# LabJunBMI/E3-invaraint-diffusion-model

Measured on AMD Instinct MI355X. Metric: denoising-steps/sec (batched pocket graphs), higher is better.
Workload: dtype f32 storage and accumulation, f16x3 products (fp32 grade); 1 GPU; structure_model sampling step, 256 x 256-residue pockets per GPU, 12+12 layers x 768, T=1000 schedule, encoder recomputed every step (as the reference); pockets_per_gpu=256, seq_len=256, parallelism=pocket-sharded x1, no collective

## Files before the change

### e3-invaraint-diffusion-model_amd/autograd.py

```python
import os

import torch

from . import hip, ops
from .ops import _chk, _p, _stream


def gemm_general(a, a_kmajor, b, b_kmajor, M, N, K, bias=None, act=ops.ACT_NONE, mode=None):
    _chk(a, "gemm_general.a"); _chk(b, "gemm_general.b"); _chk(bias, "gemm_general.bias")
    assert a.dim() == 2 and b.dim() == 2 and a.stride(1) == 1 and b.stride(1) == 1
    out = torch.empty((M, N), device=a.device, dtype=torch.float32)
    terms = ops.GEMM_MODES[ops.GEMM_MODE if mode is None else mode] or 6
    hip.check(hip.lib().e3d_gemm_f32_split_general(_p(a), a.stride(0), int(a_kmajor), _p(b), b.stride(0),
                                                   int(b_kmajor), _p(bias), _p(out), out.stride(0), M, N, K, act,
                                                   terms, _stream()), "e3d_gemm_f32_split_general")
    return out


class deferred_weight_grads:
    active = None

    MAX_BYTES = int(float(os.environ.get("E3D_DEFER_WGRAD_MAX_GB", "16")) * 2 ** 30)

    OVERLAP = os.environ.get("E3D_WGRAD_OVERLAP", "0") == "1"
# ... 437 lines not shown
        dy = torch.empty_like(y)
        dmod = torch.zeros_like(mod)
        hip.check(hip.lib().e3d_adaln_gate_bwd(_p(dout), _p(y), _p(mod), ctx.branch, ctx.rpc, _p(dy), _p(dmod), M, H,
                                               _stream()), "e3d_adaln_gate_bwd")
        return dout, dy, dmod, None, None


class _EmbedLayerNorm(torch.autograd.Function):

    @staticmethod
    def forward(ctx, x, weight, bias, gamma, beta, eps, post_add, rows_per_add):
        out, z = ops.embed_layernorm(x, weight, bias, gamma, beta, eps, post_add, rows_per_add, want_z=True)
        ctx.save_for_backward(x, z, gamma)
        ctx.eps, ctx.rpa, ctx.has_add = eps, rows_per_add, post_add is not None
        return out

    @staticmethod
    def backward(ctx, dout):
        x, z, gamma = ctx.saved_tensors
        dout = dout.contiguous()
        dz, dg, db_ln = layernorm_bwd(dout, z, gamma, ctx.eps)
        dW, db = small_k_wgrad(dz, x)
        dadd = group_sum(dout, ctx.rpa) if (ctx.has_add and ctx.needs_input_grad[6]) else None
        return None, dW, db, dg, db_ln, None, dadd, None


class _HeadLinear(torch.autograd.Function):
    @staticmethod
    def forward(ctx, x, weight, bias):
        ctx.save_for_backward(x, weight)
        return ops.head_linear(x, weight, bias)

    @staticmethod
    def backward(ctx, dout):
        x, weight = ctx.saved_tensors
        dout = dout.contiguous()
        M, H = x.shape
        dx = torch.empty_like(x)
        hip.check(hip.lib().e3d_head_linear_bwd_dx(_p(dout), _p(weight), _p(dx), M, H, weight.shape[0], _stream()),
                  "e3d_head_linear_bwd_dx")
        dW, _ = small_k_wgrad(x, dout, transpose_out=True, want_bias=False)
        return dx, dW, colsum(dout)


FUSE_HIDDEN_DROPOUT = os.environ.get("E3D_FUSE_HIDDEN_DROPOUT", "1") == "1"


def _needs_grad(*tensors):
    return torch.is_grad_enabled() and any(t is not None and t.requires_grad for t in tensors)


class functional:
    @staticmethod
    def linear(x, weight, bias=None, act=ops.ACT_NONE, absmax=None):
        if _needs_grad(x, weight, bias):
            out = _Linear.apply(x, weight, bias, act, absmax)
        else:
            out = ops.gemm(x, weight, bias, act, absmax=absmax)
        if absmax is not None:
            out._e3d_absmax = absmax
        return out

    @staticmethod
    def attention(q_src, kv_src, B, nh, Lq, Lk, key_mask=None, dist_emb=None, max_pos=0, drop_p=0.0, row_keys=None):
        q_abs = getattr(q_src, "_e3d_absmax", None)
        k_abs = q_abs if kv_src is None else getattr(kv_src, "_e3d_absmax", None)
        bounds = (q_abs, k_abs) if q_abs is not None and k_abs is not None else None
        if _needs_grad(q_src, kv_src, dist_emb):
            return _Attention.apply(q_src, kv_src, dist_emb, key_mask, B, nh, Lq, Lk, max_pos, drop_p, bounds, row_keys)
        q, k, v = _Attention._views(q_src, kv_src, nh * 64)
        drop = ops.site_drop(drop_p, row_keys) if drop_p > 0 else None
        return ops.attention(q, k, v, B, nh, Lq, Lk, key_mask=key_mask, dist_emb=dist_emb, max_pos=max_pos, drop=drop,
                             bounds=bounds)

    @staticmethod
    def dropout(x, p, training=True, row_keys=None):
        if not training or not p:
            return x
        if _needs_grad(x):
            return _Dropout.apply(x, p, row_keys)
        p, seed = ops.site_drop(p, row_keys)[:2]
        return ops.dropout(x.contiguous(), p, seed, row_keys=row_keys)

    @staticmethod
    def residual_layernorm(x, residual, gamma, beta, eps, p_drop=0.0, row_keys=None):
        if _needs_grad(x, residual, gamma, beta):
            return _ResidualLayerNorm.apply(x, residual, gamma, beta, eps, p_drop, row_keys)
        drop = ops.site_drop(p_drop, row_keys) if p_drop and p_drop > 0 else None
        return ops.residual_layernorm(x, residual, gamma, beta, eps, drop=drop)

    @staticmethod
    def linear_residual_layernorm(x, weight, bias, residual, gamma, beta, eps, p_drop=0.0, row_keys=None):
        if not p_drop and not _needs_grad(x, weight, bias, residual, gamma, beta):
            return ops.linear_residual_layernorm(x, weight, bias, residual, gamma, beta, eps)
        fn = functional
        if FUSE_HIDDEN_DROPOUT:
            return fn.residual_layernorm(fn.linear(x, weight, bias), residual, gamma, beta, eps, p_drop, row_keys)
        return fn.residual_layernorm(fn.dropout(fn.linear(x, weight, bias), p_drop, row_keys=row_keys), residual, gamma, beta, eps)

    @staticmethod
    def adaln_gate(x, y, mod, branch, rows_per_cond):
        if _needs_grad(x, y, mod):
            return _AdaLNGate.apply(x, y, mod, branch, rows_per_cond)
        return ops.adaln_gate(x, y, mod, branch, rows_per_cond)

    @staticmethod
    def embed_layernorm(x, weight, bias, gamma, beta, eps, post_add=None, rows_per_add=1):
        if _needs_grad(weight, bias, gamma, beta, post_add):
            return _EmbedLayerNorm.apply(x, weight, bias, gamma, beta, eps, post_add, rows_per_add)
        return ops.embed_layernorm(x, weight, bias, gamma, beta, eps, post_add, rows_per_add)

    @staticmethod
    def head_linear(x, weight, bias):
        if _needs_grad(x, weight, bias):
            return _HeadLinear.apply(x, weight, bias)
        return ops.head_linear(x, weight, bias)
```

### e3-invaraint-diffusion-model_amd/bert.py

```python
from dataclasses import dataclass

import os

import torch
from torch import nn

from . import ops
from .autograd import functional as F


@dataclass
class BertConfig:
    hidden_size: int = 768
    num_attention_heads: int = 12
    intermediate_size: int = 1024
    num_hidden_layers: int = 12
    max_position_embeddings: int = 64
    position_embedding_type: str = "relative_key"
    hidden_dropout_prob: float = 0.1
    attention_probs_dropout_prob: float = 0.1
    layer_norm_eps: float = 1e-12
    hidden_act: str = "gelu"
    use_cache: bool = False
    is_decoder: bool = False
# ... 111 lines not shown
    if not ok:
        with torch.no_grad():
            ent = torch.cat([t.detach() for t in tensors], dim=0).contiguous()
            r0 = 0
            for t in tensors:
                t.data = ent[r0:r0 + t.shape[0]]
                r0 += t.shape[0]
        tied[name] = ent
    return ent


def _packed(owner, name, weights, biases):
    if torch.is_grad_enabled() and any(t.requires_grad for t in weights):
        if TIE_PACKED and all(t.dtype == torch.float32 for t in list(weights) + list(biases)):
            w, b = _TiedPack.apply(_tie(owner, "w_" + name, weights), _tie(owner, "b_" + name, biases), len(weights),
                                   *weights, *biases)
        else:
            w, b = torch.cat(list(weights), dim=0), torch.cat(list(biases), dim=0)
        w._e3d_parts, b._e3d_parts = list(weights), list(biases)
        return w, b
    out = []
    cache = owner.__dict__.setdefault("_e3d_pack", {})
    for key_name, tensors in (("w_" + name, weights), ("b_" + name, biases)):
        key = ops.weight_key(*tensors)
        hit = cache.get(key_name)
        if hit is None or hit[0] != key:
            with torch.no_grad():
                hit = (key, torch.cat([t.detach() for t in tensors], dim=0).contiguous())
            cache[key_name] = hit
        out.append(hit[1])
    return out[0], out[1]


def qkv_weights(sa):
    return _packed(sa, "qkv", [sa.query.weight, sa.key.weight, sa.value.weight], [sa.query.bias, sa.key.bias, sa.value.bias])


def kv_weights(sa):
    return _packed(sa, "kv", [sa.key.weight, sa.value.weight], [sa.key.bias, sa.value.bias])


def dropout_rates(module):
    if not module.training:
        return 0.0, 0.0
    cfg = module.config
    return float(getattr(cfg, "hidden_dropout_prob", 0.0)), float(getattr(cfg, "attention_probs_dropout_prob", 0.0))


def _attention_output(att, ctx, x, p_hidden=0.0, row_keys=None):
    return F.linear_residual_layernorm(ctx, att.output.dense.weight, att.output.dense.bias, x, att.output.LayerNorm.weight,
                                       att.output.LayerNorm.bias, att.eps, p_hidden, row_keys)


def drop_keys(drop):
    return drop[2] if len(drop) > 2 else None


def run_self_attention(att, x, mask, B, L, drop=(0.0, 0.0), layout=None):
    sa = att.self
    w, b = qkv_weights(sa)
    qkv = F.linear(x, w, b, absmax=ops.absmax_slot(sa, "qkv", x.device))
    relkey = sa.position_embedding_type == "relative_key"
    if layout is not None:
        H = att.num_heads * 64
        ctx = ops.attention_varlen(qkv[:, :H], qkv[:, H:2 * H], qkv[:, 2 * H:], layout, layout, att.num_heads,
                                   dist_emb=sa.distance_embedding.weight if relkey else None,
                                   max_pos=sa.max_position_embeddings)
        return _attention_output(att, ctx, x)
    ctx = F.attention(qkv, None, B, att.num_heads, L, L, key_mask=mask,
                      dist_emb=sa.distance_embedding.weight if relkey else None,
                      max_pos=sa.max_position_embeddings, drop_p=drop[1], row_keys=drop_keys(drop))
    return _attention_output(att, ctx, x, drop[0], drop_keys(drop))


def project_cross_kv(att, enc):
    w, b = kv_weights(att.self)
    return F.linear(enc, w, b, absmax=torch.zeros(1, device=enc.device, dtype=torch.float32))


def run_cross_attention(att, x, kv, enc_mask, B, Lq, Lk, drop=(0.0, 0.0), layout=None, enc_layout=None):
    q = F.linear(x, att.self.query.weight, att.self.query.bias, absmax=ops.absmax_slot(att.self, "q", x.device))
    if layout is not None:
        H = att.num_heads * 64
        ctx = ops.attention_varlen(q, kv[:, :H], kv[:, H:], layout, enc_layout, att.num_heads)
        return _attention_output(att, ctx, x)
    ctx = F.attention(q, kv, B, att.num_heads, Lq, Lk, key_mask=enc_mask, drop_p=drop[1], row_keys=drop_keys(drop))
    return _attention_output(att, ctx, x, drop[0], drop_keys(drop))


def run_layer(layer, x, mask, B, L, cross_kv=None, enc_mask=None, Lk=None, drop=(0.0, 0.0), layout=None,
              enc_layout=None):
    x = run_self_attention(layer.attention, x, mask, B, L, drop, layout=layout)
    if hasattr(layer, "crossattention"):
        if cross_kv is None:
            raise ValueError("decoder layer needs encoder states")
        x = run_cross_attention(layer.crossattention, x, cross_kv, enc_mask, B, L, Lk, drop, layout=layout,
                                enc_layout=enc_layout)
    inter = F.linear(x, layer.intermediate.dense.weight, layer.intermediate.dense.bias, ops.ACT_GELU)
    return F.linear_residual_layernorm(inter, layer.output.dense.weight, layer.output.dense.bias, x,
                                       layer.output.LayerNorm.weight, layer.output.LayerNorm.bias, layer.eps, drop[0],
                                       drop_keys(drop))


def run_encoder(encoder, x, mask, B, L, enc=None, enc_mask=None, Lk=None, cross_kv=None, layout=None, enc_layout=None,
                row_keys=None):
    drop = dropout_rates(encoder)
    if layout is not None and drop != (0.0, 0.0):
        raise RuntimeError("packed layouts are inference-only: put the model in eval mode")
    if row_keys is not None:
        drop = drop + (row_keys,)
    for i, layer in enumerate(encoder.layer):
        kv = None
        if hasattr(layer, "crossattention"):
            kv = cross_kv[i] if cross_kv is not None else project_cross_kv(layer.crossattention, enc)
        x = run_layer(layer, x, mask, B, L, kv, enc_mask, Lk, drop, layout=layout, enc_layout=enc_layout)
    return x
```

### e3-invaraint-diffusion-model_amd/csrc/attn_relkey_coop.hip

```cpp
#include <type_traits>

#include "e3d_common.h"

namespace {

typedef __bf16 bf16x8 __attribute__((ext_vector_type(8)));
typedef __bf16 bf16x4 __attribute__((ext_vector_type(4)));
typedef _Float16 f16x8 __attribute__((ext_vector_type(8)));
typedef _Float16 f16x4 __attribute__((ext_vector_type(4)));
template <typename E> struct AV;
template <> struct AV<__bf16> { typedef bf16x8 x8; typedef bf16x4 x4; };
template <> struct AV<_Float16> { typedef f16x8 x8; typedef f16x4 x4; };
template <typename X> struct Elem;
template <> struct Elem<bf16x8> { typedef __bf16 type; };
template <> struct Elem<bf16x4> { typedef __bf16 type; };
template <> struct Elem<f16x8> { typedef _Float16 type; };
template <> struct Elem<f16x4> { typedef _Float16 type; };
__device__ __forceinline__ f32x16 mma16(const bf16x8 a, const bf16x8 b, const f32x16 c) {
    return __builtin_amdgcn_mfma_f32_32x32x16_bf16(a, b, c, 0, 0, 0);
}
__device__ __forceinline__ f32x16 mma16(const f16x8 a, const f16x8 b, const f32x16 c) {
    return __builtin_amdgcn_mfma_f32_32x32x16_f16(a, b, c, 0, 0, 0);
}

// ... 54 lines not shown
    acc = mma16(a[0], b[1], acc);
    acc = mma16(a[1], b[0], acc);
    acc = mma16(a[0], b[0], acc);
    return acc;
}

typedef short short4v __attribute__((ext_vector_type(4)));
typedef short short8v __attribute__((ext_vector_type(8)));
template <typename X8>
__device__ __forceinline__ X8 tr_read8(const unsigned char* lo4, const unsigned char* hi4) {
    typedef __attribute__((address_space(3))) short4v* lds_p;
    const short4v a = __builtin_amdgcn_ds_read_tr16_b64_v4i16((lds_p)(lo4));
    const short4v b = __builtin_amdgcn_ds_read_tr16_b64_v4i16((lds_p)(hi4));
    const short8v c = __builtin_shufflevector(a, b, 0, 1, 2, 3, 4, 5, 6, 7);
    return __builtin_bit_cast(X8, c);
}

template <typename E>
__global__ __launch_bounds__(256) void e_fragments_kernel(const float* __restrict__ e, typename AV<E>::x8* __restrict__ frag,
                                                          int P, int J0, int n_items, float* __restrict__ e_absmax) {
    const int i = blockIdx.x * 256 + threadIdx.x;
    if (i >= n_items) return;
    const int lane = i & 63, kb = (i >> 6) & 3, plane = (i >> 8) & 1, j = i >> 9;
    const int row = min(max(P + 32 * (j - J0) + (lane & 31), 0), 2 * P - 2);
    const float* src = e + row * D + 16 * kb + 8 * (lane >> 5);
    typename AV<E>::x8 out;
    unsigned amax = 0;
#pragma unroll
    for (int t = 0; t < 8; ++t) {
        const float v = src[t];
        const E hi = (E)v;
        out[t] = plane ? (E)(v - (float)hi) : hi;
        e3d_absmax_accum(amax, v);
    }
    frag[i] = out;
    if (e_absmax && plane == 0) e3d_absmax_commit(amax, e_absmax, lane);
}

#ifdef E3D_ATTN_STAMPS
__device__ long long e3d_attn_stamps[16][8];
#define ASTAMP(slot)                                                                                     \
    do {                                                                                                 \
        if (blockIdx.x == 1000 && wid == 1 && lane == 0 && kt < 16) e3d_attn_stamps[kt][slot] = __builtin_readcyclecounter(); \
    } while (0)
#define KSTAMP(i)                                                                                        \
    do {                                                                                                 \
        if (blockIdx.x == 1000 && wid == 1 && lane == 0) e3d_attn_stamps[15][i] = __builtin_readcyclecounter(); \
    } while (0)
#else
#define ASTAMP(slot) do {} while (0)
#define KSTAMP(i) do {} while (0)
#endif

template <int W, bool RELKEY, typename E, bool DROP = false>
__global__ __launch_bounds__(W * 64, 2) void attn_coop_kernel(
    const float* __restrict__ q, int64_t q_bs, int64_t q_rs, const float* __restrict__ k, int64_t k_bs,
    int64_t k_rs, const float* __restrict__ v, int64_t v_bs, int64_t v_rs, const typename AV<E>::x8* __restrict__ e_frag,
    int P, const float* __restrict__ key_mask, float* __restrict__ out, float* __restrict__ lse, int nh, int Lq, int Lk,
    int groups_per_bh, int skip_padded_tiles, E3dBounds bnd, float rescale_tau, E3dDrop drop_in) {
    const E3dDrop drop = e3d_drop_resolve(drop_in);
    typedef typename AV<E>::x8 bf16x8;
    typedef typename AV<E>::x4 bf16x4;
    extern __shared__ __attribute__((aligned(16))) unsigned char smem_raw[];
    constexpr int NT = W * 64, NI = 512 / NT;
    const int tid = threadIdx.x, lane = tid & 63, wid = tid >> 6;
    const int qi = lane & 31, half = lane >> 5;
    const int blk = xcd_remap(blockIdx.x, gridDim.x);
    const int grp = blk % groups_per_bh, bh = blk / groups_per_bh, h = bh % nh, b = bh / nh;
    const int q0 = (grp * W + wid) * 32;
    float* ring = reinterpret_cast<float*>(smem_raw + 2 * KV_BUF_B) + wid * RING_F;
    KSTAMP(0);

    const float* kb_ = k + b * k_bs + h * D;
    const float* vb_ = v + b * v_bs + h * D;
    const float* mb = key_mask ? key_mask + (int64_t)b * Lk : nullptr;
    f32x4 qraw[8];
    {
        const float* qrow = q + b * q_bs + (int64_t)min(q0 + qi, Lq - 1) * q_rs + h * D + 8 * half;
#pragma unroll
        for (int kb = 0; kb < 4; ++kb) {
            qraw[2 * kb] = *reinterpret_cast<const f32x4*>(qrow + 16 * kb);
            qraw[2 * kb + 1] = *reinterpret_cast<const f32x4*>(qrow + 16 * kb + 4);
        }
    }
    uint64_t drop_row = 0;
    if (DROP) drop_row = e3d_drop_attn_row(drop, b, h, nh, Lq, Lk, min(q0 + qi, Lq - 1));
    const bool scan_mask = mb && skip_padded_tiles && e3d_mask_skip_is_exact(bnd);
    float mv[4];
    {
        const float* mp = mb ? mb : kb_;
#pragma unroll
        for (int c = 0; c < 4; ++c) mv[c] = mp[min(64 * c + lane, Lk - 1)];
    }

    bf16x8 qf[4][2];
    int k_tiles = (Lk + 31) >> 5;

    constexpr bool DEEP = NI <= 2;
    constexpr int NSET = DEEP ? 2 : 1;
    f32x4 sk[NSET][NI], sv[NSET][NI];
    float smask[NSET];
    int voff_k[NI], voff_v[NI];
#pragma unroll
    for (int i = 0; i < NI; ++i) {
        const int f = tid + NT * i;
        voff_k[i] = ((f >> 4) * (int)k_rs + 4 * (f & 15)) * 4;
        voff_v[i] = ((f >> 4) * (int)v_rs + 4 * (f & 15)) * 4;
// ... 176 lines not shown
        if (DROP) {
#pragma unroll
            for (int g = 0; g < 4; ++g) {
                float m[4];
                e3d_drop_mult4_row(drop, drop_row, (uint32_t)(kt * 8 + 2 * g + half), m);
#pragma unroll
                for (int j = 0; j < 4; ++j) s[4 * g + j] *= m[j];
            }
        }
        ASTAMP(4);

        const unsigned char* vr = buf + 2 * K_PLANE_B + (4 * half + ((lane >> 2) & 3)) * V_ROW_B +
                                  2 * (16 * ((lane >> 4) & 1) + 4 * (lane & 3));
#pragma unroll
        for (int st = 0; st < 2; ++st) {
            float pv[8];
#pragma unroll
            for (int j = 0; j < 8; ++j) pv[j] = s[8 * st + j];
            bf16x8 pb[2], a0[2], a1[2];
            split8x2(pv, pb[0], pb[1]);
            const unsigned char* v0 = vr + 16 * st * V_ROW_B;
#pragma unroll
            for (int pl = 0; pl < 2; ++pl) {
                a0[pl] = tr_read8<bf16x8>(v0 + pl * V_PLANE_B, v0 + pl * V_PLANE_B + 8 * V_ROW_B);
                a1[pl] = tr_read8<bf16x8>(v0 + pl * V_PLANE_B + 64, v0 + pl * V_PLANE_B + 8 * V_ROW_B + 64);
            }
            o0 = mfma3(a0, pb, o0);
            o1 = mfma3(a1, pb, o1);
        }

        ASTAMP(5);
        if (more) {
            if (DEEP == (PAR == 0)) stage_store(Set1{}, kt_next * 32, smem_raw + (PAR ^ 1) * KV_BUF_B);
            else stage_store(Set0{}, kt_next * 32, smem_raw + (PAR ^ 1) * KV_BUF_B);
        }
        ASTAMP(6);
        if (RELKEY && more) {
            const f32x16 t = dot_q(ef);
            e_load(qt - (kt + 2 < k_tiles ? kt + 2 : k_tiles - 1) - 1 + J0);
#pragma unroll
            for (int r = 0; r < 16; ++r) ring_w[(32 * (PAR ^ 1) + (r & 3) + 8 * (r >> 2)) * RING_LD] = t[r];
        }
        __syncthreads();
        ASTAMP(7);
    };
    for (int kt = 0; kt < k_tiles; kt += 2) {
        tile(std::integral_constant<int, 0>{}, kt);
        if (kt + 1 < k_tiles) tile(std::integral_constant<int, 1>{}, kt + 1);
    }

    KSTAMP(2);
    const float l_tot = l_run + __shfl_xor(l_run, 32, 64);
    const float inv = 1.0f / l_tot;
    __builtin_amdgcn_wave_barrier();
#pragma unroll
    for (int g = 0; g < 4; ++g) {
        f32x4 a, c;
#pragma unroll
        for (int j = 0; j < 4; ++j) { a[j] = o0[4 * g + j] * inv; c[j] = o1[4 * g + j] * inv; }
        *reinterpret_cast<f32x4*>(ring + qi * OUT_LD + 8 * g + 4 * half) = a;
        *reinterpret_cast<f32x4*>(ring + qi * OUT_LD + 32 + 8 * g + 4 * half) = c;
    }
    __builtin_amdgcn_fence(__ATOMIC_RELEASE, "wavefront");
    __builtin_amdgcn_wave_barrier();
    __builtin_amdgcn_fence(__ATOMIC_ACQUIRE, "wavefront");
    float* obase = out + ((int64_t)b * Lq + q0) * (nh * D) + h * D;
#pragma unroll
    for (int i = 0; i < 8; ++i) {
        const int row = 4 * i + (lane >> 4);
        if (q0 + row < Lq)
            *reinterpret_cast<f32x4*>(obase + (int64_t)row * (nh * D) + 4 * (lane & 15)) =
                *reinterpret_cast<const f32x4*>(ring + row * OUT_LD + 4 * (lane & 15));
    }
    if (lse && half == 0 && q0 + qi < Lq) lse[((int64_t)b * nh + h) * Lq + q0 + qi] = m_run * LN2 + logf(l_tot);
    KSTAMP(3);
#ifdef E3D_ATTN_STAMPS
    asm volatile("s_waitcnt vmcnt(0)" ::: "memory");
    KSTAMP(4);
#endif
}

template <int W, bool RELKEY, typename E>
int launch_w(const float* q, int64_t q_bs, int64_t q_rs, const float* k, int64_t k_bs, int64_t k_rs, const float* v,
             int64_t v_bs, int64_t v_rs, const void* e_frag, int P, const float* key_mask,
             float* out, float* lse, int B, int nh, int Lq, int Lk, int q_tiles, int skip, E3dBounds bnd, E3dDrop drop,
             bool dropping, hipStream_t s) {
    const size_t lds = 2 * KV_BUF_B + (size_t)W * RING_F * sizeof(float);
    const int groups = q_tiles / W;
    if constexpr (std::is_same<E, __bf16>::value) {
        if (dropping) {
            static std::atomic<uint64_t> lds_ok_d{0};
            e3d_allow_lds(lds_ok_d, attn_coop_kernel<W, RELKEY, E, true>, lds);
            hipLaunchKernelGGL((attn_coop_kernel<W, RELKEY, E, true>), dim3(B * nh * groups), dim3(W * 64), lds, s, q, q_bs, q_rs,
                               k, k_bs, k_rs, v, v_bs, v_rs, reinterpret_cast<const typename AV<E>::x8*>(e_frag), P, key_mask,
                               out, lse, nh, Lq, Lk, groups, skip, bnd, g_rescale_tau, drop);
            return e3d_launch_status("e3d_relkey_attn_fwd_split (cooperative, dropout)");
        }
    }
    static std::atomic<uint64_t> lds_ok{0};
    e3d_allow_lds(lds_ok, attn_coop_kernel<W, RELKEY, E>, lds);
    hipLaunchKernelGGL((attn_coop_kernel<W, RELKEY, E>), dim3(B * nh * groups), dim3(W * 64), lds, s, q, q_bs, q_rs, k, k_bs,
                       k_rs, v, v_bs, v_rs, reinterpret_cast<const typename AV<E>::x8*>(e_frag), P, key_mask, out, lse, nh, Lq, Lk, groups, skip, bnd, g_rescale_tau, drop);
    return e3d_launch_status("e3d_relkey_attn_fwd_split (cooperative)");
}

template <bool RELKEY, typename E>
int launch_any(int W, const float* q, int64_t q_bs, int64_t q_rs, const float* k, int64_t k_bs, int64_t k_rs,
               const float* v, int64_t v_bs, int64_t v_rs, const void* e_frag, int P,
               const float* key_mask, float* out, float* lse, int B, int nh, int Lq, int Lk, int q_tiles, int skip,
               E3dBounds bnd, E3dDrop drop, bool dropping, hipStream_t s) {
#define E3D_COOP_CASE(w)                                                                                          \
    case w:                                                                                                       \
        return launch_w<w, RELKEY, E>(q, q_bs, q_rs, k, k_bs, k_rs, v, v_bs, v_rs, e_frag, P, key_mask, out, lse, B, nh, \
                                   Lq, Lk, q_tiles, skip, bnd, drop, dropping, s)
    switch (W) {
        E3D_COOP_CASE(8);
        E3D_COOP_CASE(4);
    }
#undef E3D_COOP_CASE
    return -1;
}

}

template <typename E>
static int coop_launch_t(const float* q, int64_t q_bs, int64_t q_rs, const float* k, int64_t k_bs, int64_t k_rs,
                         const float* v, int64_t v_bs, int64_t v_rs, const float* dist_emb, int P,
                         const float* key_mask, float* out, float* lse, int B, int nh, int Lq, int Lk, int skip,
                         E3dBounds bnd, void* e_scratch, int e_ready, E3dDrop drop, bool dropping, hipStream_t s) {
    const int q_tiles = (Lq + 31) / 32;
    static int w_pref = 0;
    if (!w_pref) {
        const char* e = getenv("E3D_ATTN_W");
        w_pref = e ? atoi(e) : 4;
    }
    const int W = (w_pref == 8 && q_tiles % 8 == 0) ? 8 : 4;
    if (!dist_emb)
        return launch_any<false, E>(W, q, q_bs, q_rs, k, k_bs, k_rs, v, v_bs, v_rs, nullptr, P, key_mask, out, lse, B, nh,
                                    Lq, Lk, q_tiles, skip, bnd, drop, dropping, s);
    if (!e_scratch) {
        e3d_set_error("attn_coop: rel-key attention needs the caller's scratch for the distance-table planes");
        return -1;
    }
    const int J0 = (Lk + 31) / 32, n_items = 2 * J0 * 512;
    if (!e_ready)
        hipLaunchKernelGGL(e_fragments_kernel<E>, dim3((n_items + 255) / 256), dim3(256), 0, s, dist_emb,
                           reinterpret_cast<typename AV<E>::x8*>(e_scratch), P, J0, n_items, (float*)nullptr);
    return launch_any<true, E>(W, q, q_bs, q_rs, k, k_bs, k_rs, v, v_bs, v_rs, e_scratch, P, key_mask, out, lse, B, nh, Lq,
                               Lk, q_tiles, skip, bnd, drop, dropping, s);
}

int e3d_attn_coop_launch(const float* q, int64_t q_bs, int64_t q_rs, const float* k, int64_t k_bs, int64_t k_rs,
                         const float* v, int64_t v_bs, int64_t v_rs, const float* dist_emb, int P,
                         const float* key_mask, float* out, float* lse, int B, int nh, int Lq, int Lk, int skip,
                         E3dBounds bnd, void* e_scratch, int e_ready, int f16, E3dDrop drop, bool dropping, hipStream_t s) {
    if (f16)
        return coop_launch_t<_Float16>(q, q_bs, q_rs, k, k_bs, k_rs, v, v_bs, v_rs, dist_emb, P, key_mask, out, lse, B, nh, Lq,
                                       Lk, skip, bnd, e_scratch, e_ready, drop, dropping, s);
    return coop_launch_t<__bf16>(q, q_bs, q_rs, k, k_bs, k_rs, v, v_bs, v_rs, dist_emb, P, key_mask, out, lse, B, nh, Lq, Lk,
                                 skip, bnd, e_scratch, e_ready, drop, dropping, s);
}

extern "C" float e3d_attn_rescale_tau(float tau) {
    const float prev = g_rescale_tau;
    if (tau >= 0.f) g_rescale_tau = tau;
    return prev;
}

#ifdef E3D_ATTN_STAMPS
extern "C" int e3d_debug_read_attn_stamps(long long* host_out) {
    return (int)hipMemcpyFromSymbol(host_out, HIP_SYMBOL(e3d_attn_stamps), sizeof(long long) * 16 * 8);
}
#endif

int e3d_attn_fill_planes(const float* dist_emb, int P, int Lk, void* scratch, int f16, float* e_absmax, hipStream_t s) {
    const int J0 = (Lk + 31) / 32, n_items = 2 * J0 * 512;
    if (f16)
        hipLaunchKernelGGL(e_fragments_kernel<_Float16>, dim3((n_items + 255) / 256), dim3(256), 0, s, dist_emb,
                           reinterpret_cast<f16x8*>(scratch), P, J0, n_items, e_absmax);
    else
        hipLaunchKernelGGL(e_fragments_kernel<__bf16>, dim3((n_items + 255) / 256), dim3(256), 0, s, dist_emb,
                           reinterpret_cast<bf16x8*>(scratch), P, J0, n_items, e_absmax);
    return e3d_launch_status("e3d_relkey_attn_fwd_split (distance-table planes)");
}

extern "C" int64_t e3d_attn_scratch_bytes(int Lk) { return (int64_t)2 * ((Lk + 31) / 32) * 512 * 16; }
```

### e3-invaraint-diffusion-model_amd/csrc/attn_relkey_split.hip

```cpp
#include "attn_split_frag.h"

namespace {

template <int NS, bool RELKEY, bool DROP, typename E>
__global__ __launch_bounds__(256, 2) void attn_fwd_split_kernel(
    const float* __restrict__ q, int64_t q_bs, int64_t q_rs, const float* __restrict__ k, int64_t k_bs,
    int64_t k_rs, const float* __restrict__ v, int64_t v_bs, int64_t v_rs, const float* __restrict__ dist_emb,
    int P, const float* __restrict__ key_mask, float* __restrict__ out, float* __restrict__ lse, int nh, int Lq,
    int Lk, int q_tiles, int n_units, int skip_padded_tiles, E3dBounds bnd, E3dDrop drop_in) {
    const E3dDrop drop = e3d_drop_resolve(drop_in);
    typedef typename AV<E>::x8 bf16x8;
    extern __shared__ __attribute__((aligned(16))) float smem[];
    const int lane = threadIdx.x & 63, wid = threadIdx.x >> 6;
    const int qi = lane & 31, half = lane >> 5;
    const int unit = xcd_remap(blockIdx.x, gridDim.x) * (blockDim.x >> 6) + wid;
    if (unit >= n_units) return;
    const int qt = unit % q_tiles, bh = unit / q_tiles, h = bh % nh, b = bh / nh;
    float* ring = smem + wid * WAVE_LDS_F;
    float* stg = ring + RING_F;
    float* kbias = stg + STG_F;

    const int q0 = qt * 32;
    const int lq = min(q0 + qi, Lq - 1);
    uint64_t drop_row = 0;
// ... 116 lines not shown
            split8<NS>(v0, a0);
            split8<NS>(v1, a1);
            o0 = mfma_terms<NS>(a0, pb, o0);
            o1 = mfma_terms<NS>(a1, pb, o1);
        }
    }

    const float l_tot = l_run + __shfl_xor(l_run, 32, 64);
    const float inv = 1.0f / l_tot;
    if (q0 + qi < Lq) {
        float* orow = out + ((int64_t)b * Lq + q0 + qi) * (nh * D) + h * D;
#pragma unroll
        for (int g = 0; g < 4; ++g) {
            f32x4 lo, hi;
            lo[0] = o0[4 * g + 0] * inv; lo[1] = o1[4 * g + 0] * inv;
            lo[2] = o0[4 * g + 1] * inv; lo[3] = o1[4 * g + 1] * inv;
            hi[0] = o0[4 * g + 2] * inv; hi[1] = o1[4 * g + 2] * inv;
            hi[2] = o0[4 * g + 3] * inv; hi[3] = o1[4 * g + 3] * inv;
            *reinterpret_cast<f32x4*>(orow + 16 * g + 8 * half) = lo;
            *reinterpret_cast<f32x4*>(orow + 16 * g + 8 * half + 4) = hi;
        }
        if (lse && half == 0) lse[((int64_t)b * nh + h) * Lq + q0 + qi] = m_run + logf(l_tot);
    }
}

int g_skip_padded = 1;

template <int NS, bool DROP = false, typename E = __bf16>
int launch(const float* q, int64_t q_bs, int64_t q_rs, const float* k, int64_t k_bs, int64_t k_rs, const float* v,
           int64_t v_bs, int64_t v_rs, const float* dist_emb, int P, const float* key_mask, float* out, float* lse,
           int B, int nh, int Lq, int Lk, E3dBounds bnd, hipStream_t s, E3dDrop drop = E3dDrop{0, 0, 1.f}) {
    const int q_tiles = (Lq + 31) / 32;
    const int n_units = B * nh * q_tiles;
    const int wpb = 4;
    const int n_blocks = (n_units + wpb - 1) / wpb;
    const size_t lds = (size_t)wpb * WAVE_LDS_F * sizeof(float);
    if (dist_emb)
        hipLaunchKernelGGL((attn_fwd_split_kernel<NS, true, DROP, E>), dim3(n_blocks), dim3(64 * wpb), lds, s, q, q_bs, q_rs, k,
                           k_bs, k_rs, v, v_bs, v_rs, dist_emb, P, key_mask, out, lse, nh, Lq, Lk, q_tiles, n_units, g_skip_padded, bnd, drop);
    else
        hipLaunchKernelGGL((attn_fwd_split_kernel<NS, false, DROP, E>), dim3(n_blocks), dim3(64 * wpb), lds, s, q, q_bs, q_rs, k,
                           k_bs, k_rs, v, v_bs, v_rs, dist_emb, P, key_mask, out, lse, nh, Lq, Lk, q_tiles, n_units, g_skip_padded, bnd, drop);
    return e3d_launch_status("e3d_relkey_attn_fwd_split");
}

}

extern "C" int e3d_attn_skip_padded_tiles(int enable) {
    const int prev = g_skip_padded;
    g_skip_padded = enable ? 1 : 0;
    return prev;
}

static int attn_fwd_dispatch(const float* q, int64_t q_bs, int64_t q_rs, const float* k, int64_t k_bs, int64_t k_rs,
                             const float* v, int64_t v_bs, int64_t v_rs, const float* dist_emb, int P, const float* key_mask,
                             float* out, float* lse, int B, int nh, int Lq, int Lk, int terms, float drop_p, const E3dDrop d,
                             void* e_scratch, int e_scratch_ready, const float* q_absmax, const float* k_absmax,
                             float* e_absmax, void* stream) {
    const E3dBounds bnd{q_absmax, k_absmax, dist_emb ? e_absmax : nullptr};
    E3D_REQUIRE(!dist_emb || !q_absmax || e_absmax, "attn_split: rel-key attention with element bounds needs e_absmax too");
    E3D_REQUIRE(drop_p >= 0.f && drop_p < 1.f, "attn_split: drop_p=%g outside [0, 1)", (double)drop_p);
    E3D_REQUIRE(q && k && v && out, "attn_split: null pointer");
    E3D_REQUIRE(B > 0 && nh > 0 && Lq > 0 && Lk > 0, "attn_split: bad shape B=%d nh=%d Lq=%d Lk=%d", B, nh, Lq, Lk);
    E3D_REQUIRE(q_rs % 4 == 0 && k_rs % 4 == 0 && v_rs % 2 == 0 && q_bs % 4 == 0 && k_bs % 4 == 0 && v_bs % 2 == 0,
                "attn_split: strides must keep 16B (q,k) / 8B (v) alignment");
    E3D_REQUIRE(((uintptr_t)q % 16) == 0 && ((uintptr_t)k % 16) == 0 && ((uintptr_t)v % 16) == 0 &&
                    ((uintptr_t)out % 16) == 0, "attn_split: pointers must be 16B aligned");
    E3D_REQUIRE(terms == 3 || terms == 6 || terms == E3D_TERMS_F16X3, "attn_split: terms must be 3, 6 or 19 (got %d)", terms);
    const int f16 = terms == E3D_TERMS_F16X3;
    E3D_REQUIRE((int64_t)Lk * k_rs < (1ll << 30) && (int64_t)Lk * v_rs < (1ll << 30),
                "attn_split: one batch item's K/V slab must stay below 2^30 elements (32-bit lane offsets)");
    if (dist_emb) {
        E3D_REQUIRE(Lq == Lk && Lq <= P, "attn_split: relative_key needs Lq == Lk <= P (Lq=%d Lk=%d P=%d)", Lq, Lk, P);
        E3D_REQUIRE(((uintptr_t)dist_emb % 16) == 0, "attn_split: dist_emb must be 16B aligned");
    }
    E3D_REQUIRE((int64_t)B * nh * ((Lq + 31) / 32) < (1ll << 30), "attn_split: too many tiles");
    hipStream_t s = (hipStream_t)stream;
    if (dist_emb && e_scratch && !e_scratch_ready) {
        const int rc = e3d_attn_fill_planes(dist_emb, P, Lk, e_scratch, f16, e_absmax, s);
        if (rc) return rc;
        e_scratch_ready = 1;
    }
    static int coop = -1;
    if (coop < 0) {
        const char* e = getenv("E3D_ATTN_COOP");
        coop = e ? atoi(e) : 1;
    }
    const bool dropping = drop_p > 0.f;
    const bool span_ok = (int64_t)Lk * (k_rs > v_rs ? k_rs : v_rs) * 4 < ((int64_t)1 << 31) && k_rs > 0 && v_rs > 0 &&
                         k_rs < ((int64_t)1 << 24) && v_rs < ((int64_t)1 << 24);
    if ((terms == 3 || (f16 && !dropping)) && coop && span_ok && v_rs % 4 == 0 && v_bs % 4 == 0 && ((Lq + 31) / 32) % 4 == 0 &&
        (!dist_emb || e_scratch))
        return e3d_attn_coop_launch(q, q_bs, q_rs, k, k_bs, k_rs, v, v_bs, v_rs, dist_emb, P, key_mask, out, lse, B, nh,
                                    Lq, Lk, g_skip_padded, bnd, e_scratch, e_scratch_ready, f16, d, dropping, s);
    if (dropping) {
        if (terms == 3)
            return launch<2, true>(q, q_bs, q_rs, k, k_bs, k_rs, v, v_bs, v_rs, dist_emb, P, key_mask, out, lse, B, nh, Lq, Lk, bnd, s, d);
        return launch<3, true>(q, q_bs, q_rs, k, k_bs, k_rs, v, v_bs, v_rs, dist_emb, P, key_mask, out, lse, B, nh, Lq, Lk, bnd, s, d);
    }
    if (f16)
        return launch<2, false, _Float16>(q, q_bs, q_rs, k, k_bs, k_rs, v, v_bs, v_rs, dist_emb, P, key_mask, out, lse, B, nh,
                                          Lq, Lk, bnd, s);
    if (terms == 3)
        return launch<2>(q, q_bs, q_rs, k, k_bs, k_rs, v, v_bs, v_rs, dist_emb, P, key_mask, out, lse, B, nh, Lq, Lk, bnd, s);
    return launch<3>(q, q_bs, q_rs, k, k_bs, k_rs, v, v_bs, v_rs, dist_emb, P, key_mask, out, lse, B, nh, Lq, Lk, bnd, s);
}

extern "C" int e3d_relkey_attn_fwd_split_ex(const float* q, int64_t q_bs, int64_t q_rs, const float* k, int64_t k_bs,
                                            int64_t k_rs, const float* v, int64_t v_bs, int64_t v_rs,
                                            const float* dist_emb, int P, const float* key_mask, float* out,
                                            float* lse, int B, int nh, int Lq, int Lk, int terms, float drop_p,
                                            uint64_t drop_seed, void* e_scratch, int e_scratch_ready, const float* q_absmax,
                                            const float* k_absmax, float* e_absmax, void* stream) {
    return attn_fwd_dispatch(q, q_bs, q_rs, k, k_bs, k_rs, v, v_bs, v_rs, dist_emb, P, key_mask, out, lse, B, nh, Lq, Lk, terms,
                             drop_p, e3d_drop_make(drop_p, drop_seed), e_scratch, e_scratch_ready, q_absmax, k_absmax, e_absmax,
                             stream);
}

extern "C" int e3d_relkey_attn_fwd_split_ex_keyed(const float* q, int64_t q_bs, int64_t q_rs, const float* k, int64_t k_bs,
                                                  int64_t k_rs, const float* v, int64_t v_bs, int64_t v_rs,
                                                  const float* dist_emb, int P, const float* key_mask, float* out,
                                                  float* lse, int B, int nh, int Lq, int Lk, int terms, float drop_p,
                                                  uint32_t site, const uint64_t* row_keys, void* e_scratch, int e_scratch_ready,
                                                  const float* q_absmax, const float* k_absmax, float* e_absmax, void* stream) {
    E3D_REQUIRE(row_keys && drop_p > 0.f, "attn_split (keyed): row keys and drop_p > 0 required");
    E3D_REQUIRE(site < E3D_DROP_MAX_SITE && nh < E3D_DROP_MAX_HEADS, "attn_split (keyed): site %u / %d heads out of range", site, nh);
    return attn_fwd_dispatch(q, q_bs, q_rs, k, k_bs, k_rs, v, v_bs, v_rs, dist_emb, P, key_mask, out, lse, B, nh, Lq, Lk, terms,
                             drop_p, e3d_drop_make_keyed(drop_p, site, row_keys), e_scratch, e_scratch_ready, q_absmax, k_absmax,
                             e_absmax, stream);
}

extern "C" int e3d_relkey_attn_fwd_split(const float* q, int64_t q_bs, int64_t q_rs, const float* k, int64_t k_bs,
                                         int64_t k_rs, const float* v, int64_t v_bs, int64_t v_rs,
                                         const float* dist_emb, int P, const float* key_mask, float* out, float* lse,
                                         int B, int nh, int Lq, int Lk, int terms, void* stream) {
    return e3d_relkey_attn_fwd_split_ex(q, q_bs, q_rs, k, k_bs, k_rs, v, v_bs, v_rs, dist_emb, P, key_mask, out, lse, B,
                                        nh, Lq, Lk, terms, 0.f, 0, nullptr, 0, nullptr, nullptr, nullptr, stream);
}

extern "C" int e3d_relkey_attn_fwd_split_drop(const float* q, int64_t q_bs, int64_t q_rs, const float* k, int64_t k_bs,
                                              int64_t k_rs, const float* v, int64_t v_bs, int64_t v_rs,
                                              const float* dist_emb, int P, const float* key_mask, float* out,
                                              float* lse, int B, int nh, int Lq, int Lk, int terms, float drop_p,
                                              uint64_t drop_seed, void* stream) {
    return e3d_relkey_attn_fwd_split_ex(q, q_bs, q_rs, k, k_bs, k_rs, v, v_bs, v_rs, dist_emb, P, key_mask, out, lse, B,
                                        nh, Lq, Lk, terms, drop_p, drop_seed, nullptr, 0, nullptr, nullptr, nullptr, stream);
}

extern "C" int e3d_relkey_attn_fwd_split_drop_keyed(const float* q, int64_t q_bs, int64_t q_rs, const float* k, int64_t k_bs,
                                                    int64_t k_rs, const float* v, int64_t v_bs, int64_t v_rs,
                                                    const float* dist_emb, int P, const float* key_mask, float* out,
                                                    float* lse, int B, int nh, int Lq, int Lk, int terms, float drop_p,
                                                    uint32_t site, const uint64_t* row_keys, void* stream) {
    return e3d_relkey_attn_fwd_split_ex_keyed(q, q_bs, q_rs, k, k_bs, k_rs, v, v_bs, v_rs, dist_emb, P, key_mask, out, lse, B,
                                              nh, Lq, Lk, terms, drop_p, site, row_keys, nullptr, 0, nullptr, nullptr, nullptr,
                                              stream);
}
```

### e3-invaraint-diffusion-model_amd/csrc/e3d_common.h

```cpp
#pragma once
#include <hip/hip_runtime.h>
#include <stdint.h>
#include <stdio.h>
#include <math.h>
#include <atomic>

#include "../../include/e3d_hip.h"

typedef float f32x4 __attribute__((ext_vector_type(4)));
typedef float f32x16 __attribute__((ext_vector_type(16)));

void e3d_set_error(const char* fmt, ...);

struct E3dBounds { const float* q; const float* k; const float* e; };


#define E3D_REQUIRE(cond, ...)       \
    do {                             \
        if (!(cond)) {               \
            e3d_set_error(__VA_ARGS__); \
            return -1;               \
        }                            \
    } while (0)

// ... 130 lines not shown
    d.epoch = e3d_dropout_epoch_ptr();
    d.thr = (uint32_t)t;
    d.scale = 65536.0f / (float)(65536 - t);
    d.row_keys = nullptr;
    d.site = 0;
    return d;
}
#define E3D_DROP_MAX_SITE (1u << 24)
#define E3D_DROP_MAX_HEADS (1 << 16)
static inline E3dDrop e3d_drop_make_keyed(float p, uint32_t site, const uint64_t* row_keys) {
    E3dDrop d = e3d_drop_make(p, 0);
    d.epoch = nullptr;
    d.row_keys = row_keys;
    d.site = (uint64_t)site << 40;
    return d;
}
__device__ __forceinline__ E3dDrop e3d_drop_resolve(E3dDrop d) {
    if (d.epoch) d.seed += *d.epoch * 0xD1342543DE82EF95ull;
    d.epoch = nullptr;
    return d;
}
__device__ __forceinline__ void e3d_drop_mult4_row(const E3dDrop d, uint64_t row_term, uint32_t group, float (&m)[4]) {
    uint64_t z = row_term + group;
    z = (z ^ (z >> 30)) * 0xBF58476D1CE4E5B9ull;
    z = (z ^ (z >> 27)) * 0x94D049BB133111EBull;
    z ^= z >> 31;
#pragma unroll
    for (int j = 0; j < 4; ++j) m[j] = ((uint32_t)(z >> (16 * j)) & 0xFFFFu) >= d.thr ? d.scale : 0.f;
}
__device__ __forceinline__ uint64_t e3d_drop_hidden_row(const E3dDrop d, int64_t row, int H4) {
    if (d.row_keys) return d.row_keys[row] * 0x9E3779B97F4A7C15ull + 0x9E3779B97F4A7C15ull + d.site;
    return (uint64_t)row * (uint64_t)H4 + d.seed * 0x9E3779B97F4A7C15ull + 0x9E3779B97F4A7C15ull;
}
__device__ __forceinline__ uint64_t e3d_drop_attn_row(const E3dDrop d, int b, int h, int nh, int Lq, int Lk, int q) {
    if (d.row_keys)
        return d.row_keys[(int64_t)b * Lq + q] * 0x9E3779B97F4A7C15ull + 0x9E3779B97F4A7C15ull + (d.site | (uint64_t)h << 24);
    return ((uint64_t)(b * nh + h) * Lq + q) * (uint64_t)((Lk + 3) >> 2) + d.seed * 0x9E3779B97F4A7C15ull +
           0x9E3779B97F4A7C15ull;
}
__device__ __forceinline__ void e3d_drop_mult4(const E3dDrop d, uint64_t idx4, float (&m)[4]) {
    uint64_t z = idx4 + d.seed * 0x9E3779B97F4A7C15ull + 0x9E3779B97F4A7C15ull;
    z = (z ^ (z >> 30)) * 0xBF58476D1CE4E5B9ull;
    z = (z ^ (z >> 27)) * 0x94D049BB133111EBull;
    z ^= z >> 31;
#pragma unroll
    for (int j = 0; j < 4; ++j) m[j] = ((uint32_t)(z >> (16 * j)) & 0xFFFFu) >= d.thr ? d.scale : 0.f;
}

int e3d_attn_fill_planes(const float* dist_emb, int P, int Lk, void* scratch, int f16, float* e_absmax, hipStream_t s);

int e3d_attn_coop_launch(const float* q, int64_t q_bs, int64_t q_rs, const float* k, int64_t k_bs, int64_t k_rs,
                         const float* v, int64_t v_bs, int64_t v_rs, const float* dist_emb, int P,
                         const float* key_mask, float* out, float* lse, int B, int nh, int Lq, int Lk, int skip,
                         E3dBounds bnd, void* e_scratch, int e_ready, int f16, E3dDrop drop, bool dropping, hipStream_t s);

int e3d_attn_bwd_split_launch(const float* q, int64_t q_bs, int64_t q_rs, const float* k, int64_t k_bs, int64_t k_rs,
                              const float* v, int64_t v_bs, int64_t v_rs, const float* dist_emb, int P,
                              const float* key_mask, const float* out, const float* lse, const float* dout, float* dq,
                              int64_t dq_bs, int64_t dq_rs, float* dk, int64_t dk_bs, int64_t dk_rs, float* dv,
                              int64_t dv_bs, int64_t dv_rs, float* Pm, float* dSm, float* part, int B, int nh, int Lq,
                              int Lk, E3dDrop drop, bool dropping, hipStream_t s);

int64_t e3d_attn_bwd_coop_scratch_bytes(int Lk);
int64_t e3d_attn_bwd_coop_de_floats(int Lq, int Lk);
bool e3d_attn_bwd_coop_supported(int Lq, int Lk, bool dropping);
int e3d_attn_bwd_coop_launch(const float* q, int64_t q_bs, int64_t q_rs, const float* k, int64_t k_bs, int64_t k_rs,
                             const float* v, int64_t v_bs, int64_t v_rs, const float* dist_emb, int P,
                             const float* key_mask, const float* out, const float* lse, const float* dout, float* dq,
                             int64_t dq_bs, int64_t dq_rs, float* dk, int64_t dk_bs, int64_t dk_rs, float* dv,
                             int64_t dv_bs, int64_t dv_rs, float* d_dist_emb, void* e_scratch, float* part, int B, int nh,
                             int Lq, int Lk, E3dDrop drop, bool dropping, hipStream_t s);

__device__ __forceinline__ int xcd_remap(int id, int n) {
    const int q = n >> 3, r = n & 7, xcd = id & 7, slot = id >> 3;
    return (xcd < r ? xcd * (q + 1) : r * (q + 1) + (xcd - r) * q) + slot;
}
```

### e3-invaraint-diffusion-model_amd/csrc/gemm_rowln.hip

```cpp
#include <type_traits>

#include "e3d_common.h"

namespace {

typedef __bf16 bf16x8 __attribute__((ext_vector_type(8)));
typedef _Float16 f16x8 __attribute__((ext_vector_type(8)));
template <typename E> struct V8;
template <> struct V8<__bf16> { typedef bf16x8 t; };
template <> struct V8<_Float16> { typedef f16x8 t; };
__device__ __forceinline__ f32x16 mma16(const bf16x8 a, const bf16x8 b, const f32x16 c) {
    return __builtin_amdgcn_mfma_f32_32x32x16_bf16(a, b, c, 0, 0, 0);
}
__device__ __forceinline__ f32x16 mma16(const f16x8 a, const f16x8 b, const f32x16 c) {
    return __builtin_amdgcn_mfma_f32_32x32x16_f16(a, b, c, 0, 0, 0);
}

constexpr int RN = 768, RBM = 96, NBLK = RN / 32;
constexpr int W_STEP = NBLK * 2 * 1024;
constexpr int A_PAIR = 128 * 128;
constexpr int LDS_A = 2 * W_STEP;
constexpr int RES_CHUNK = 16 * RN * 4;
constexpr int LDS_STATS = 3 * RES_CHUNK;
constexpr int LDS_COLS = LDS_STATS + (8 * RBM + RBM) * 4;
// ... 39 lines not shown

#ifndef ROWLN_LAB
#define ROWLN_LAB 0
#endif
#ifdef ROWLN_STAMPS
__device__ long long rowln_stamps[2][64][8];
__device__ long long rowln_tile_stamps[2][8][8];
__device__ long long rowln_wg_times[512][4];
#define RSTAMP(step, slot)                                                                                        \
    do {                                                                                                          \
        if (stamp_on && (step) < 64 && lane == 0) rowln_stamps[wid >> 2][(step)][(slot)] = __builtin_readcyclecounter(); \
    } while (0)
#define TSTAMP(slot)                                                                                              \
    do {                                                                                                          \
        if (stamp_on && tile_no < 8 && lane == 0) rowln_tile_stamps[wid >> 2][tile_no][(slot)] = __builtin_readcyclecounter(); \
    } while (0)
#else
#define RSTAMP(step, slot) do {} while (0)
#define TSTAMP(slot) do {} while (0)
#endif
#define E3D_VMCNT(n) asm volatile("s_waitcnt vmcnt(" #n ")" ::: "memory")
#define E3D_BARRIER()                          \
    do {                                       \
        asm volatile("" ::: "memory");         \
        __builtin_amdgcn_s_barrier();          \
        asm volatile("" ::: "memory");         \
        __builtin_amdgcn_sched_barrier(0);     \
    } while (0)
#define E3D_LDS_BARRIER()                                   \
    do {                                                    \
        asm volatile("s_waitcnt lgkmcnt(0)" ::: "memory");  \
        E3D_BARRIER();                                      \
    } while (0)

template <int OFF = 0>
__device__ __forceinline__ void glds16(const void* g, unsigned char* lds_wave_base) {
    __builtin_amdgcn_global_load_lds((const __attribute__((address_space(1))) void*)g,
                                     (__attribute__((address_space(3))) void*)lds_wave_base, 16, OFF, 0);
}

__device__ __forceinline__ int next_tile_rows(int left, int pattern, int group_rows) {
#ifndef ROWLN_NO_PATTERNS
    if (group_rows == 256) {
        if (pattern == 1 && left == 256) return 64;
        if (pattern == 2 && left == 160) return 64;
        if (pattern == 3) return 64;
    }
#endif
    if (left >= 160 || left == 96) return 96;
    if (left > 96) return 64;
    return left;
}

template <typename E>
__global__ __launch_bounds__(512, 2) void gemm_rowln_kernel(const float* __restrict__ A, int64_t lda,
                                                            const unsigned char* __restrict__ Wp, const float* __restrict__ bias,
                                                            const float* __restrict__ res, int64_t ldr,
                                                            const float* __restrict__ gamma, const float* __restrict__ beta,
                                                            float eps, float* __restrict__ out, int64_t ldo, int M, int K,
                                                            int rows_per_wg, float out_scale) {
    extern __shared__ __attribute__((aligned(16))) unsigned char smem[];
    typedef typename V8<E>::t X8;
    const int tid = threadIdx.x, lane = tid & 63;
    const int wid = __builtin_amdgcn_readfirstlane(tid >> 6);
    const int l31 = lane & 31, half = lane >> 5;
    const int npairs = K / 32, last_step = 2 * npairs - 1;

    int row0 = blockIdx.x * rows_per_wg;
    const int row_end = min(M, row0 + rows_per_wg);
    if (row0 >= row_end) return;

    const unsigned w_lane = (unsigned)(wid * 6144 + lane * 16);
    unsigned a_lane[2];
    auto a_offsets = [&](int rows) {
#pragma unroll
        for (int i = 0; i < 2; ++i) {
            const int row = (wid + 8 * i) * 8 + (lane >> 3);
            a_lane[i] = (unsigned)(min(row, rows - 1) * (int)lda + (((lane & 7) ^ ((row >> 1) & 7)) << 2)) * 4u;
        }
    };
    unsigned r_lane[2];
#pragma unroll
    for (int j = 0; j < 2; ++j) r_lane[j] = (unsigned)((2 * wid + j) * (int)ldr + lane * 4) * 4u;
    const int a_roff = LDS_A + l31 * 128 + (((2 * half) ^ ((l31 >> 1) & 7)) << 4);
    const int b_roff = (wid * 3) * 2048 + lane * 16;

    auto issue_w = [&](int src, int buf) {
        const unsigned char* g = Wp + (int64_t)src * W_STEP + w_lane;
        unsigned char* l = smem + buf * W_STEP + wid * 6144;
        glds16<0>(g, l);
        glds16<1024>(g, l);
        glds16<2048>(g, l);
        glds16<3072>(g, l);
        glds16<0>(g + 4096, l + 4096);
        glds16<1024>(g + 4096, l + 4096);
    };
    auto issue_a = [&](const float* a_tile, int pair, int buf) {
        const unsigned char* g = reinterpret_cast<const unsigned char*>(a_tile + pair * 32);
        unsigned char* l = smem + LDS_A + buf * A_PAIR + wid * 1024;
        glds16<0>(g + a_lane[0], l);
        glds16<0>(g + a_lane[1], l + 8192);
    };

    float* red = reinterpret_cast<float*>(smem + LDS_STATS);
    float* rowc = red + 8 * RBM;
    const int colbase = wid * 96 + l31;
    float* colc = reinterpret_cast<float*>(smem + LDS_COLS);
    for (int i = tid; i < RN; i += 512) {
        colc[i] = bias ? bias[i] : 0.f;
        colc[RN + i] = gamma[i];
        colc[2 * RN + i] = beta[i];
    }
    asm volatile("s_waitcnt vmcnt(0) lgkmcnt(0)" ::: "memory");
    constexpr float inv_n = 1.0f / RN;
    const bool bit8 = (lane & 8) != 0, bit4 = (lane & 4) != 0, bit2 = (lane & 2) != 0,
               bit1 = (lane & 1) != 0;

    const int pattern = (blockIdx.x >> 3) & 3, group_rows = row_end - row0;
    int rows = next_tile_rows(row_end - row0, pattern, group_rows);
    a_offsets(rows);
    issue_a(A + (int64_t)row0 * lda, 0, 0);
    issue_w(0, 0);
    issue_w(1, 1);
    issue_a(A + (int64_t)row0 * lda, 1, 1);
    int next_row0 = 0, next_rows = 0;
#ifdef ROWLN_STAMPS
    const bool stamp_on = blockIdx.x == 77 && (wid & 3) == 0;
    int tile_no = 0;
    if (tid == 0 && blockIdx.x < 512) {
        rowln_wg_times[blockIdx.x][0] = __builtin_amdgcn_s_memrealtime();
        rowln_wg_times[blockIdx.x][1] = __builtin_readcyclecounter();
    }
#endif

    auto tile_body = [&](auto nm_c) -> bool {
        constexpr int NM = decltype(nm_c)::value;
        const float* a_tile = A + (int64_t)row0 * lda;
        f32x16 acc[NM][3];
#pragma unroll
        for (int m = 0; m < NM; ++m)
#pragma unroll
            for (int n = 0; n < 3; ++n)
#pragma unroll
                for (int r = 0; r < 16; ++r) acc[m][n][r] = 0.f;

        TSTAMP(0);
        int a_cur = 0, a_nxt = A_PAIR, a_nx2 = 2 * A_PAIR;
        E3D_VMCNT(8);
        E3D_BARRIER();
        TSTAMP(1);
        X8 bh0[3], bl0[3], bh1[3], bl1[3];
        f32x4 x0, x1;
#pragma unroll
        for (int n = 0; n < 3; ++n) {
            bh0[n] = *reinterpret_cast<const X8*>(smem + b_roff + n * 2048);
            bl0[n] = *reinterpret_cast<const X8*>(smem + b_roff + n * 2048 + 1024);
        }
        x0 = *reinterpret_cast<const f32x4*>(smem + a_cur + a_roff);
        x1 = *reinterpret_cast<const f32x4*>(smem + a_cur + (a_roff ^ 16));

        const bool res_on = res != nullptr && !(ROWLN_LAB & 1);
        const unsigned char* res_tile = reinterpret_cast<const unsigned char*>(res + (int64_t)row0 * ldr);
        const int64_t res_chunk_stride = 16 * ldr * 4;
        auto step = [&](auto ks_c, X8 (&bh)[3], X8 (&bl)[3], X8 (&nh)[3], X8 (&nl)[3], int w_next, int a_pair_next, int tail_chunk, int stamp_step) {
            constexpr int KS = decltype(ks_c)::value;
            RSTAMP(stamp_step, 0);
            asm volatile("s_waitcnt lgkmcnt(0)" ::: "memory");
            const bool tail = tail_chunk >= 0;
            const unsigned char* gbase = tail ? res_tile + tail_chunk * res_chunk_stride : Wp + (int64_t)w_next * W_STEP;
            const unsigned char* g0 = gbase + (tail ? r_lane[0] : w_lane);
            const unsigned char* g1 = gbase + (tail ? r_lane[1] : w_lane + 3072u);
            unsigned char* lw = smem + KS * W_STEP + wid * 6144;
            f32x4 y0 = x0, y1 = x1;
#pragma unroll
            for (int m = 0; m < NM; ++m) {
                X8 ah, al;
                split8(x0, x1, ah, al);
                if (m + 1 < NM) {
                    x0 = *reinterpret_cast<const f32x4*>(smem + a_cur + ((a_roff ^ (64 * KS)) + (m + 1) * 4096));
                    x1 = *reinterpret_cast<const f32x4*>(smem + a_cur + ((a_roff ^ (64 * KS + 16)) + (m + 1) * 4096));
                }
#pragma unroll
                for (int n = 0; n < 3; ++n) {
                    if (ROWLN_LAB & 8) {
                        asm volatile("" :: "v"(ah), "v"(al), "v"(bh[n]), "v"(bl[n]));
                    } else {
                        acc[m][n] = mma16(ah, bl[n], acc[m][n]);
                        acc[m][n] = mma16(al, bh[n], acc[m][n]);
                        acc[m][n] = mma16(ah, bh[n], acc[m][n]);
                    }
                    if (m == 0) {
                        if (n == 0) { glds16<0>(g0, lw); glds16<1024>(g0, lw); }
                        if (n == 1) { glds16<2048>(g0, lw); glds16<0>(g1, lw + 3072); }
                        if (n == 2) { glds16<1024>(g1, lw + 3072); glds16<2048>(g1, lw + 3072); }
                    }
                    __builtin_amdgcn_sched_barrier(0);
                }
                if (m == 0) {
                    RSTAMP(stamp_step, 1);
                    if (KS == 1) {
                        E3D_VMCNT(12);
                        E3D_BARRIER();
                        RSTAMP(stamp_step, 4);
                        if (a_pair_next >= 0) {
                            const unsigned char* ga = reinterpret_cast<const unsigned char*>(a_tile + a_pair_next * 32);
                            unsigned char* la = smem + LDS_A + a_nx2 + wid * 1024;
                            glds16<0>(ga + a_lane[0], la);
                            glds16<0>(ga + a_lane[1], la + 8192);
                        }
                    }
                    E3D_VMCNT(8);
                    RSTAMP(stamp_step, 3);
                    const unsigned char* wn = smem + (KS ^ 1) * W_STEP + b_roff;
#pragma unroll
                    for (int n = 0; n < 3; ++n) {
                        nh[n] = *reinterpret_cast<const X8*>(wn + n * 2048);
                        nl[n] = *reinterpret_cast<const X8*>(wn + n * 2048 + 1024);
                    }
                    const int an = KS == 0 ? a_cur : a_nxt;
                    y0 = *reinterpret_cast<const f32x4*>(smem + an + (a_roff ^ (64 * (KS ^ 1))));
                    y1 = *reinterpret_cast<const f32x4*>(smem + an + (a_roff ^ (64 * (KS ^ 1) + 16)));
                    __builtin_amdgcn_sched_barrier(0);
                }
            }
            x0 = y0;
            x1 = y1;
            RSTAMP(stamp_step, 2);
        };

        for (int p = 0; p < npairs; ++p) {
            const bool last_pair = p + 1 == npairs;
            step(std::integral_constant<int, 0>{}, bh0, bl0, bh1, bl1, min(2 * p + 2, last_step), 0, last_pair && res_on ? 0 : -1, 2 * p);
            step(std::integral_constant<int, 1>{}, bh1, bl1, bh0, bl0, min(2 * p + 3, last_step), last_pair ? -1 : min(p + 2, npairs - 1),
                 last_pair && res_on ? 1 : -1, 2 * p + 1);
            const int t = a_cur;
            a_cur = a_nxt;
            a_nxt = a_nx2;
            a_nx2 = t;
        }
        if (!res_on) E3D_VMCNT(0);
        E3D_LDS_BARRIER();
        TSTAMP(2);

#pragma unroll
        for (int m = 0; m < NM; ++m)
#pragma unroll
            for (int n = 0; n < 3; ++n)
#pragma unroll
                for (int r = 0; r < 16; ++r) acc[m][n][r] = fmaf(acc[m][n][r], out_scale, colc[colbase + 32 * n]);
        if (res_on) {
            auto issue_r = [&](int c) {
                const unsigned char* g = res_tile + c * res_chunk_stride;
                unsigned char* l = smem + (c % 3) * RES_CHUNK + wid * 6144;
                glds16<0>(g + r_lane[0], l);
                glds16<1024>(g + r_lane[0], l);
                glds16<2048>(g + r_lane[0], l);
                glds16<0>(g + r_lane[1], l + 3072);
                glds16<1024>(g + r_lane[1], l + 3072);
                glds16<2048>(g + r_lane[1], l + 3072);
            };
            constexpr int NCH = 2 * NM;
#pragma unroll
            for (int c = 0; c < NCH; ++c) {
                if (c + 1 < NCH) E3D_VMCNT(6);
                else E3D_VMCNT(0);
                E3D_BARRIER();
                if (c + 2 < NCH) issue_r(c + 2);
                const int m = c >> 1, r0 = 8 * (c & 1);
                const unsigned char* cb = smem + (c % 3) * RES_CHUNK + colbase * 4 + half * (4 * RN * 4);
#pragma unroll
                for (int n = 0; n < 3; ++n)
#pragma unroll
                    for (int j = 0; j < 8; ++j) {
                        const int lr = (j & 3) + 8 * (j >> 2);
// ... 102 lines not shown
                        else u[4 * q + j] = t;
                    }
                }
            if (PAIR) tv = reduce32(v);
            if (SINGLE) tu = reduce16(u);
            exchange(tv, tu, true);
        }
        TSTAMP(4);
        float gv[3], bt[3];
#pragma unroll
        for (int n = 0; n < 3; ++n) {
            gv[n] = colc[RN + colbase + 32 * n];
            bt[n] = colc[2 * RN + colbase + 32 * n];
        }
#pragma unroll
        for (int m = 0; m < NM; ++m)
#pragma unroll
            for (int q = 0; q < 4; ++q) {
                const f32x4 rstd = *reinterpret_cast<const f32x4*>(rowc + m * 32 + 8 * q + 4 * half);
                float* o = out + (int64_t)(row0 + m * 32 + 8 * q + 4 * half) * ldo + colbase;
#pragma unroll
                for (int j = 0; j < 4; ++j)
#pragma unroll
                    for (int n = 0; n < 3; ++n) o[(int64_t)j * ldo + 32 * n] = fmaf(acc[m][n][4 * q + j] * rstd[j], gv[n], bt[n]);
            }
        TSTAMP(5);
#ifdef ROWLN_STAMPS
        asm volatile("s_waitcnt vmcnt(0)" ::: "memory");
        TSTAMP(6);
        ++tile_no;
#endif
        if (more) E3D_LDS_BARRIER();
        return more;
    };

    while (true) {
        bool more;
        if (rows == 96) more = tile_body(std::integral_constant<int, 3>{});
        else if (rows == 64) more = tile_body(std::integral_constant<int, 2>{});
        else more = tile_body(std::integral_constant<int, 1>{});
        if (!more) break;
        row0 = next_row0;
        rows = next_rows;
    }
    E3D_VMCNT(0);
#ifdef ROWLN_STAMPS
    if (tid == 0 && blockIdx.x < 512) {
        rowln_wg_times[blockIdx.x][2] = __builtin_amdgcn_s_memrealtime();
        rowln_wg_times[blockIdx.x][3] = __builtin_readcyclecounter();
    }
#endif
}

template <typename E>
int launch_rowln(const float* A, int64_t lda, const void* Wp, const float* bias, const float* res, int64_t ldr,
                 const float* gamma, const float* beta, float eps, float* out, int64_t ldo, int M, int K, float out_scale,
                 hipStream_t s) {
    static std::atomic<uint64_t> lds_ok{0};
    e3d_allow_lds(lds_ok, gemm_rowln_kernel<E>, (size_t)LDS_TOTAL);
    const int n_cu = e3d_cu_count();
    const int rows_per_wg = ((M + n_cu - 1) / n_cu + 31) / 32 * 32;
    const int grid = (M + rows_per_wg - 1) / rows_per_wg;
    hipLaunchKernelGGL((gemm_rowln_kernel<E>), dim3(grid), dim3(512), LDS_TOTAL, s, A, lda,
                       reinterpret_cast<const unsigned char*>(Wp), bias, res, ldr, gamma, beta, eps, out, ldo, M, K, rows_per_wg,
                       out_scale);
    return e3d_launch_status("e3d_gemm_residual_layernorm_f32_split");
}

}

#ifdef ROWLN_STAMPS
extern "C" int e3d_debug_rowln_stamps(long long* steps, long long* tiles) {
    int rc = (int)hipMemcpyFromSymbol(steps, HIP_SYMBOL(rowln_stamps), sizeof(long long) * 2 * 64 * 8);
    if (rc) return rc;
    return (int)hipMemcpyFromSymbol(tiles, HIP_SYMBOL(rowln_tile_stamps), sizeof(long long) * 2 * 8 * 8);
}
extern "C" int e3d_debug_rowln_wg_times(long long* t) {
    return (int)hipMemcpyFromSymbol(t, HIP_SYMBOL(rowln_wg_times), sizeof(long long) * 512 * 4);
}
#endif

extern "C" int64_t e3d_weight_planes_bytes(int N, int K) { return (N % 32 || K % 16 || N <= 0 || K <= 0) ? -1 : (int64_t)N * K * 4; }

extern "C" int e3d_weight_planes_f32_split(const float* W, int N, int K, int terms, void* planes, void* stream) {
    E3D_REQUIRE(W && planes, "weight_planes: null pointer");
    E3D_REQUIRE(N > 0 && K > 0 && N % 32 == 0 && K % 16 == 0 && ((uintptr_t)W % 16) == 0 && ((uintptr_t)planes % 16) == 0,
                "weight_planes: need N%%32==0, K%%16==0, 16-byte alignment (N=%d K=%d)", N, K);
    E3D_REQUIRE(terms == 3 || terms == E3D_TERMS_F16X3, "weight_planes: terms must be 3 or 19 (got %d)", terms);
    const int pieces = (K / 16) * (N / 32);
    const dim3 grid((pieces + 3) / 4), block(256);
    if (terms == 3) hipLaunchKernelGGL(weight_planes_kernel<__bf16>, grid, block, 0, (hipStream_t)stream, W, N, K, (unsigned char*)planes);
    else hipLaunchKernelGGL(weight_planes_kernel<_Float16>, grid, block, 0, (hipStream_t)stream, W, N, K, (unsigned char*)planes);
    return e3d_launch_status("e3d_weight_planes_f32_split");
}

extern "C" int e3d_gemm_residual_layernorm_supported(int M, int N, int K, int64_t lda) {
    return M >= 32 && M % 32 == 0 && N == RN && K >= 64 && K % 32 == 0 && lda >= K && lda % 4 == 0 && (int64_t)RBM * lda < (1ll << 31);
}

extern "C" int e3d_gemm_residual_layernorm_f32_split(const float* A, int64_t lda, const void* w_planes, const float* bias,
                                                     const float* residual, int64_t ldr, const float* gamma, const float* beta,
                                                     float eps, float* out, int64_t ldo, int M, int N, int K, int terms,
                                                     float out_scale, void* stream) {
    E3D_REQUIRE(A && w_planes && gamma && beta && out, "gemm_residual_layernorm: null pointer");
    E3D_REQUIRE(e3d_gemm_residual_layernorm_supported(M, N, K, lda),
                "gemm_residual_layernorm: need M%%32==0, N==768, K%%32==0, K>=64 (M=%d N=%d K=%d lda=%lld)", M, N, K, (long long)lda);
    E3D_REQUIRE(((uintptr_t)A % 16) == 0 && ((uintptr_t)w_planes % 16) == 0 && ldo >= N, "gemm_residual_layernorm: alignment / ldo");
    E3D_REQUIRE(!residual || (ldr >= N && ldr % 4 == 0 && ((uintptr_t)residual % 16) == 0 && 16 * ldr < (1ll << 31)),
                "gemm_residual_layernorm: residual needs ldr >= N, ldr%%4==0, 16-byte alignment");
    E3D_REQUIRE(terms == 3 || terms == E3D_TERMS_F16X3, "gemm_residual_layernorm: terms must be 3 or 19 (got %d)", terms);
    hipStream_t s = (hipStream_t)stream;
    if (terms == 3) return launch_rowln<__bf16>(A, lda, w_planes, bias, residual, ldr, gamma, beta, eps, out, ldo, M, K, out_scale, s);
    return launch_rowln<_Float16>(A, lda, w_planes, bias, residual, ldr, gamma, beta, eps, out, ldo, M, K, out_scale, s);
}
```

### e3-invaraint-diffusion-model_amd/csrc/gemm_split.hip

```cpp
#include <type_traits>

#include "e3d_common.h"

namespace {

typedef __bf16 bf16x8 __attribute__((ext_vector_type(8)));
typedef __bf16 bf16x4 __attribute__((ext_vector_type(4)));
typedef _Float16 f16x8 __attribute__((ext_vector_type(8)));
typedef _Float16 f16x4 __attribute__((ext_vector_type(4)));

template <typename E> struct Vec;
template <> struct Vec<__bf16> { typedef bf16x8 x8; typedef bf16x4 x4; };
template <> struct Vec<_Float16> { typedef f16x8 x8; typedef f16x4 x4; };
__device__ __forceinline__ f32x16 mma16(const bf16x8 a, const bf16x8 b, const f32x16 c) {
    return __builtin_amdgcn_mfma_f32_32x32x16_bf16(a, b, c, 0, 0, 0);
}
__device__ __forceinline__ f32x16 mma16(const f16x8 a, const f16x8 b, const f32x16 c) {
    return __builtin_amdgcn_mfma_f32_32x32x16_f16(a, b, c, 0, 0, 0);
}

struct Epi { float* absmax; float scale; int plan_m = 0; const int* run_if = nullptr; };

constexpr int BN = 128, BK = 32;
#ifdef GEMM_STAMPS
// ... 665 lines not shown
            if (more) {
#pragma unroll
                for (int i = 0; i < NI; ++i) item_store(i, next);
            }
            STAMP(5);
            __syncthreads();
            STAMP(6);
            cur ^= 1;
        } else {
            __syncthreads();
            if (more) {
#pragma unroll
                for (int i = 0; i < NI; ++i) item_store(i, smem_raw);
            }
            __syncthreads();
        }
    }

    STAMP_K(3);
    unsigned amax = 0;
#pragma unroll
    for (int m = 0; m < 4; ++m) {
#pragma unroll
        for (int n = 0; n < 2; ++n) {
            const int col = col0 + wc * 64 + n * 32 + l31;
            const float bv = bias ? bias[col] : 0.f;
#pragma unroll
            for (int r = 0; r < 16; ++r) {
                const int row = row0 + wr * 128 + m * 32 + mfma32_row(r, half);
                float v = fmaf(acc[m][n][r], out_scale, bv);
                if (ACT == E3D_ACT_GELU) v = gelu_erf(v);
                if (ACT == E3D_ACT_SILU) v = silu(v);
                if (row < M) {
                    out[(int64_t)row * ldc + col] = v;
                    if (ACT == E3D_ACT_NONE && absmax) e3d_absmax_accum(amax, v);
                }
            }
        }
    }
    if (ACT == E3D_ACT_NONE && absmax) e3d_absmax_commit(amax, absmax, lane);
    STAMP_K(4);
#ifdef E3D_STAMPS
    asm volatile("s_waitcnt vmcnt(0)" ::: "memory");
    STAMP_K(5);
#endif
}

#ifdef E3D_NT_STORES
#define E3D_STORE_OUT(ptr, val) __builtin_nontemporal_store((val), (ptr))
#else
#define E3D_STORE_OUT(ptr, val) (*(ptr) = (val))
#endif

template <int ACT, typename E>
__global__ __launch_bounds__(512, 2) void gemm_split256p_kernel(const float* __restrict__ A, int64_t lda,
                                                                 const float* __restrict__ W,
                                                                 const float* __restrict__ bias,
                                                                 float* __restrict__ out, int64_t ldc, int N, int K,
                                                                 int tiles_m, int tiles_n, float* __restrict__ absmax, float out_scale,
                                                                 const int* __restrict__ run_if) {
    if (run_if && *run_if == 0) return;
    extern __shared__ __attribute__((aligned(16))) unsigned char smem_raw[];
    constexpr int NS = 2, T_BYTES = BT * ROW64, BUF_BYTES = 2 * NS * T_BYTES;
    constexpr int NI = 8;
    const int total = tiles_m * tiles_n, nk = K / BK;
    const int tid = threadIdx.x, lane = tid & 63, wid = tid >> 6;
    const int wr = wid >> 2, wc = wid & 3;
    const int l31 = lane & 31, half = lane >> 5;

    unsigned goff[NI];
    int dst[NI];
#pragma unroll
    for (int i = 0; i < NI; ++i) {
        const int f = tid + 512 * (i & 3), r = f >> 3, kg = f & 7;
        goff[i] = (unsigned)(r * (i < 4 ? (int)lda : K) + kg * 4);
        dst[i] = (i < 4 ? 0 : NS * T_BYTES) + swz_off(r, kg >> 1) + (kg & 1) * 8;
    }

    int ld_tile = blockIdx.x, ld_k = 0;
    const float* ld_a;
    const float* ld_w;
    auto cursor_bases = [&]() {
        const int lid = xcd_remap(ld_tile, total);
        ld_a = A + (int64_t)(lid / tiles_n) * BT * lda + ld_k * BK;
        ld_w = W + (int64_t)(lid % tiles_n) * BT * K + ld_k * BK;
    };
    auto cursor_advance = [&]() {
        if (ld_k + 1 < nk) {
            ++ld_k;
            ld_a += BK;
            ld_w += BK;
        } else if (ld_tile + (int)gridDim.x < total) {
            ld_tile += gridDim.x;
            ld_k = 0;
            cursor_bases();
        }
    };
    f32x4 rg[NI];
    auto item_load = [&](int i) { rg[i] = *reinterpret_cast<const f32x4*>((i < 4 ? ld_a : ld_w) + goff[i]); };
    auto item_store = [&](int i, unsigned char* buf) {
        typename Vec<E>::x4 p[NS];
        split4<NS, E>(rg[i], p);
#pragma unroll
        for (int s = 0; s < NS; ++s) *reinterpret_cast<typename Vec<E>::x4*>(buf + s * T_BYTES + dst[i]) = p[s];
    };
    cursor_bases();
#pragma unroll
    for (int i = 0; i < NI; ++i) item_load(i);
    cursor_advance();
#pragma unroll
    for (int i = 0; i < NI; ++i) item_store(i, smem_raw);
#pragma unroll
    for (int i = 0; i < NI; ++i) item_load(i);
    cursor_advance();
    __syncthreads();

    int a_row[4], b_row[2];
#pragma unroll
    for (int m = 0; m < 4; ++m) a_row[m] = wr * 128 + m * 32 + l31;
#pragma unroll
    for (int n = 0; n < 2; ++n) b_row[n] = wc * 64 + n * 32 + l31;
    int cur = 0;
    unsigned amax = 0;

    for (int tile = blockIdx.x; tile < total; tile += gridDim.x) {
        f32x16 acc[4][2];
#pragma unroll
        for (int m = 0; m < 4; ++m)
#pragma unroll
            for (int n = 0; n < 2; ++n)
#pragma unroll
                for (int r = 0; r < 16; ++r) acc[m][n][r] = 0.f;
        for (int kt = 0; kt < nk; ++kt) {
            const unsigned char* base = smem_raw + cur * BUF_BYTES;
            unsigned char* next = smem_raw + (cur ^ 1) * BUF_BYTES;
#pragma unroll
            for (int ks = 0; ks < 2; ++ks) {
                typename Vec<E>::x8 fa[NS][4], fb[NS][2];
#pragma unroll
                for (int s = 0; s < NS; ++s) {
#pragma unroll
                    for (int n = 0; n < 2; ++n)
                        fb[s][n] = *reinterpret_cast<const typename Vec<E>::x8*>(base + (NS + s) * T_BYTES +
                                                                    swz_off(b_row[n], 2 * ks + half));
#pragma unroll
                    for (int m = 0; m < 4; ++m)
                        fa[s][m] = *reinterpret_cast<const typename Vec<E>::x8*>(base + s * T_BYTES + swz_off(a_row[m], 2 * ks + half));
                }
#pragma unroll
                for (int m = 0; m < 4; ++m) {
                    const int g = ks * 4 + m;
                    item_store(g, next);
                    item_load(g);
#pragma unroll
                    for (int n = 0; n < 2; ++n) {
                        acc[m][n] = mma16(fa[0][m], fb[1][n], acc[m][n]);
                        acc[m][n] = mma16(fa[1][m], fb[0][n], acc[m][n]);
                        acc[m][n] = mma16(fa[0][m], fb[0][n], acc[m][n]);
                    }
                    __builtin_amdgcn_sched_barrier(0);
                }
            }
            cursor_advance();
            __syncthreads();
            cur ^= 1;
        }

        const int lid = xcd_remap(tile, total);
        const int row0 = (lid / tiles_n) * BT, col0 = (lid % tiles_n) * BT;
#pragma unroll
        for (int m = 0; m < 4; ++m) {
#pragma unroll
            for (int n = 0; n < 2; ++n) {
                const int col = col0 + wc * 64 + n * 32 + l31;
                const float bv = bias ? bias[col] : 0.f;
                float* o = out + (int64_t)(row0 + wr * 128 + m * 32 + 4 * half) * ldc + col;
#pragma unroll
                for (int r = 0; r < 16; ++r) {
                    float v = fmaf(acc[m][n][r], out_scale, bv);
                    if (ACT == E3D_ACT_GELU) v = gelu_erf(v);
                    if (ACT == E3D_ACT_SILU) v = silu(v);
                    E3D_STORE_OUT(&o[(int64_t)((r & 3) + 8 * (r >> 2)) * ldc], v);
                    if (ACT == E3D_ACT_NONE && absmax) e3d_absmax_accum(amax, v);
                }
            }
        }
    }
    if (ACT == E3D_ACT_NONE && absmax) e3d_absmax_commit(amax, absmax, lane);
}

template <int ACT, typename E>
int launch256p(const float* A, int64_t lda, const float* W, const float* bias, float* out, int64_t ldc, int M, int N,
               int K, Epi epi, hipStream_t s) {
    const int tiles_m = M / BT, tiles_n = N / BT;
    constexpr size_t lds = 2 * 2 * 2 * BT * ROW64;
    static std::atomic<uint64_t> lds_ok{0};
    const int n_cu = e3d_cu_count();
    const int total = tiles_m * tiles_n;
    e3d_allow_lds(lds_ok, gemm_split256p_kernel<ACT, E>, lds);
    hipLaunchKernelGGL((gemm_split256p_kernel<ACT, E>), dim3(total < n_cu ? total : n_cu), dim3(512), lds, s, A, lda, W, bias, out,
                       ldc, N, K, tiles_m, tiles_n, epi.absmax, epi.scale, epi.run_if);
    return e3d_launch_status("e3d_gemm_f32_split (persistent 256x256)");
}

int g_general_form = -1;
int g_tile_pref = -1;

template <int NS, int ACT, int WR, int WC, int NBUF, bool PIPE, typename E>
int launch256(const float* A, int64_t lda, const float* W, const float* bias, float* out, int64_t ldc, int M, int N,
              int K, Epi epi, hipStream_t s) {
    constexpr int TM = WR * 128, TN = WC * 64;
    const int tiles_m = (M + TM - 1) / TM, tiles_n = N / TN;
    const size_t lds = (size_t)NBUF * NS * (TM + TN) * ROW64;
    static std::atomic<uint64_t> lds_ok{0};
    e3d_allow_lds(lds_ok, gemm_split256_kernel<NS, ACT, WR, WC, NBUF, PIPE, E>, lds);
    hipLaunchKernelGGL((gemm_split256_kernel<NS, ACT, WR, WC, NBUF, PIPE, E>), dim3(tiles_m * tiles_n), dim3(WR * WC * 64), lds, s,
                       A, lda, W, bias, out, ldc, M, N, K, tiles_m, tiles_n, epi.absmax, epi.scale, epi.run_if);
    return e3d_launch_status("e3d_gemm_f32_split (128x64 wave tiles)");
}

template <int NS, int ACT, bool A_KMAJ, bool B_KMAJ, int WM, int WN, typename E, int TN = 2, bool TR = false>
int launch_general(const float* A, int64_t lda, const float* B, int64_t ldb, const float* bias, float* out, int64_t ldc,
                   int M, int N, int K, Epi epi, hipStream_t s);

int p_min() {
    static int v = 0;
    if (!v) {
        const char* e = getenv("E3D_GEMM_P_MIN");
        v = e ? atoi(e) : 160;
    }
    return v;
}

template <int NS, int ACT, bool A_KMAJ, bool B_KMAJ, typename E>
int launch(const float* A, int64_t lda, const float* B, int64_t ldb, const float* bias, float* out, int64_t ldc,
           int M, int N, int K, Epi epi, hipStream_t s) {
    if (g_tile_pref < 0) {
        const char* e = getenv("E3D_GEMM_TILE");
        g_tile_pref = e ? atoi(e) : 4;
    }
    const int Mp = epi.plan_m > 0 ? epi.plan_m : M;
    if constexpr (!A_KMAJ && !B_KMAJ) {
        if constexpr (NS == 2) {
            const int64_t n_tiles = (int64_t)(Mp / BT) * (N / BT);
            if (N % BT == 0 && M % BT == 0 && Mp % BT == 0 && ldb == K && g_tile_pref >= 4 && K >= 2 * BK && lda < (1 << 22) &&
                (g_tile_pref >= 5 || n_tiles >= p_min() || (n_tiles >= 96 && N >= 6 * BT && !getenv("E3D_GEMM_P_MIN"))))
                return launch256p<ACT, E>(A, lda, B, bias, out, ldc, M, N, K, epi, s);
            if (N % BT == 0 && ldb == K && g_tile_pref >= 3 && (int64_t)((Mp + BT - 1) / BT) * (N / BT) >= 256)
                return launch256<NS, ACT, 2, 4, 2, true, E>(A, lda, B, bias, out, ldc, M, N, K, epi, s);
        }
        if constexpr (NS == 1) {
            if (N % BT == 0 && ldb == K && g_tile_pref >= 3 && (int64_t)((Mp + BT - 1) / BT) * (N / BT) >= 160)
                return launch256<NS, ACT, 2, 4, 2, true, E>(A, lda, B, bias, out, ldc, M, N, K, epi, s);
        }
        if (N % BT == 0 && ldb == K && g_tile_pref >= 1 &&
            (int64_t)((Mp + BT - 1) / BT) * (N / BT) >= 256)
            return launch256<NS, ACT, 2, 4, (NS <= 2 ? 2 : 1), false, E>(A, lda, B, bias, out, ldc, M, N, K, epi, s);
    }
    if (g_general_form < 0) {
        const char* e = getenv("E3D_GEMM_FORM");
        g_general_form = e ? atoi(e) : 0;
    }
    int form = g_general_form;
    if (form != 1 && form != 2 && form != 3 && form != 4) {
        const int64_t g256 = (int64_t)((Mp + 255) / 256) * ((N + 127) / 128), g128 = (int64_t)((Mp + 127) / 128) * ((N + 127) / 128);
        const int64_t cus = e3d_cu_count();
        if (NS == 3) form = g256 < 128 && !A_KMAJ && !B_KMAJ ? 2 : 1;
        else if (A_KMAJ && B_KMAJ) form = 1;
        else if (A_KMAJ) form = g128 <= cus ? 2 : (g256 <= cus ? 1 : (45 * ((g128 + 2 * cus - 1) / (2 * cus)) < 37 * ((g256 + cus - 1) / cus) ? 2 : 1));
        else form = 25 * ((g128 + cus - 1) / cus) <= 38 * ((g256 + cus - 1) / cus) ? 3 : 1;
        if (NS == 2 && !A_KMAJ && !B_KMAJ && Mp <= 2048 && N <= 1024) form = 4;
    }
    if constexpr (NS == 2 && !A_KMAJ && !B_KMAJ) {
        if (form == 4) return launch_general<NS, ACT, A_KMAJ, B_KMAJ, 2, 2, E, 1>(A, lda, B, ldb, bias, out, ldc, M, N, K, epi, s);
    }
    if (form == 4) form = 3;
    if constexpr (NS <= 2 && !A_KMAJ) {
        if (form == 3) return launch_general<NS, ACT, A_KMAJ, B_KMAJ, 2, 4, E, 1>(A, lda, B, ldb, bias, out, ldc, M, N, K, epi, s);
    }
    if (form == 3) form = 2;
    if (form == 2) return launch_general<NS, ACT, A_KMAJ, B_KMAJ, 2, 2, E>(A, lda, B, ldb, bias, out, ldc, M, N, K, epi, s);
    if constexpr (A_KMAJ && B_KMAJ) {
        static const bool tr_on = !getenv("E3D_WGRAD_TR") || atoi(getenv("E3D_WGRAD_TR")) != 0;
        if (tr_on && M % 4 == 0 && N % 4 == 0 && lda % 4 == 0 && ldb % 4 == 0 && ((uintptr_t)A % 16) == 0 && ((uintptr_t)B % 16) == 0 &&
            e3d_tr_span_ok(K, lda) && e3d_tr_span_ok(K, ldb))
            return launch_general<NS, ACT, A_KMAJ, B_KMAJ, 4, 2, E, 2, true>(A, lda, B, ldb, bias, out, ldc, M, N, K, epi, s);
    }
    return launch_general<NS, ACT, A_KMAJ, B_KMAJ, 4, 2, E>(A, lda, B, ldb, bias, out, ldc, M, N, K, epi, s);
}

template <int NS, int ACT, bool A_KMAJ, bool B_KMAJ, int WM, int WN, typename E, int TN, bool TR>
int launch_general(const float* A, int64_t lda, const float* B, int64_t ldb, const float* bias, float* out, int64_t ldc,
                   int M, int N, int K, Epi epi, hipStream_t s) {
    constexpr int BM = WM * 64, BNt = WN * 32 * TN;
    const int tiles_m = (M + BM - 1) / BM, tiles_n = (N + BNt - 1) / BNt;
    constexpr int NBUF = NS <= 2 ? 2 : 1;
    size_t lds = (size_t)NBUF * NS * (BM + BNt) * ROW_B;
    static const bool spread = !getenv("E3D_GEMM_SPREAD") || atoi(getenv("E3D_GEMM_SPREAD")) != 0;
    if (spread && BM * BNt == 128 * 128 && (int64_t)tiles_m * tiles_n <= e3d_cu_count() && lds < (size_t)84 * 1024) lds = (size_t)84 * 1024;
// ... 183 lines not shown
        if (p < count) {
            tiles += (int64_t)((N[q] + 255) / 256) * ((K[q] + 127) / 128);
            tr = tr && N[q] % 4 == 0 && K[q] % 4 == 0 && ldz[q] % 4 == 0 && ldx[q] % 4 == 0 && ((uintptr_t)dz[q] % 16) == 0 &&
                 ((uintptr_t)x[q] % 16) == 0 && e3d_tr_span_ok(M, ldz[q]) && e3d_tr_span_ok(M, ldx[q]);
        }
    }
    E3D_REQUIRE(tiles < (1ll << 30), "gemm_wgrad_ragged: too many tiles");
    for (int p = count; p <= 64; ++p) g.tile_start[p] = (int)tiles;
    g.accumulate = accumulate_bits;
    const dim3 grid((unsigned)tiles), block(512);
    hipStream_t s = (hipStream_t)stream;
    auto go = [&](auto kern, size_t lds, std::atomic<uint64_t>& lds_ok) {
        e3d_allow_lds(lds_ok, kern, lds);
        hipLaunchKernelGGL(kern, grid, block, lds, s, g, M, count);
    };
    static std::atomic<uint64_t> ok1{0}, ok1t{0}, ok2{0}, ok2t{0}, ok3{0}, ok3t{0};
    if (terms == E3D_TERMS_BF16) {
        const size_t lds = (size_t)2 * 1 * (256 + 128) * ROW_B;
        if (tr) go(gemm_wgrad_ragged_kernel<1, true>, lds, ok1t);
        else go(gemm_wgrad_ragged_kernel<1, false>, lds, ok1);
    } else if (terms == 3) {
        const size_t lds = (size_t)2 * 2 * (256 + 128) * ROW_B;
        if (tr) go(gemm_wgrad_ragged_kernel<2, true>, lds, ok2t);
        else go(gemm_wgrad_ragged_kernel<2, false>, lds, ok2);
    } else {
        const size_t lds = (size_t)1 * 3 * (256 + 128) * ROW_B;
        if (tr) go(gemm_wgrad_ragged_kernel<3, true>, lds, ok3t);
        else go(gemm_wgrad_ragged_kernel<3, false>, lds, ok3);
    }
    return e3d_launch_status("e3d_gemm_wgrad_ragged_f32_split");
}

extern "C" int e3d_gemm_bias_act_f32_split(const float* A, int64_t lda, const float* W,
                                           const float* bias, float* out, int64_t ldc, int M,
                                           int N, int K, int act, int terms, void* stream) {
    E3D_REQUIRE(N % BN == 0, "gemm_split: need N%%128==0 (N=%d)", N);
    return gemm_split_general(A, lda, 0, W, (int64_t)K, 0, bias, out, ldc, M, N, K, act, terms, nullptr, 1.0f, stream);
}

extern "C" int e3d_gemm_bias_act_f32_split_ex(const float* A, int64_t lda, const float* W, const float* bias, float* out,
                                              int64_t ldc, int M, int N, int K, int act, int terms, float* out_absmax,
                                              float out_scale, void* stream) {
    E3D_REQUIRE(N % BN == 0, "gemm_split: need N%%128==0 (N=%d)", N);
    return gemm_split_general(A, lda, 0, W, (int64_t)K, 0, bias, out, ldc, M, N, K, act, terms, out_absmax, out_scale, stream);
}

extern "C" int e3d_gemm_bias_act_f32_split_gated(const float* A, int64_t lda, const float* W, const float* bias, float* out,
                                                 int64_t ldc, int M, int N, int K, int act, int terms, float* out_absmax,
                                                 float out_scale, int plan_m, const int* run_if, void* stream) {
    E3D_REQUIRE(N % BN == 0, "gemm_split: need N%%128==0 (N=%d)", N);
    return gemm_split_general(A, lda, 0, W, (int64_t)K, 0, bias, out, ldc, M, N, K, act, terms, out_absmax, out_scale, stream,
                              plan_m, run_if);
}
```

### e3-invaraint-diffusion-model_amd/hip.py

```python
import ctypes
import os
from ctypes import c_char_p, c_float, c_int, c_int64, c_uint32, c_uint64, c_void_p

_HERE = os.path.dirname(os.path.abspath(__file__))
LIB_PATH = os.environ.get("E3D_HIP_LIB", os.path.join(_HERE, "libe3d_hip.so"))
ABI_VERSION = 5

_P = c_void_p
_SIGNATURES = {
    "e3d_abi_version": (c_int, []),
    "e3d_last_error": (c_char_p, []),
    "e3d_gemm_bias_act_f32": (c_int, [_P, c_int64, _P, _P, _P, c_int64, c_int, c_int, c_int, c_int, _P]),
    "e3d_gemm_bias_act_f32_split": (c_int, [_P, c_int64, _P, _P, _P, c_int64, c_int, c_int, c_int, c_int, c_int, _P]),
    "e3d_gemm_bias_act_f32_split_ex": (c_int, [_P, c_int64, _P, _P, _P, c_int64, c_int, c_int, c_int, c_int, c_int, _P, c_float, _P]),
    "e3d_gemm_bias_act_f32_split_gated": (c_int, [_P, c_int64, _P, _P, _P, c_int64, c_int, c_int, c_int, c_int, c_int, _P, c_float,
                                                  c_int, _P, _P]),
    "e3d_absmax_f32": (c_int, [_P, c_int64, _P, _P]),
    "e3d_relkey_attn_fwd": (c_int, [_P, c_int64, c_int64, _P, c_int64, c_int64, _P, c_int64, c_int64,
                                    _P, c_int, _P, _P, _P, c_int, c_int, c_int, c_int, _P]),
    "e3d_relkey_attn_fwd_split": (c_int, [_P, c_int64, c_int64, _P, c_int64, c_int64, _P, c_int64, c_int64,
                                          _P, c_int, _P, _P, _P, c_int, c_int, c_int, c_int, c_int, _P]),
    "e3d_gemm_skinny_workspace_bytes": (c_int64, [c_int, c_int, c_int]),
    "e3d_gemm_skinny_f32_split": (c_int, [_P, c_int64, _P, _P, _P, c_int64, c_int, c_int, c_int, c_int, c_int, _P, c_int64, _P]),
    "e3d_gemm_skinny_f32_split_ex": (c_int, [_P, c_int64, _P, _P, _P, c_int64, c_int, c_int, c_int, c_int, c_int, _P, c_int64, _P, c_float, _P]),
    "e3d_gemm_skinny_plan_select": (None, [c_int, c_int]),
    "e3d_gemm_skinny_residual_layernorm_f32_split": (c_int, [_P, c_int64, _P, _P, _P, _P, _P, c_float, _P, c_int, c_int, c_int,
                                                     c_int, _P, c_int64, _P]),
    "e3d_gemm_skinny_residual_layernorm_f32_split_ex": (c_int, [_P, c_int64, _P, _P, _P, _P, _P, c_float, _P, c_int, c_int, c_int,
                                                        c_int, _P, c_int64, c_float, _P]),
    "e3d_attn_skip_padded_tiles": (c_int, [c_int]),
    "e3d_gemm_kernel_select": (c_int, [c_int]),
    "e3d_gemm_general_select": (c_int, [c_int]),
    "e3d_attn_rescale_tau": (c_float, [c_float]),
    "e3d_residual_layernorm_fwd": (c_int, [_P, _P, _P, _P, c_float, _P, _P, c_int, c_int, _P]),
    "e3d_adaln_gate_fwd": (c_int, [_P, _P, _P, c_int, c_int, _P, c_int, c_int, _P]),
    "e3d_embed_layernorm_fwd": (c_int, [_P, c_int, _P, _P, _P, _P, c_float, _P, c_int, _P, _P, c_int, c_int, _P]),
    "e3d_adaln_gate_indexed_fwd": (c_int, [_P, _P, _P, _P, c_int, _P, c_int, _P, c_int, c_int, _P]),
    "e3d_classify_onehot_rows": (c_int, [_P, c_int, _P, _P, c_int, _P]),
    "e3d_embed_layernorm_fwd_ex": (c_int, [_P, c_int, _P, _P, _P, _P, c_float, _P, c_int, _P, _P, c_int, c_int, _P, _P]),
    "e3d_nerf_backbone": (c_int, [_P, _P, _P, c_int, c_int, c_int, _P]),
    "e3d_gemm_f32_split_general": (c_int, [_P, c_int64, c_int, _P, c_int64, c_int, _P, _P, c_int64, c_int, c_int,
                                           c_int, c_int, c_int, _P]),
    "e3d_transpose_grouped_f32": (c_int, [_P, _P, c_int, c_int, c_int, c_int64, c_int64, _P]),
    "e3d_gemm_wgrad_grouped_f32_split": (c_int, [_P, _P, _P, _P, c_uint64, c_int, c_int64, c_int64, c_int, c_int, c_int, c_int, _P]),
    "e3d_residual_layernorm_drop_fwd": (c_int, [_P, _P, _P, _P, c_float, _P, _P, c_int, c_int, c_float, c_uint64, _P]),
    "e3d_layernorm_bwd_drop": (c_int, [_P, _P, _P, c_float, _P, _P, _P, _P, c_int, c_int, c_float, c_uint64, _P]),
    "e3d_weight_planes_bytes": (c_int64, [c_int, c_int]),
    "e3d_weight_planes_f32_split": (c_int, [_P, c_int, c_int, c_int, _P, _P]),
    "e3d_gemm_residual_layernorm_supported": (c_int, [c_int, c_int, c_int, c_int64]),
    "e3d_gemm_residual_layernorm_f32_split": (c_int, [_P, c_int64, _P, _P, _P, c_int64, _P, _P, c_float, _P, c_int64,
                                                      c_int, c_int, c_int, c_int, c_float, _P]),
    "e3d_gemm_wgrad_ragged_f32_split": (c_int, [_P, _P, _P, _P, _P, _P, _P, _P, c_uint64, c_int, c_int, c_int, _P]),
    "e3d_relkey_attn_bwd_workspace_floats": (c_int64, [c_int, c_int, c_int, c_int, c_int]),
    "e3d_relkey_attn_bwd": (c_int, [_P, c_int64, c_int64, _P, c_int64, c_int64, _P, c_int64, c_int64, _P, c_int, _P,
                                    _P, _P, _P, _P, c_int64, c_int64, _P, c_int64, c_int64, _P, c_int64, c_int64,
                                    _P, _P, c_int, c_int, c_int, c_int, _P]),
    "e3d_dropout_f32": (c_int, [_P, c_float, c_uint64, _P, c_int64, _P]),
    "e3d_relkey_attn_fwd_split_drop": (c_int, [_P, c_int64, c_int64, _P, c_int64, c_int64, _P, c_int64, c_int64,
                                               _P, c_int, _P, _P, _P, c_int, c_int, c_int, c_int, c_int, c_float,
                                               c_uint64, _P]),
    "e3d_relkey_attn_fwd_split_ex": (c_int, [_P, c_int64, c_int64, _P, c_int64, c_int64, _P, c_int64, c_int64,
                                             _P, c_int, _P, _P, _P, c_int, c_int, c_int, c_int, c_int, c_float,
                                             c_uint64, _P, c_int, _P, _P, _P, _P]),
    "e3d_attn_scratch_bytes": (c_int64, [c_int]),
    "e3d_ddpm_step_wrap_table": (c_int, [_P, _P, _P, _P, _P, c_int, _P, c_int64, _P]),
    "e3d_relkey_attn_bwd_drop": (c_int, [_P, c_int64, c_int64, _P, c_int64, c_int64, _P, c_int64, c_int64, _P, c_int, _P,
                                         _P, _P, _P, _P, c_int64, c_int64, _P, c_int64, c_int64, _P, c_int64, c_int64,
                                         _P, _P, c_int, c_int, c_int, c_int, c_float, c_uint64, _P]),
    "e3d_relkey_attn_bwd_ex": (c_int, [_P, c_int64, c_int64, _P, c_int64, c_int64, _P, c_int64, c_int64, _P, c_int, _P,
                                       _P, _P, _P, _P, c_int64, c_int64, _P, c_int64, c_int64, _P, c_int64, c_int64,
                                       _P, _P, c_int, c_int, c_int, c_int, c_int, c_float, c_uint64, _P]),
    "e3d_attn_dropout_mask": (c_int, [c_int, c_int, c_int, c_int, c_float, c_uint64, _P, _P]),
    "e3d_layernorm_bwd": (c_int, [_P, _P, _P, c_float, _P, _P, _P, c_int, c_int, _P]),
    "e3d_layernorm_bwd_workspace_floats": (c_int64, [c_int, c_int]),
    "e3d_layernorm_bwd_ws": (c_int, [_P, _P, _P, c_float, _P, _P, _P, _P, c_int, c_int, c_float, c_uint64, _P, c_int64, _P]),
    "e3d_adaln_gate_bwd": (c_int, [_P, _P, _P, c_int, c_int, _P, _P, c_int, c_int, _P]),
    "e3d_act_fwd": (c_int, [_P, c_int, _P, c_int64, _P]),
    "e3d_act_bwd": (c_int, [_P, _P, c_int, _P, c_int64, _P]),
    "e3d_colsum": (c_int, [_P, c_int64, _P, c_int, c_int, _P]),
    "e3d_group_sum": (c_int, [_P, c_int, _P, c_int, c_int, _P]),
    "e3d_small_k_wgrad": (c_int, [_P, _P, _P, _P, c_int, c_int, c_int, c_int, _P]),
    "e3d_head_linear_bwd_dx": (c_int, [_P, _P, _P, c_int, c_int, c_int, _P]),
    "e3d_head_linear_fwd": (c_int, [_P, _P, _P, _P, c_int, c_int, c_int, _P]),
    "e3d_ddpm_step_wrap": (c_int, [_P, _P, _P, c_float, c_float, c_float, c_float, c_int, _P, c_int64, _P]),
    "e3d_q_sample_wrap": (c_int, [_P, _P, _P, _P, _P, _P, c_int, c_int64, _P]),
    "e3d_discrete_posterior_sample": (c_int, [_P, _P, _P, _P, _P, c_int, _P, _P, c_int, c_int, c_int, _P]),
    "e3d_discrete_q_sample": (c_int, [_P, _P, _P, c_int, _P, c_int, c_int, c_int, _P]),
    "e3d_optim_chunk_elems": (c_int, []),
    "e3d_grad_global_norm": (c_int, [_P, _P, _P, _P, c_int, c_float, _P, _P, _P]),
    "e3d_adamw_step_dyn": (c_int, [_P, _P, _P, _P, _P, _P, _P, c_int, _P, _P, c_float, c_float, c_float, c_float, _P]),
    "e3d_adamw_step_dev": (c_int, [_P, _P, _P, _P, _P, _P, _P, c_int, _P, _P, _P]),
    "e3d_dropout_set_epoch_ptr": (c_int, [_P]),
    "e3d_adamw_step": (c_int, [_P, _P, _P, _P, _P, _P, _P, c_int, _P, c_float, c_float, c_float, c_float, c_float, c_int, _P]),
    "e3d_attn_varlen_fwd": (c_int, [_P, c_int64, _P, c_int64, _P, c_int64, _P, _P, _P, _P, _P, c_int, _P, c_int, _P,
                                    c_int64, c_int, c_int, c_int, c_int, _P]),
    "e3d_keyed_ddpm_step_wrap": (c_int, [_P, _P, _P, _P, _P, c_uint64, c_int, _P, c_int64, c_int, _P]),
    "e3d_keyed_discrete_posterior_sample": (c_int, [_P, _P, _P, _P, _P, c_uint64, _P, _P, c_int, c_int, c_int, _P]),
    "e3d_keyed_draws": (c_int, [_P, c_uint64, c_int, c_int, c_int, c_int, c_int, c_float, _P, c_int64, _P]),
    "e3d_strided_step_wrap": (c_int, [_P, _P, _P, _P, _P, c_int, c_int, c_int, _P, c_int64, _P]),
    "e3d_keyed_strided_step_wrap": (c_int, [_P, _P, _P, _P, c_int, _P, c_uint64, c_int, c_int, _P, c_int64, c_int, _P]),
    "e3d_keyed_timesteps": (c_int, [_P, _P, c_uint64, c_int, c_int, _P, c_int, _P]),
    "e3d_keyed_q_sample_wrap": (c_int, [_P, _P, _P, _P, c_int, c_float, _P, _P, c_uint64, _P, _P, c_int, c_int, c_int, _P]),
    "e3d_keyed_discrete_q_sample": (c_int, [_P, _P, _P, _P, c_uint64, _P, c_int, c_int, c_int, _P]),
    "e3d_keyed_drop_row_keys": (c_int, [_P, c_int, c_int, _P, c_uint64, c_int, _P, _P]),
# ... 55 lines not shown
```

### e3-invaraint-diffusion-model_amd/ops.py

```python
import contextlib
import math
import os
import warnings

import torch

from . import hip, keyed

ACT_NONE, ACT_GELU, ACT_SILU = 0, 1, 2


def _stream():
    return torch.cuda.current_stream().cuda_stream


TRACE = None


_ROCTX = None


def _roctx():
    global _ROCTX
    if _ROCTX is None:
# ... 134 lines not shown
    global _f16_warned
    ent = getattr(weight, "_e3d_f16w", None)
    key = weight_key(weight)
    if ent is not None and ent[0] == key:
        return ent[1], ent[2]
    if torch.cuda.is_current_stream_capturing():
        raise RuntimeError("f16x3: the pre-scaled copy of a weight is missing inside a stream capture -- run the step eagerly once "
                           "before capturing it (building the copy reads max |w| back to the host)")
    with torch.no_grad():
        amax = float(weight.detach().abs().max())
        if not math.isfinite(amax) or amax == 0.0:
            if not math.isfinite(amax) and not _f16_warned:
                _f16_warned = True
                warnings.warn("f16x3: a weight holds inf / NaN -- used as it is (the outputs will say so)")
            scaled, inv = weight.detach(), 1.0
        else:
            k = max(-120, min(120, F16_WEIGHT_EXP - math.frexp(amax)[1]))
            scaled, inv = (weight.detach() * (2.0 ** k)).contiguous(), 2.0 ** -k
    try:
        weight._e3d_f16w = (key, scaled, inv)
    except AttributeError:
        pass
    return scaled, inv


SKINNY_MAX_M = 1024 if os.environ.get("E3D_GEMM_SKINNY", "1") == "1" else 0
SKINNY_GEMM_MAX_M = int(os.environ.get("E3D_GEMM_SKINNY_MAX_M", "512"))
SKINNY_MAX_TILES = 768
_SKINNY_WS = {}
_SKINNY_RETIRED = []


def _skinny_workspace(device, M, N, K):
    nbytes = hip.lib().e3d_gemm_skinny_workspace_bytes(M, N, K)
    key = (device.index, torch.cuda.current_stream(device).cuda_stream)
    ws = _SKINNY_WS.get(key)
    if ws is None or ws.numel() < nbytes:
        if ws is not None:
            _SKINNY_RETIRED.append(ws)
        ws = _SKINNY_WS[key] = torch.empty(max(nbytes, 8 << 20), dtype=torch.uint8, device=device)
    return ws


def _skinny_ok(terms, M, N, K, a):
    return (terms in (3, 19) and 0 < M <= SKINNY_MAX_M and N % 32 == 0 and K % 16 == 0 and a.stride(0) % 4 == 0
            and -(-M // 32) * (N // 32) <= SKINNY_MAX_TILES)


def gemm_is_tiled(M, mode=None):
    terms = GEMM_MODES[GEMM_MODE if mode is None else mode]
    return terms != 0 and not (terms in (3, 19) and M <= min(SKINNY_MAX_M, SKINNY_GEMM_MAX_M))


def gemm(a, weight, bias=None, act=ACT_NONE, out=None, mode=None, absmax=None, prescale=True, plan_m=None, run_if=None):
    _chk(a, "gemm.a"); _chk(weight, "gemm.weight"); _chk(bias, "gemm.bias")
    assert a.dim() == 2 and a.stride(1) == 1 and weight.is_contiguous()
    M, K = a.shape
    N = weight.shape[0]
    assert weight.shape[1] == K, (a.shape, weight.shape)
    if out is None:
        out = torch.empty((M, N), device=a.device, dtype=torch.float32)
    assert out.dim() == 2 and out.stride(1) == 1 and out.shape == (M, N)
    terms = GEMM_MODES[GEMM_MODE if mode is None else mode]
    if absmax is not None:
        _chk(absmax, "gemm.absmax")
        assert act == ACT_NONE and absmax.numel() == 1
    scale = 1.0
    if terms == 19 and prescale:
        weight, scale = f16_weight(weight)
    if plan_m is not None or run_if is not None:
        _chk(run_if, "gemm.run_if", torch.int32)
        plan_m = M if plan_m is None else plan_m
        if not gemm_is_tiled(plan_m, mode):
            raise ValueError(f"gemm: plan_m / run_if exist on the tiled split kernels only (plan_m={plan_m}, mode={mode or GEMM_MODE})")
        with _timed("gemm" if run_if is None else "gemm_gated", (M, N, K, act)):
            hip.check(hip.lib().e3d_gemm_bias_act_f32_split_gated(
                _p(a), a.stride(0), _p(weight), _p(bias), _p(out), out.stride(0), M, N, K, act, terms, _p(absmax), scale,
                plan_m, _p(run_if), _stream()), "e3d_gemm_bias_act_f32_split_gated")
        return out
    with _timed("gemm", (M, N, K, act)):
        if _skinny_ok(terms, M, N, K, a) and out.stride(0) % 4 == 0 and M <= min(SKINNY_MAX_M, SKINNY_GEMM_MAX_M):
            ws = _skinny_workspace(a.device, M, N, K)
            hip.check(hip.lib().e3d_gemm_skinny_f32_split_ex(_p(a), a.stride(0), _p(weight), _p(bias), _p(out), out.stride(0),
                                                             M, N, K, act, terms, _p(ws), ws.numel(), _p(absmax), scale, _stream()),
                      "e3d_gemm_skinny_f32_split_ex")
        elif terms == 0:
            hip.check(hip.lib().e3d_gemm_bias_act_f32(_p(a), a.stride(0), _p(weight), _p(bias), _p(out),
                                                      out.stride(0), M, N, K, act, _stream()), "e3d_gemm_bias_act_f32")
        else:
            hip.check(hip.lib().e3d_gemm_bias_act_f32_split_ex(
                _p(a), a.stride(0), _p(weight), _p(bias), _p(out), out.stride(0), M, N, K, act, terms, _p(absmax), scale,
                _stream()), "e3d_gemm_bias_act_f32_split_ex")
    return out


class arithmetic:

    def __init__(self, mode, respect_env=True):
        self.gemm = os.environ.get("E3D_GEMM_MODE", mode) if respect_env else mode
        self.attn = os.environ.get("E3D_ATTN_MODE", self.gemm) if respect_env else mode

    def __enter__(self):
        self.prev = (set_gemm_mode(self.gemm), set_attn_mode(self.attn))
        return self

    def __exit__(self, *exc):
        set_gemm_mode(self.prev[0])
        set_attn_mode(self.prev[1])


ATTN_MODE = os.environ.get("E3D_ATTN_MODE", GEMM_MODE)
if ATTN_MODE == "bf16":
    ATTN_MODE = "bf16x3"
if ATTN_MODE not in GEMM_MODES:
    raise ValueError(f"E3D_ATTN_MODE must be one of {sorted(GEMM_MODES)}, got {ATTN_MODE!r}")

# ... 85 lines not shown
    p, site, row_keys = drop
    if not 0 <= int(site) < MAX_DROPOUT_SITES:
        raise ValueError(f"{what}: dropout site {site} outside [0, 2^24)")
    if heads >= MAX_DROPOUT_HEADS:
        raise ValueError(f"{what}: keyed dropout holds fewer than 2^16 heads, got {heads}")
    if row_keys.dtype != torch.int64 or not row_keys.is_cuda or not row_keys.is_contiguous() or row_keys.numel() != rows:
        raise ValueError(f"{what}: row keys must be a contiguous int64 device tensor of {rows} keys")
    return float(p), int(site), _p(row_keys)


def keyed_drop_row_keys(ids, L, epoch_word, seed, stream):
    if stream not in (keyed.DROP_LIGAND, keyed.DROP_POCKET):
        raise ValueError(f"dropout row keys live on streams {keyed.DROP_LIGAND} / {keyed.DROP_POCKET}, got {stream}")
    if L > keyed.MAX_POSITION:
        raise ValueError(f"keyed streams hold positions below 2^24, got a frame of {L}")
    B = ids.numel()
    assert ids.dtype == torch.int64 and ids.is_cuda and ids.is_contiguous() and epoch_word.dtype == torch.int64 and epoch_word.is_cuda
    out = torch.empty((B * L,), device=ids.device, dtype=torch.int64)
    hip.check(hip.lib().e3d_keyed_drop_row_keys(_p(ids), B, L, _p(epoch_word), keyed.check_seed(seed), int(stream), _p(out),
                                                _stream()), "e3d_keyed_drop_row_keys")
    return out


def dropout(x, p, seed, out=None, row_keys=None):
    _chk(x, "dropout.x")
    assert x.is_contiguous()
    out = torch.empty_like(x) if out is None else out
    if row_keys is not None:
        H = x.shape[-1]
        M = x.numel() // H
        p, site, keys = _keyed_drop((p, seed, row_keys), M, "dropout")
        hip.check(hip.lib().e3d_dropout_f32_keyed(_p(x), p, site, keys, _p(out), M, H, _stream()), "e3d_dropout_f32_keyed")
        return out
    hip.check(hip.lib().e3d_dropout_f32(_p(x), float(p), int(seed), _p(out), x.numel(), _stream()), "e3d_dropout_f32")
    return out


def keyed_attn_dropout_mask(B, nh, Lq, Lk, p, site, row_keys):
    out = torch.empty((B, nh, Lq, Lk), device=row_keys.device, dtype=torch.float32)
    p, site, keys = _keyed_drop((p, site, row_keys), B * Lq, "keyed_attn_dropout_mask", nh)
    hip.check(hip.lib().e3d_keyed_attn_dropout_mask(B, nh, Lq, Lk, p, site, keys, _p(out), _stream()),
              "e3d_keyed_attn_dropout_mask")
    return out


def attn_dropout_mask(B, nh, Lq, Lk, p, seed, device="cuda"):
    out = torch.empty((B, nh, Lq, Lk), device=device, dtype=torch.float32)
    hip.check(hip.lib().e3d_attn_dropout_mask(B, nh, Lq, Lk, float(p), int(seed), _p(out), _stream()),
              "e3d_attn_dropout_mask")
    return out


def attention(q, k, v, B, nh, Lq, Lk, key_mask=None, dist_emb=None, max_pos=0, want_lse=False, mode=None, drop=None,
              bounds=None):
    for n, t in (("q", q), ("k", k), ("v", v), ("key_mask", key_mask), ("dist_emb", dist_emb)):
        _chk(t, "attention." + n)
    assert q.stride(1) == 1 and k.stride(1) == 1 and v.stride(1) == 1
    assert q.shape[0] == B * Lq and k.shape[0] == B * Lk and v.shape[0] == B * Lk
    if key_mask is not None:
        assert key_mask.is_contiguous() and key_mask.shape == (B, Lk)
    if dist_emb is not None:
        assert dist_emb.is_contiguous() and dist_emb.shape == (2 * max_pos - 1, 64), dist_emb.shape
    out = torch.empty((B * Lq, nh * 64), device=q.device, dtype=torch.float32)
    lse = torch.empty((B, nh, Lq), device=q.device, dtype=torch.float32) if want_lse else None
    terms = GEMM_MODES[ATTN_MODE if mode is None else mode]
    with _timed("attn_relkey" if dist_emb is not None else "attn_cross", (B, nh, Lq, Lk)):
        args = (_p(q), Lq * q.stride(0), q.stride(0), _p(k), Lk * k.stride(0), k.stride(0),
                _p(v), Lk * v.stride(0), v.stride(0), _p(dist_emb), max_pos, _p(key_mask), _p(out), _p(lse),
                B, nh, Lq, Lk)
        dropping = drop is not None and drop[0] > 0
        if terms == 0 and not dropping:
            hip.check(hip.lib().e3d_relkey_attn_fwd(*args, _stream()), "e3d_relkey_attn_fwd")
        else:
            scratch, ready, e_abs = None, 0, None
            q_abs, k_abs = bounds if bounds is not None else (None, None)
            if dist_emb is not None:
                infer = not torch.is_grad_enabled()
                ent = getattr(dist_emb, "_e3d_planes", None) if infer else None
                if ent is not None and ent[0] == weight_key(dist_emb) + (Lk, terms):
                    scratch, ready, e_abs = ent[1], 1, ent[2]
                else:
                    scratch = torch.empty((hip.lib().e3d_attn_scratch_bytes(Lk),), device=q.device, dtype=torch.uint8)
                    e_abs = None
                    have_bounds = q_abs is not None and k_abs is not None
                    if have_bounds and not infer:
                        try:
                            e_abs = absmax_slot(dist_emb, "e", q.device)
                        except AttributeError:
                            e_abs = torch.zeros(1, device=q.device, dtype=torch.float32)
                    elif have_bounds:
                        e_abs = torch.zeros(1, device=q.device, dtype=torch.float32)
                    if infer and not torch.cuda.is_current_stream_capturing():
                        try:
                            if e_abs is None:
                                e_abs = absmax(dist_emb.detach())
                            dist_emb._e3d_planes = (weight_key(dist_emb) + (Lk, terms), scratch, e_abs)
                        except AttributeError:
                            pass
            p, seed = (float(drop[0]), int(drop[1])) if dropping else (0.0, 0)
            if q_abs is None or k_abs is None or (dist_emb is not None and e_abs is None):
                q_abs = k_abs = e_abs = None
            if dropping and len(drop) == 3:
                p, site, keys = _keyed_drop(drop, B * Lq, "attention", nh)
                hip.check(hip.lib().e3d_relkey_attn_fwd_split_ex_keyed(*args, terms or 6, p, site, keys, _p(scratch), ready,
                                                                       _p(q_abs), _p(k_abs), _p(e_abs), _stream()),
                          "e3d_relkey_attn_fwd_split_ex_keyed")
                return (out, lse) if want_lse else out
            hip.check(hip.lib().e3d_relkey_attn_fwd_split_ex(*args, terms or 6, p, seed, _p(scratch), ready, _p(q_abs),
                                                             _p(k_abs), _p(e_abs), _stream()),
                      "e3d_relkey_attn_fwd_split_ex")
    return (out, lse) if want_lse else out


def attention_varlen(q, k, v, q_layout, k_layout, nh, dist_emb=None, max_pos=0, mode=None):
    if torch.is_grad_enabled() and any(t is not None and t.requires_grad for t in (q, k, v, dist_emb)):
        raise RuntimeError("attention_varlen is inference-only: run it under torch.no_grad()")
    for n, t in (("q", q), ("k", k), ("v", v), ("dist_emb", dist_emb)):
        _chk(t, "attention_varlen." + n)
    assert q.dim() == 2 and q.stride(1) == 1 and k.stride(1) == 1 and v.stride(1) == 1
    if q.shape[0] != q_layout.rows or k.shape[0] != k_layout.rows or v.shape[0] != k_layout.rows:
        raise ValueError(f"attention_varlen: rows q {q.shape[0]} / k {k.shape[0]} / v {v.shape[0]} against layouts of "
                         f"{q_layout.rows} / {k_layout.rows} rows")
    if q_layout.B != k_layout.B:
        raise ValueError(f"attention_varlen: {q_layout.B} query segments against {k_layout.B} key segments")
    if dist_emb is not None:
        assert dist_emb.is_contiguous() and dist_emb.shape == (2 * max_pos - 1, 64), dist_emb.shape
        if not q_layout.same_segments(k_layout):
            raise ValueError("attention_varlen: relative_key self-attention needs q_len == k_len for every segment")
    alloc = torch.zeros if q_layout.padded_frame else torch.empty
    out = alloc((q_layout.rows, nh * 64), device=q.device, dtype=torch.float32)
    terms = GEMM_MODES[ATTN_MODE if mode is None else mode]
    if q_layout.n_tiles == 0:
        return out
    with _timed("attn_varlen", (q_layout.B, nh, q_layout.rows, k_layout.rows)):
        hip.check(hip.lib().e3d_attn_varlen_fwd(
            _p(q), q.stride(0), _p(k), k.stride(0), _p(v), v.stride(0), _p(q_layout.start_dev), _p(q_layout.len_dev),
            _p(k_layout.start_dev), _p(k_layout.len_dev), _p(q_layout.tiles), q_layout.n_tiles, _p(dist_emb), max_pos,
            _p(out), q_layout.rows, nh, q_layout.max_len, k_layout.max_len, terms, _stream()), "e3d_attn_varlen_fwd")
    return out


def residual_layernorm(x, residual, gamma, beta, eps, want_s=False, drop=None):
    for n, t in (("x", x), ("residual", residual), ("gamma", gamma), ("beta", beta)):
        _chk(t, "residual_layernorm." + n)
    assert x.is_contiguous() and (residual is None or residual.is_contiguous())
    M, H = x.shape
    out = torch.empty_like(x)
    s = torch.empty_like(x) if want_s else None
    with _timed("residual_layernorm", (M, H)):
        if drop is not None and drop[0] > 0 and len(drop) == 3:
            p, site, keys = _keyed_drop(drop, M, "residual_layernorm")
            hip.check(hip.lib().e3d_residual_layernorm_drop_fwd_keyed(_p(x), _p(residual), _p(gamma), _p(beta), eps, _p(s), _p(out),
                                                                      M, H, p, site, keys, _stream()),
                      "e3d_residual_layernorm_drop_fwd_keyed")
        elif drop is not None and drop[0] > 0:
            hip.check(hip.lib().e3d_residual_layernorm_drop_fwd(_p(x), _p(residual), _p(gamma), _p(beta), eps, _p(s), _p(out), M, H,
                                                                float(drop[0]), int(drop[1]), _stream()),
                      "e3d_residual_layernorm_drop_fwd")
        else:
            hip.check(hip.lib().e3d_residual_layernorm_fwd(_p(x), _p(residual), _p(gamma), _p(beta), eps, _p(s),
                                                           _p(out), M, H, _stream()), "e3d_residual_layernorm_fwd")
    return (out, s) if want_s else out


ROWLN_MIN_M = int(os.environ.get("E3D_GEMM_ROWLN_MIN_M", "8192")) if os.environ.get("E3D_GEMM_ROWLN", "1") == "1" else 1 << 62


def weight_planes(weight, terms):
    ent = getattr(weight, "_e3d_planes_w", None)
    key = weight_key(weight) + (terms,)
    if ent is not None and ent[0] == key:
        return ent[1], ent[2]
    if torch.cuda.is_current_stream_capturing():
        raise RuntimeError("weight_planes: cache miss inside a stream capture (warm the op up before capturing)")
    src, scale = f16_weight(weight) if terms == 19 else (weight.detach(), 1.0)
    N, K = src.shape
    nbytes = hip.lib().e3d_weight_planes_bytes(N, K)
    if nbytes < 0:
        raise ValueError(f"weight_planes: unsupported shape {tuple(src.shape)}")
    planes = torch.empty((nbytes,), dtype=torch.uint8, device=src.device)
    hip.check(hip.lib().e3d_weight_planes_f32_split(_p(src), N, K, terms, _p(planes), _stream()), "e3d_weight_planes_f32_split")
    try:
        weight._e3d_planes_w = (key, planes, scale)
    except AttributeError:
        pass
    return planes, scale


def rowln_ok(terms, M, H, K, a, residual=None):
    return (terms in (3, 19) and M >= ROWLN_MIN_M and a.stride(1) == 1 and a.data_ptr() % 16 == 0
            and (residual is None or (residual.stride(1) == 1 and residual.stride(0) % 4 == 0 and residual.data_ptr() % 16 == 0))
            and bool(hip.lib().e3d_gemm_residual_layernorm_supported(M, H, K, a.stride(0))))


def linear_residual_layernorm(a, weight, bias, residual, gamma, beta, eps, mode=None):
    M, K = a.shape
    H = weight.shape[0]
    terms = GEMM_MODES[GEMM_MODE if mode is None else mode]
    if rowln_ok(terms, M, H, K, a, residual):
        for t, n in ((a, "a"), (weight, "weight"), (bias, "bias"), (residual, "residual"), (gamma, "gamma"), (beta, "beta")):
            _chk(t, "linear_residual_layernorm." + n)
        assert weight.is_contiguous() and weight.shape[1] == K and (residual is None or residual.shape == (M, H))
        planes, scale = weight_planes(weight, terms)
        out = torch.empty((M, H), device=a.device, dtype=torch.float32)
        with _timed("gemm_layernorm", (M, H, K)):
            hip.check(hip.lib().e3d_gemm_residual_layernorm_f32_split(
                _p(a), a.stride(0), _p(planes), _p(bias), _p(residual), residual.stride(0) if residual is not None else 0,
                _p(gamma), _p(beta), eps, _p(out), out.stride(0), M, H, K, terms, scale, _stream()),
                "e3d_gemm_residual_layernorm_f32_split")
        return out
    if not (_skinny_ok(terms, M, H, K, a) and H in (256, 512, 768, 1024) and a.stride(1) == 1):
        return residual_layernorm(gemm(a, weight, bias, mode=mode), residual, gamma, beta, eps)
    for t, n in ((a, "a"), (weight, "weight"), (bias, "bias"), (residual, "residual"), (gamma, "gamma"), (beta, "beta")):
        _chk(t, "linear_residual_layernorm." + n)
    assert weight.is_contiguous() and weight.shape[1] == K and (residual is None or (residual.is_contiguous() and residual.shape == (M, H)))
    out = torch.empty((M, H), device=a.device, dtype=torch.float32)
    ws = _skinny_workspace(a.device, M, H, K)
    scale = 1.0
    if terms == 19:
        weight, scale = f16_weight(weight)
    with _timed("gemm_layernorm", (M, H, K)):
        hip.check(hip.lib().e3d_gemm_skinny_residual_layernorm_f32_split_ex(
            _p(a), a.stride(0), _p(weight), _p(bias), _p(residual), _p(gamma), _p(beta), eps, _p(out), M, H, K, terms,
            _p(ws), ws.numel(), scale, _stream()), "e3d_gemm_skinny_residual_layernorm_f32_split_ex")
    return out

def adaln_gate(x, y, mod, branch, rows_per_cond):
    for n, t in (("x", x), ("y", y), ("mod", mod)):
        _chk(t, "adaln_gate." + n)
    assert x.is_contiguous() and y.is_contiguous() and mod.is_contiguous()
    M, H = x.shape
    assert mod.shape[1] == 6 * H and mod.shape[0] * rows_per_cond == M, (mod.shape, M, rows_per_cond)
    out = torch.empty_like(x)
    with _timed("adaln_gate", (M, H)):
        hip.check(hip.lib().e3d_adaln_gate_fwd(_p(x), _p(y), _p(mod), branch, rows_per_cond, _p(out),
                                               M, H, _stream()), "e3d_adaln_gate_fwd")
    return out


def adaln_gate_indexed(x, y, idx, table, mod, branch):
    for n, t in (("x", x), ("y", y), ("table", table), ("mod", mod)):
        _chk(t, "adaln_gate_indexed." + n)
    _chk(idx, "adaln_gate_indexed.idx", torch.int32)
    assert x.is_contiguous() and y.is_contiguous() and mod.is_contiguous() and table.is_contiguous() and idx.is_contiguous()
    M, H = x.shape
    assert y.shape == x.shape and mod.shape == (M, 6 * H) and table.shape[1] == 6 * H and idx.shape == (M,), (mod.shape, table.shape, idx.shape)
    out = torch.empty_like(x)
    with _timed("adaln_gate", (M, H)):
        hip.check(hip.lib().e3d_adaln_gate_indexed_fwd(_p(x), _p(y), _p(idx), _p(table), table.shape[0], _p(mod), branch,
                                                       _p(out), M, H, _stream()), "e3d_adaln_gate_indexed_fwd")
    return out
# ... 280 lines not shown
```

### include/e3d_hip.h

```cpp
#ifndef E3D_HIP_H
#define E3D_HIP_H

#include <stdint.h>

#ifdef __cplusplus
extern "C" {
#endif

#define E3D_ABI_VERSION 5

#define E3D_TERMS_BF16 1
#define E3D_TERMS_BF16X3 3
#define E3D_TERMS_BF16X6 6
#define E3D_TERMS_F16X3 19

#define E3D_ACT_NONE 0
#define E3D_ACT_GELU 1
#define E3D_ACT_SILU 2

int e3d_abi_version(void);
const char* e3d_last_error(void);

int e3d_gemm_bias_act_f32(const float* A, int64_t lda, const float* W, const float* bias,
                          float* out, int64_t ldc, int M, int N, int K, int act, void* stream);
// ... 171 lines not shown
int e3d_relkey_attn_bwd_drop(const float* q, int64_t q_bs, int64_t q_rs, const float* k, int64_t k_bs,
                             int64_t k_rs, const float* v, int64_t v_bs, int64_t v_rs,
                             const float* dist_emb, int P, const float* key_mask, const float* out,
                             const float* lse, const float* dout, float* dq, int64_t dq_bs,
                             int64_t dq_rs, float* dk, int64_t dk_bs, int64_t dk_rs, float* dv,
                             int64_t dv_bs, int64_t dv_rs, float* d_dist_emb, float* workspace, int B,
                             int nh, int Lq, int Lk, float drop_p, uint64_t drop_seed, void* stream);

int e3d_relkey_attn_bwd_ex(const float* q, int64_t q_bs, int64_t q_rs, const float* k, int64_t k_bs,
                           int64_t k_rs, const float* v, int64_t v_bs, int64_t v_rs,
                           const float* dist_emb, int P, const float* key_mask, const float* out,
                           const float* lse, const float* dout, float* dq, int64_t dq_bs, int64_t dq_rs,
                           float* dk, int64_t dk_bs, int64_t dk_rs, float* dv, int64_t dv_bs,
                           int64_t dv_rs, float* d_dist_emb, float* workspace, int B, int nh, int Lq,
                           int Lk, int terms, float drop_p, uint64_t drop_seed, void* stream);

int e3d_attn_dropout_mask(int B, int nh, int Lq, int Lk, float p, uint64_t seed, float* out, void* stream);

int e3d_layernorm_bwd(const float* dy, const float* s, const float* gamma, float eps, float* ds,
                      float* dgamma, float* dbeta, int M, int H, void* stream);

int e3d_adaln_gate_bwd(const float* dout, const float* y, const float* mod, int branch,
                       int rows_per_cond, float* dy, float* dmod, int M, int H, void* stream);

int e3d_act_fwd(const float* z, int act, float* out, int64_t n, void* stream);
int e3d_act_bwd(const float* dh, const float* z, int act, float* dz, int64_t n, void* stream);

int e3d_colsum(const float* x, int64_t ld, float* out, int M, int N, void* stream);
int e3d_transpose_grouped_f32(const float* const* src, float* const* dst, int count, int rows, int cols, int64_t ld_src,
                              int64_t ld_dst, void* stream);
int e3d_group_sum(const float* x, int rows_per_group, float* out, int M, int H, void* stream);

int e3d_small_k_wgrad(const float* g, const float* x, float* dW, float* db, int M, int H, int F,
                      int transpose_out, void* stream);

int e3d_head_linear_bwd_dx(const float* dout, const float* W, float* dx, int M, int H, int Nout,
                           void* stream);

int e3d_residual_layernorm_drop_fwd(const float* x, const float* residual, const float* gamma, const float* beta, float eps,
                                    float* s_out, float* out, int M, int H, float drop_p, uint64_t drop_seed, void* stream);
int e3d_layernorm_bwd_drop(const float* dy, const float* s, const float* gamma, float eps, float* ds, float* ds_dropped,
                           float* dgamma, float* dbeta, int M, int H, float drop_p, uint64_t drop_seed, void* stream);
int64_t e3d_layernorm_bwd_workspace_floats(int M, int H);
int e3d_layernorm_bwd_ws(const float* dy, const float* s, const float* gamma, float eps, float* ds, float* ds_dropped,
                         float* dgamma, float* dbeta, int M, int H, float drop_p, uint64_t drop_seed, float* workspace,
                         int64_t workspace_floats, void* stream);

int64_t e3d_weight_planes_bytes(int N, int K);
int e3d_weight_planes_f32_split(const float* W, int N, int K, int terms, void* planes, void* stream);
int e3d_gemm_residual_layernorm_supported(int M, int N, int K, int64_t lda);
int e3d_gemm_residual_layernorm_f32_split(const float* A, int64_t lda, const void* w_planes, const float* bias,
                                          const float* residual, int64_t ldr, const float* gamma, const float* beta, float eps,
                                          float* out, int64_t ldo, int M, int N, int K, int terms, float out_scale, void* stream);

int e3d_adamw_step_dyn(float* const* params, const float* const* grads, float* const* exp_avg, float* const* exp_avg_sq,
                       const int64_t* numel, const int* chunk_tensor, const int64_t* chunk_first, int n_chunks,
                       const float* norm_and_clip, const float* lr_and_step, float beta1, float beta2, float eps,
                       float weight_decay, void* stream);
int e3d_adamw_step_dev(float* const* params, const float* const* grads, float* const* exp_avg, float* const* exp_avg_sq,
                       const int64_t* numel, const int* chunk_tensor, const int64_t* chunk_first, int n_chunks,
                       const float* norm_and_clip, const float* hyper, void* stream);
int e3d_dropout_set_epoch_ptr(const uint64_t* device_word);
int e3d_optim_chunk_elems(void);
int e3d_grad_global_norm(const float* const* grads, const int64_t* numel, const int* chunk_tensor, const int64_t* chunk_first,
                         int n_chunks, float max_norm, float* partial, float* norm_and_clip, void* stream);
int e3d_adamw_step(float* const* params, const float* const* grads, float* const* exp_avg, float* const* exp_avg_sq,
                   const int64_t* numel, const int* chunk_tensor, const int64_t* chunk_first, int n_chunks,
                   const float* norm_and_clip, float lr, float beta1, float beta2, float eps, float weight_decay, int step,
                   void* stream);

int e3d_keyed_drop_row_keys(const int64_t* ids, int B, int L, const int64_t* epoch_word, uint64_t seed, int stream,
                            uint64_t* out, void* st);
int e3d_dropout_f32_keyed(const float* x, float p, uint32_t site, const uint64_t* row_keys, float* out, int M, int H,
                          void* stream);
int e3d_keyed_attn_dropout_mask(int B, int nh, int Lq, int Lk, float p, uint32_t site, const uint64_t* row_keys, float* out,
                                void* stream);
int e3d_residual_layernorm_drop_fwd_keyed(const float* x, const float* residual, const float* gamma, const float* beta, float eps,
                                          float* s_out, float* out, int M, int H, float drop_p, uint32_t site,
                                          const uint64_t* row_keys, void* stream);
int e3d_layernorm_bwd_drop_keyed(const float* dy, const float* s, const float* gamma, float eps, float* ds, float* ds_dropped,
                                 float* dgamma, float* dbeta, int M, int H, float drop_p, uint32_t site, const uint64_t* row_keys,
                                 void* stream);
int e3d_layernorm_bwd_ws_keyed(const float* dy, const float* s, const float* gamma, float eps, float* ds, float* ds_dropped,
                               float* dgamma, float* dbeta, int M, int H, float drop_p, uint32_t site, const uint64_t* row_keys,
                               float* workspace, int64_t workspace_floats, void* stream);
int e3d_relkey_attn_fwd_split_drop_keyed(const float* q, int64_t q_bs, int64_t q_rs, const float* k, int64_t k_bs,
                                         int64_t k_rs, const float* v, int64_t v_bs, int64_t v_rs, const float* dist_emb,
                                         int P, const float* key_mask, float* out, float* lse, int B, int nh, int Lq, int Lk,
                                         int terms, float drop_p, uint32_t site, const uint64_t* row_keys, void* stream);
int e3d_relkey_attn_fwd_split_ex_keyed(const float* q, int64_t q_bs, int64_t q_rs, const float* k, int64_t k_bs,
                                       int64_t k_rs, const float* v, int64_t v_bs, int64_t v_rs, const float* dist_emb,
                                       int P, const float* key_mask, float* out, float* lse, int B, int nh, int Lq, int Lk,
                                       int terms, float drop_p, uint32_t site, const uint64_t* row_keys, void* e_scratch,
                                       int e_scratch_ready, const float* q_absmax, const float* k_absmax, float* e_absmax,
                                       void* stream);
int e3d_relkey_attn_bwd_drop_keyed(const float* q, int64_t q_bs, int64_t q_rs, const float* k, int64_t k_bs, int64_t k_rs,
                                   const float* v, int64_t v_bs, int64_t v_rs, const float* dist_emb, int P,
                                   const float* key_mask, const float* out, const float* lse, const float* dout, float* dq,
                                   int64_t dq_bs, int64_t dq_rs, float* dk, int64_t dk_bs, int64_t dk_rs, float* dv,
                                   int64_t dv_bs, int64_t dv_rs, float* d_dist_emb, float* workspace, int B, int nh, int Lq,
                                   int Lk, float drop_p, uint32_t site, const uint64_t* row_keys, void* stream);
int e3d_relkey_attn_bwd_ex_keyed(const float* q, int64_t q_bs, int64_t q_rs, const float* k, int64_t k_bs, int64_t k_rs,
                                 const float* v, int64_t v_bs, int64_t v_rs, const float* dist_emb, int P,
                                 const float* key_mask, const float* out, const float* lse, const float* dout, float* dq,
                                 int64_t dq_bs, int64_t dq_rs, float* dk, int64_t dk_bs, int64_t dk_rs, float* dv,
                                 int64_t dv_bs, int64_t dv_rs, float* d_dist_emb, float* workspace, int B, int nh, int Lq,
// ... 16 lines not shown
```

Measured before the change: 3991 pocket-steps/s.

## Emit pre-split hi/lo activation planes from attention and GELU GEMM epilogues

The attention kernel and the intermediate GELU GEMM can now write their outputs directly as split hi/lo 16-bit operand planes in the tiled layout the following GEMM+residual+LayerNorm kernel reads. That kernel gains a path that consumes these planes instead of re-reading fp32 activations and splitting them in its prologue. The aim is to cut activation memory traffic and the repeated split work in the inference path. The cost is extra kernel variants, layout coupling between stages, and the gating logic that decides when the plane path applies.

```diff
diff --git a/e3-invaraint-diffusion-model_amd/autograd.py b/e3-invaraint-diffusion-model_amd/autograd.py
--- a/e3-invaraint-diffusion-model_amd/autograd.py
+++ b/e3-invaraint-diffusion-model_amd/autograd.py
@@ -513,9 +513,12 @@
 
 class functional:
     @staticmethod
-    def linear(x, weight, bias=None, act=ops.ACT_NONE, absmax=None):
+    def linear(x, weight, bias=None, act=ops.ACT_NONE, absmax=None, planes_for=None):
         if _needs_grad(x, weight, bias):
             out = _Linear.apply(x, weight, bias, act, absmax)
+        elif planes_for is not None and absmax is None and ops.gemm_planes_ok(x, weight, bias, act, planes_for[0].shape[0],
+                                                                              planes_for[1]):
+            return ops.gemm(x, weight, bias, act, planes_out=True)
         else:
             out = ops.gemm(x, weight, bias, act, absmax=absmax)
         if absmax is not None:
@@ -523,7 +526,8 @@
         return out
 
     @staticmethod
-    def attention(q_src, kv_src, B, nh, Lq, Lk, key_mask=None, dist_emb=None, max_pos=0, drop_p=0.0, row_keys=None):
+    def attention(q_src, kv_src, B, nh, Lq, Lk, key_mask=None, dist_emb=None, max_pos=0, drop_p=0.0, row_keys=None,
+                  planes_for=None):
         q_abs = getattr(q_src, "_e3d_absmax", None)
         k_abs = q_abs if kv_src is None else getattr(kv_src, "_e3d_absmax", None)
         bounds = (q_abs, k_abs) if q_abs is not None and k_abs is not None else None
@@ -531,8 +535,10 @@
             return _Attention.apply(q_src, kv_src, dist_emb, key_mask, B, nh, Lq, Lk, max_pos, drop_p, bounds, row_keys)
         q, k, v = _Attention._views(q_src, kv_src, nh * 64)
         drop = ops.site_drop(drop_p, row_keys) if drop_p > 0 else None
+        planes = (planes_for is not None and drop is None and
+                  ops.attention_planes_ok(q, k, v, nh, Lq, Lk, planes_for[0].shape[0], planes_for[1]))
         return ops.attention(q, k, v, B, nh, Lq, Lk, key_mask=key_mask, dist_emb=dist_emb, max_pos=max_pos, drop=drop,
-                             bounds=bounds)
+                             bounds=bounds, planes_out=planes)
 
     @staticmethod
     def dropout(x, p, training=True, row_keys=None):
diff --git a/e3-invaraint-diffusion-model_amd/bert.py b/e3-invaraint-diffusion-model_amd/bert.py
--- a/e3-invaraint-diffusion-model_amd/bert.py
+++ b/e3-invaraint-diffusion-model_amd/bert.py
@@ -187,6 +187,10 @@
                                        att.output.LayerNorm.bias, att.eps, p_hidden, row_keys)
 
 
+def _planes_for(att, x, drop):
+    return (att.output.dense.weight, x) if drop[0] == 0 and drop[1] == 0 else None
+
+
 def drop_keys(drop):
     return drop[2] if len(drop) > 2 else None
 
@@ -204,7 +208,8 @@
         return _attention_output(att, ctx, x)
     ctx = F.attention(qkv, None, B, att.num_heads, L, L, key_mask=mask,
                       dist_emb=sa.distance_embedding.weight if relkey else None,
-                      max_pos=sa.max_position_embeddings, drop_p=drop[1], row_keys=drop_keys(drop))
+                      max_pos=sa.max_position_embeddings, drop_p=drop[1], row_keys=drop_keys(drop),
+                      planes_for=_planes_for(att, x, drop))
     return _attention_output(att, ctx, x, drop[0], drop_keys(drop))
 
 
@@ -219,7 +224,8 @@
         H = att.num_heads * 64
         ctx = ops.attention_varlen(q, kv[:, :H], kv[:, H:], layout, enc_layout, att.num_heads)
         return _attention_output(att, ctx, x)
-    ctx = F.attention(q, kv, B, att.num_heads, Lq, Lk, key_mask=enc_mask, drop_p=drop[1], row_keys=drop_keys(drop))
+    ctx = F.attention(q, kv, B, att.num_heads, Lq, Lk, key_mask=enc_mask, drop_p=drop[1], row_keys=drop_keys(drop),
+                      planes_for=_planes_for(att, x, drop))
     return _attention_output(att, ctx, x, drop[0], drop_keys(drop))
 
 
@@ -231,7 +237,8 @@
             raise ValueError("decoder layer needs encoder states")
         x = run_cross_attention(layer.crossattention, x, cross_kv, enc_mask, B, L, Lk, drop, layout=layout,
                                 enc_layout=enc_layout)
-    inter = F.linear(x, layer.intermediate.dense.weight, layer.intermediate.dense.bias, ops.ACT_GELU)
+    inter = F.linear(x, layer.intermediate.dense.weight, layer.intermediate.dense.bias, ops.ACT_GELU,
+                     planes_for=(layer.output.dense.weight, x) if drop[0] == 0 and drop[1] == 0 else None)
     return F.linear_residual_layernorm(inter, layer.output.dense.weight, layer.output.dense.bias, x,
                                        layer.output.LayerNorm.weight, layer.output.LayerNorm.bias, layer.eps, drop[0],
                                        drop_keys(drop))
diff --git a/e3-invaraint-diffusion-model_amd/csrc/attn_relkey_coop.hip b/e3-invaraint-diffusion-model_amd/csrc/attn_relkey_coop.hip
--- a/e3-invaraint-diffusion-model_amd/csrc/attn_relkey_coop.hip
+++ b/e3-invaraint-diffusion-model_amd/csrc/attn_relkey_coop.hip
@@ -130,7 +130,7 @@
 #define KSTAMP(i) do {} while (0)
 #endif
 
-template <int W, bool RELKEY, typename E, bool DROP = false>
+template <int W, bool RELKEY, typename E, bool DROP = false, bool PLANES = false>
 __global__ __launch_bounds__(W * 64, 2) void attn_coop_kernel(
     const float* __restrict__ q, int64_t q_bs, int64_t q_rs, const float* __restrict__ k, int64_t k_bs,
     int64_t k_rs, const float* __restrict__ v, int64_t v_bs, int64_t v_rs, const typename AV<E>::x8* __restrict__ e_frag,
@@ -413,6 +413,30 @@
     KSTAMP(2);
     const float l_tot = l_run + __shfl_xor(l_run, 32, 64);
     const float inv = 1.0f / l_tot;
+    if constexpr (PLANES) {
+        unsigned char* pb = reinterpret_cast<unsigned char*>(out) +
+                            ((((int64_t)b * Lq + q0) >> 5) * (nh * 4) + 4 * h) * 2048 + lane * 16;
+#pragma unroll
+        for (int ks = 0; ks < 4; ++ks) {
+            const int r0 = 8 * (ks & 1);
+            float x[8];
+#pragma unroll
+            for (int j = 0; j < 4; ++j) {
+                float a = (ks < 2 ? o0[r0 + j] : o1[r0 + j]) * inv, c = (ks < 2 ? o0[r0 + 4 + j] : o1[r0 + 4 + j]) * inv;
+                asm volatile("" : "+v"(a));
+                asm volatile("" : "+v"(c));
+                const auto sw = __builtin_amdgcn_permlane32_swap(__float_as_uint(a), __float_as_uint(c), false, false);
+                x[j] = __uint_as_float(sw[0]);
+                x[4 + j] = __uint_as_float(sw[1]);
+            }
+            bf16x8 hi, lo;
+            split8x2(x, hi, lo);
+            *reinterpret_cast<bf16x8*>(pb + ks * 2048) = hi;
+            *reinterpret_cast<bf16x8*>(pb + ks * 2048 + 1024) = lo;
+        }
+        if (lse && half == 0 && q0 + qi < Lq) lse[((int64_t)b * nh + h) * Lq + q0 + qi] = m_run * LN2 + logf(l_tot);
+        return;
+    }
     __builtin_amdgcn_wave_barrier();
 #pragma unroll
     for (int g = 0; g < 4; ++g) {
@@ -445,9 +469,23 @@
 int launch_w(const float* q, int64_t q_bs, int64_t q_rs, const float* k, int64_t k_bs, int64_t k_rs, const float* v,
              int64_t v_bs, int64_t v_rs, const void* e_frag, int P, const float* key_mask,
              float* out, float* lse, int B, int nh, int Lq, int Lk, int q_tiles, int skip, E3dBounds bnd, E3dDrop drop,
-             bool dropping, hipStream_t s) {
+             bool dropping, bool planes, hipStream_t s) {
     const size_t lds = 2 * KV_BUF_B + (size_t)W * RING_F * sizeof(float);
     const int groups = q_tiles / W;
+    if (planes) {
+        if constexpr (W == 4) {
+            if (!dropping && Lq % 32 == 0) {
+                static std::atomic<uint64_t> lds_ok_p{0};
+                e3d_allow_lds(lds_ok_p, attn_coop_kernel<W, RELKEY, E, false, true>, lds);
+                hipLaunchKernelGGL((attn_coop_kernel<W, RELKEY, E, false, true>), dim3(B * nh * groups), dim3(W * 64), lds, s, q, q_bs,
+                                   q_rs, k, k_bs, k_rs, v, v_bs, v_rs, reinterpret_cast<const typename AV<E>::x8*>(e_frag), P,
+                                   key_mask, out, lse, nh, Lq, Lk, groups, skip, bnd, g_rescale_tau, drop);
+                return e3d_launch_status("e3d_relkey_attn_fwd_split_planes (cooperative)");
+            }
+        }
+        e3d_set_error("attn_coop: plane output exists for the 4-wave inference forms with Lq %% 32 == 0 only");
+        return -1;
+    }
     if constexpr (std::is_same<E, __bf16>::value) {
         if (dropping) {
             static std::atomic<uint64_t> lds_ok_d{0};
@@ -469,11 +507,11 @@
 int launch_any(int W, const float* q, int64_t q_bs, int64_t q_rs, const float* k, int64_t k_bs, int64_t k_rs,
                const float* v, int64_t v_bs, int64_t v_rs, const void* e_frag, int P,
                const float* key_mask, float* out, float* lse, int B, int nh, int Lq, int Lk, int q_tiles, int skip,
-               E3dBounds bnd, E3dDrop drop, bool dropping, hipStream_t s) {
+               E3dBounds bnd, E3dDrop drop, bool dropping, bool planes, hipStream_t s) {
 #define E3D_COOP_CASE(w)                                                                                          \
     case w:                                                                                                       \
         return launch_w<w, RELKEY, E>(q, q_bs, q_rs, k, k_bs, k_rs, v, v_bs, v_rs, e_frag, P, key_mask, out, lse, B, nh, \
-                                   Lq, Lk, q_tiles, skip, bnd, drop, dropping, s)
+                                   Lq, Lk, q_tiles, skip, bnd, drop, dropping, planes, s)
     switch (W) {
         E3D_COOP_CASE(8);
         E3D_COOP_CASE(4);
@@ -488,7 +526,7 @@
 static int coop_launch_t(const float* q, int64_t q_bs, int64_t q_rs, const float* k, int64_t k_bs, int64_t k_rs,
                          const float* v, int64_t v_bs, int64_t v_rs, const float* dist_emb, int P,
                          const float* key_mask, float* out, float* lse, int B, int nh, int Lq, int Lk, int skip,
-                         E3dBounds bnd, void* e_scratch, int e_ready, E3dDrop drop, bool dropping, hipStream_t s) {
+                         E3dBounds bnd, void* e_scratch, int e_ready, E3dDrop drop, bool dropping, bool planes, hipStream_t s) {
     const int q_tiles = (Lq + 31) / 32;
     static int w_pref = 0;
     if (!w_pref) {
@@ -498,7 +536,7 @@
     const int W = (w_pref == 8 && q_tiles % 8 == 0) ? 8 : 4;
     if (!dist_emb)
         return launch_any<false, E>(W, q, q_bs, q_rs, k, k_bs, k_rs, v, v_bs, v_rs, nullptr, P, key_mask, out, lse, B, nh,
-                                    Lq, Lk, q_tiles, skip, bnd, drop, dropping, s);
+                                    Lq, Lk, q_tiles, skip, bnd, drop, dropping, planes, s);
     if (!e_scratch) {
         e3d_set_error("attn_coop: rel-key attention needs the caller's scratch for the distance-table planes");
         return -1;
@@ -508,18 +546,24 @@
         hipLaunchKernelGGL(e_fragments_kernel<E>, dim3((n_items + 255) / 256), dim3(256), 0, s, dist_emb,
                            reinterpret_cast<typename AV<E>::x8*>(e_scratch), P, J0, n_items, (float*)nullptr);
     return launch_any<true, E>(W, q, q_bs, q_rs, k, k_bs, k_rs, v, v_bs, v_rs, e_scratch, P, key_mask, out, lse, B, nh, Lq,
-                               Lk, q_tiles, skip, bnd, drop, dropping, s);
+                               Lk, q_tiles, skip, bnd, drop, dropping, planes, s);
+}
+
+int e3d_attn_coop_waves(int Lq) {
+    const char* e = getenv("E3D_ATTN_W");
+    return ((e ? atoi(e) : 4) == 8 && ((Lq + 31) / 32) % 8 == 0) ? 8 : 4;
 }
 
 int e3d_attn_coop_launch(const float* q, int64_t q_bs, int64_t q_rs, const float* k, int64_t k_bs, int64_t k_rs,
                          const float* v, int64_t v_bs, int64_t v_rs, const float* dist_emb, int P,
                          const float* key_mask, float* out, float* lse, int B, int nh, int Lq, int Lk, int skip,
-                         E3dBounds bnd, void* e_scratch, int e_ready, int f16, E3dDrop drop, bool dropping, hipStream_t s) {
+                         E3dBounds bnd, void* e_scratch, int e_ready, int f16, E3dDrop drop, bool dropping, bool planes,
+                         hipStream_t s) {
     if (f16)
         return coop_launch_t<_Float16>(q, q_bs, q_rs, k, k_bs, k_rs, v, v_bs, v_rs, dist_emb, P, key_mask, out, lse, B, nh, Lq,
-                                       Lk, skip, bnd, e_scratch, e_ready, drop, dropping, s);
+                                       Lk, skip, bnd, e_scratch, e_ready, drop, dropping, planes, s);
     return coop_launch_t<__bf16>(q, q_bs, q_rs, k, k_bs, k_rs, v, v_bs, v_rs, dist_emb, P, key_mask, out, lse, B, nh, Lq, Lk,
-                                 skip, bnd, e_scratch, e_ready, drop, dropping, s);
+                                 skip, bnd, e_scratch, e_ready, drop, dropping, planes, s);
 }
 
 extern "C" float e3d_attn_rescale_tau(float tau) {
diff --git a/e3-invaraint-diffusion-model_amd/csrc/attn_relkey_split.hip b/e3-invaraint-diffusion-model_amd/csrc/attn_relkey_split.hip
--- a/e3-invaraint-diffusion-model_amd/csrc/attn_relkey_split.hip
+++ b/e3-invaraint-diffusion-model_amd/csrc/attn_relkey_split.hip
@@ -192,11 +192,23 @@
     return prev;
 }
 
+static bool attn_coop_ok(int64_t k_rs, int64_t v_bs, int64_t v_rs, int Lq, int Lk, int terms, bool dropping, bool have_scratch) {
+    static int coop = -1;
+    if (coop < 0) {
+        const char* e = getenv("E3D_ATTN_COOP");
+        coop = e ? atoi(e) : 1;
+    }
+    const bool span_ok = (int64_t)Lk * (k_rs > v_rs ? k_rs : v_rs) * 4 < ((int64_t)1 << 31) && k_rs > 0 && v_rs > 0 &&
+                         k_rs < ((int64_t)1 << 24) && v_rs < ((int64_t)1 << 24);
+    return (terms == 3 || (terms == E3D_TERMS_F16X3 && !dropping)) && coop && span_ok && v_rs % 4 == 0 && v_bs % 4 == 0 &&
+           ((Lq + 31) / 32) % 4 == 0 && have_scratch;
+}
+
 static int attn_fwd_dispatch(const float* q, int64_t q_bs, int64_t q_rs, const float* k, int64_t k_bs, int64_t k_rs,
                              const float* v, int64_t v_bs, int64_t v_rs, const float* dist_emb, int P, const float* key_mask,
                              float* out, float* lse, int B, int nh, int Lq, int Lk, int terms, float drop_p, const E3dDrop d,
                              void* e_scratch, int e_scratch_ready, const float* q_absmax, const float* k_absmax,
-                             float* e_absmax, void* stream) {
+                             float* e_absmax, void* stream, bool planes_out = false) {
     const E3dBounds bnd{q_absmax, k_absmax, dist_emb ? e_absmax : nullptr};
     E3D_REQUIRE(!dist_emb || !q_absmax || e_absmax, "attn_split: rel-key attention with element bounds needs e_absmax too");
     E3D_REQUIRE(drop_p >= 0.f && drop_p < 1.f, "attn_split: drop_p=%g outside [0, 1)", (double)drop_p);
@@ -221,18 +233,11 @@
         if (rc) return rc;
         e_scratch_ready = 1;
     }
-    static int coop = -1;
-    if (coop < 0) {
-        const char* e = getenv("E3D_ATTN_COOP");
-        coop = e ? atoi(e) : 1;
-    }
     const bool dropping = drop_p > 0.f;
-    const bool span_ok = (int64_t)Lk * (k_rs > v_rs ? k_rs : v_rs) * 4 < ((int64_t)1 << 31) && k_rs > 0 && v_rs > 0 &&
-                         k_rs < ((int64_t)1 << 24) && v_rs < ((int64_t)1 << 24);
-    if ((terms == 3 || (f16 && !dropping)) && coop && span_ok && v_rs % 4 == 0 && v_bs % 4 == 0 && ((Lq + 31) / 32) % 4 == 0 &&
-        (!dist_emb || e_scratch))
+    if (attn_coop_ok(k_rs, v_bs, v_rs, Lq, Lk, terms, dropping, !dist_emb || e_scratch))
         return e3d_attn_coop_launch(q, q_bs, q_rs, k, k_bs, k_rs, v, v_bs, v_rs, dist_emb, P, key_mask, out, lse, B, nh,
-                                    Lq, Lk, g_skip_padded, bnd, e_scratch, e_scratch_ready, f16, d, dropping, s);
+                                    Lq, Lk, g_skip_padded, bnd, e_scratch, e_scratch_ready, f16, d, dropping, planes_out, s);
+    E3D_REQUIRE(!planes_out, "attn_split: plane output needs the cooperative kernel (e3d_attn_planes_supported)");
     if (dropping) {
         if (terms == 3)
             return launch<2, true>(q, q_bs, q_rs, k, k_bs, k_rs, v, v_bs, v_rs, dist_emb, P, key_mask, out, lse, B, nh, Lq, Lk, bnd, s, d);
@@ -296,3 +301,20 @@
                                               nh, Lq, Lk, terms, drop_p, site, row_keys, nullptr, 0, nullptr, nullptr, nullptr,
                                               stream);
 }
+
+extern "C" int e3d_attn_planes_supported(int64_t k_rs, int64_t v_bs, int64_t v_rs, int Lq, int Lk, int terms, int have_scratch) {
+    return (terms == 3 || terms == E3D_TERMS_F16X3) && Lq > 0 && Lq % 32 == 0 && Lk > 0 &&
+           attn_coop_ok(k_rs, v_bs, v_rs, Lq, Lk, terms, false, have_scratch != 0) && e3d_attn_coop_waves(Lq) == 4;
+}
+
+extern "C" int e3d_relkey_attn_fwd_split_planes(const float* q, int64_t q_bs, int64_t q_rs, const float* k, int64_t k_bs,
+                                                int64_t k_rs, const float* v, int64_t v_bs, int64_t v_rs,
+                                                const float* dist_emb, int P, const float* key_mask, void* out_planes,
+                                                int B, int nh, int Lq, int Lk, int terms, void* e_scratch, int e_scratch_ready,
+                                                const float* q_absmax, const float* k_absmax, float* e_absmax, void* stream) {
+    E3D_REQUIRE(e3d_attn_planes_supported(k_rs, v_bs, v_rs, Lq, Lk, terms, !dist_emb || e_scratch),
+                "attn_split (planes): this call does not land on the 4-wave cooperative kernel (Lq=%d Lk=%d terms=%d)", Lq, Lk, terms);
+    return attn_fwd_dispatch(q, q_bs, q_rs, k, k_bs, k_rs, v, v_bs, v_rs, dist_emb, P, key_mask, reinterpret_cast<float*>(out_planes),
+                             nullptr, B, nh, Lq, Lk, terms, 0.f, e3d_drop_make(0.f, 0), e_scratch, e_scratch_ready, q_absmax,
+                             k_absmax, e_absmax, stream, true);
+}
diff --git a/e3-invaraint-diffusion-model_amd/csrc/e3d_common.h b/e3-invaraint-diffusion-model_amd/csrc/e3d_common.h
--- a/e3-invaraint-diffusion-model_amd/csrc/e3d_common.h
+++ b/e3-invaraint-diffusion-model_amd/csrc/e3d_common.h
@@ -206,7 +206,9 @@
 int e3d_attn_coop_launch(const float* q, int64_t q_bs, int64_t q_rs, const float* k, int64_t k_bs, int64_t k_rs,
                          const float* v, int64_t v_bs, int64_t v_rs, const float* dist_emb, int P,
                          const float* key_mask, float* out, float* lse, int B, int nh, int Lq, int Lk, int skip,
-                         E3dBounds bnd, void* e_scratch, int e_ready, int f16, E3dDrop drop, bool dropping, hipStream_t s);
+                         E3dBounds bnd, void* e_scratch, int e_ready, int f16, E3dDrop drop, bool dropping, bool planes,
+                         hipStream_t s);
+int e3d_attn_coop_waves(int Lq);
 
 int e3d_attn_bwd_split_launch(const float* q, int64_t q_bs, int64_t q_rs, const float* k, int64_t k_bs, int64_t k_rs,
                               const float* v, int64_t v_bs, int64_t v_rs, const float* dist_emb, int P,
diff --git a/e3-invaraint-diffusion-model_amd/csrc/gemm_rowln.hip b/e3-invaraint-diffusion-model_amd/csrc/gemm_rowln.hip
--- a/e3-invaraint-diffusion-model_amd/csrc/gemm_rowln.hip
+++ b/e3-invaraint-diffusion-model_amd/csrc/gemm_rowln.hip
@@ -115,7 +115,7 @@
     return left;
 }
 
-template <typename E>
+template <typename E, bool A_PLANES = false>
 __global__ __launch_bounds__(512, 2) void gemm_rowln_kernel(const float* __restrict__ A, int64_t lda,
                                                             const unsigned char* __restrict__ Wp, const float* __restrict__ bias,
                                                             const float* __restrict__ res, int64_t ldr,
@@ -138,6 +138,11 @@
     auto a_offsets = [&](int rows) {
 #pragma unroll
         for (int i = 0; i < 2; ++i) {
+            if (A_PLANES) {
+                const int q = wid + 8 * i;
+                a_lane[i] = (unsigned)(min(q >> 2, (rows >> 5) - 1) * (K >> 4) * 2048 + (q & 3) * 1024 + lane * 16);
+                continue;
+            }
             const int row = (wid + 8 * i) * 8 + (lane >> 3);
             a_lane[i] = (unsigned)(min(row, rows - 1) * (int)lda + (((lane & 7) ^ ((row >> 1) & 7)) << 2)) * 4u;
         }
@@ -145,7 +150,9 @@
     unsigned r_lane[2];
 #pragma unroll
     for (int j = 0; j < 2; ++j) r_lane[j] = (unsigned)((2 * wid + j) * (int)ldr + lane * 4) * 4u;
-    const int a_roff = LDS_A + l31 * 128 + (((2 * half) ^ ((l31 >> 1) & 7)) << 4);
+    const int a_roff = A_PLANES ? LDS_A + lane * 16 : LDS_A + l31 * 128 + (((2 * half) ^ ((l31 >> 1) & 7)) << 4);
+    auto a_frag = [&](int ks, int j) { return A_PLANES ? a_roff + ks * 2048 + j * 1024 : a_roff ^ (64 * ks + 16 * j); };
+    constexpr int A_PAIR_F = A_PLANES ? 1024 : 32;
     const int b_roff = (wid * 3) * 2048 + lane * 16;
 
     auto issue_w = [&](int src, int buf) {
@@ -159,7 +166,7 @@
         glds16<1024>(g + 4096, l + 4096);
     };
     auto issue_a = [&](const float* a_tile, int pair, int buf) {
-        const unsigned char* g = reinterpret_cast<const unsigned char*>(a_tile + pair * 32);
+        const unsigned char* g = reinterpret_cast<const unsigned char*>(a_tile + pair * A_PAIR_F);
         unsigned char* l = smem + LDS_A + buf * A_PAIR + wid * 1024;
         glds16<0>(g + a_lane[0], l);
         glds16<0>(g + a_lane[1], l + 8192);
@@ -219,8 +226,8 @@
             bh0[n] = *reinterpret_cast<const X8*>(smem + b_roff + n * 2048);
             bl0[n] = *reinterpret_cast<const X8*>(smem + b_roff + n * 2048 + 1024);
         }
-        x0 = *reinterpret_cast<const f32x4*>(smem + a_cur + a_roff);
-        x1 = *reinterpret_cast<const f32x4*>(smem + a_cur + (a_roff ^ 16));
+        x0 = *reinterpret_cast<const f32x4*>(smem + a_cur + a_frag(0, 0));
+        x1 = *reinterpret_cast<const f32x4*>(smem + a_cur + a_frag(0, 1));
 
         const bool res_on = res != nullptr && !(ROWLN_LAB & 1);
         const unsigned char* res_tile = reinterpret_cast<const unsigned char*>(res + (int64_t)row0 * ldr);
@@ -238,10 +245,15 @@
 #pragma unroll
             for (int m = 0; m < NM; ++m) {
                 X8 ah, al;
-                split8(x0, x1, ah, al);
+                if constexpr (A_PLANES) {
+                    ah = __builtin_bit_cast(X8, x0);
+                    al = __builtin_bit_cast(X8, x1);
+                } else {
+                    split8(x0, x1, ah, al);
+                }
                 if (m + 1 < NM) {
-                    x0 = *reinterpret_cast<const f32x4*>(smem + a_cur + ((a_roff ^ (64 * KS)) + (m + 1) * 4096));
-                    x1 = *reinterpret_cast<const f32x4*>(smem + a_cur + ((a_roff ^ (64 * KS + 16)) + (m + 1) * 4096));
+                    x0 = *reinterpret_cast<const f32x4*>(smem + a_cur + (a_frag(KS, 0) + (m + 1) * 4096));
+                    x1 = *reinterpret_cast<const f32x4*>(smem + a_cur + (a_frag(KS, 1) + (m + 1) * 4096));
                 }
 #pragma unroll
                 for (int n = 0; n < 3; ++n) {
@@ -266,7 +278,7 @@
                         E3D_BARRIER();
                         RSTAMP(stamp_step, 4);
                         if (a_pair_next >= 0) {
-                            const unsigned char* ga = reinterpret_cast<const unsigned char*>(a_tile + a_pair_next * 32);
+                            const unsigned char* ga = reinterpret_cast<const unsigned char*>(a_tile + a_pair_next * A_PAIR_F);
                             unsigned char* la = smem + LDS_A + a_nx2 + wid * 1024;
                             glds16<0>(ga + a_lane[0], la);
                             glds16<0>(ga + a_lane[1], la + 8192);
@@ -281,8 +293,8 @@
                         nl[n] = *reinterpret_cast<const X8*>(wn + n * 2048 + 1024);
                     }
                     const int an = KS == 0 ? a_cur : a_nxt;
-                    y0 = *reinterpret_cast<const f32x4*>(smem + an + (a_roff ^ (64 * (KS ^ 1))));
-                    y1 = *reinterpret_cast<const f32x4*>(smem + an + (a_roff ^ (64 * (KS ^ 1) + 16)));
+                    y0 = *reinterpret_cast<const f32x4*>(smem + an + a_frag(KS ^ 1, 0));
+                    y1 = *reinterpret_cast<const f32x4*>(smem + an + a_frag(KS ^ 1, 1));
                     __builtin_amdgcn_sched_barrier(0);
                 }
             }
@@ -491,19 +503,36 @@
 #endif
 }
 
-template <typename E>
+template <typename E, bool A_PLANES = false>
 int launch_rowln(const float* A, int64_t lda, const void* Wp, const float* bias, const float* res, int64_t ldr,
                  const float* gamma, const float* beta, float eps, float* out, int64_t ldo, int M, int K, float out_scale,
                  hipStream_t s) {
     static std::atomic<uint64_t> lds_ok{0};
-    e3d_allow_lds(lds_ok, gemm_rowln_kernel<E>, (size_t)LDS_TOTAL);
+    e3d_allow_lds(lds_ok, gemm_rowln_kernel<E, A_PLANES>, (size_t)LDS_TOTAL);
     const int n_cu = e3d_cu_count();
     const int rows_per_wg = ((M + n_cu - 1) / n_cu + 31) / 32 * 32;
     const int grid = (M + rows_per_wg - 1) / rows_per_wg;
-    hipLaunchKernelGGL((gemm_rowln_kernel<E>), dim3(grid), dim3(512), LDS_TOTAL, s, A, lda,
+    hipLaunchKernelGGL((gemm_rowln_kernel<E, A_PLANES>), dim3(grid), dim3(512), LDS_TOTAL, s, A, lda,
                        reinterpret_cast<const unsigned char*>(Wp), bias, res, ldr, gamma, beta, eps, out, ldo, M, K, rows_per_wg,
                        out_scale);
-    return e3d_launch_status("e3d_gemm_residual_layernorm_f32_split");
+    return e3d_launch_status(A_PLANES ? "e3d_gemm_residual_layernorm_planes_split" : "e3d_gemm_residual_layernorm_f32_split");
+}
+
+template <typename E>
+__global__ __launch_bounds__(256) void activation_planes_kernel(const float* __restrict__ X, int64_t ldx, int M, int K,
+                                                                unsigned char* __restrict__ out) {
+    const int lane = threadIdx.x & 63;
+    const int64_t piece = (int64_t)blockIdx.x * 4 + (threadIdx.x >> 6);
+    const int nks = K / 16;
+    if (piece >= (int64_t)(M / 32) * nks) return;
+    const int rb = (int)(piece / nks), ks = (int)(piece % nks);
+    const float* src = X + (int64_t)(rb * 32 + (lane & 31)) * ldx + ks * 16 + 8 * (lane >> 5);
+    const f32x4 a = *reinterpret_cast<const f32x4*>(src), b = *reinterpret_cast<const f32x4*>(src + 4);
+    typename V8<E>::t hi, lo;
+    split8(a, b, hi, lo);
+    unsigned char* dst = out + piece * 2048 + lane * 16;
+    *reinterpret_cast<typename V8<E>::t*>(dst) = hi;
+    *reinterpret_cast<typename V8<E>::t*>(dst + 1024) = lo;
 }
 
 }
@@ -552,3 +581,35 @@
     if (terms == 3) return launch_rowln<__bf16>(A, lda, w_planes, bias, residual, ldr, gamma, beta, eps, out, ldo, M, K, out_scale, s);
     return launch_rowln<_Float16>(A, lda, w_planes, bias, residual, ldr, gamma, beta, eps, out, ldo, M, K, out_scale, s);
 }
+
+extern "C" int64_t e3d_activation_planes_bytes(int M, int K) { return (M % 32 || K % 16 || M <= 0 || K <= 0) ? -1 : (int64_t)M * K * 4; }
+
+extern "C" int e3d_activation_planes_f32_split(const float* X, int64_t ldx, int M, int K, int terms, void* planes, void* stream) {
+    E3D_REQUIRE(X && planes, "activation_planes: null pointer");
+    E3D_REQUIRE(M > 0 && K > 0 && M % 32 == 0 && K % 16 == 0 && ldx >= K && ldx % 4 == 0 && ((uintptr_t)X % 16) == 0 &&
+                    ((uintptr_t)planes % 16) == 0,
+                "activation_planes: need M%%32==0, K%%16==0, ldx%%4==0, 16-byte alignment (M=%d K=%d)", M, K);
+    E3D_REQUIRE(terms == 3 || terms == E3D_TERMS_F16X3, "activation_planes: terms must be 3 or 19 (got %d)", terms);
+    const int64_t pieces = (int64_t)(M / 32) * (K / 16);
+    const dim3 grid((unsigned)((pieces + 3) / 4)), block(256);
+    if (terms == 3) hipLaunchKernelGGL(activation_planes_kernel<__bf16>, grid, block, 0, (hipStream_t)stream, X, ldx, M, K, (unsigned char*)planes);
+    else hipLaunchKernelGGL(activation_planes_kernel<_Float16>, grid, block, 0, (hipStream_t)stream, X, ldx, M, K, (unsigned char*)planes);
+    return e3d_launch_status("e3d_activation_planes_f32_split");
+}
+
+extern "C" int e3d_gemm_residual_layernorm_planes_split(const void* a_planes, const void* w_planes, const float* bias,
+                                                        const float* residual, int64_t ldr, const float* gamma, const float* beta,
+                                                        float eps, float* out, int64_t ldo, int M, int N, int K, int terms,
+                                                        float out_scale, void* stream) {
+    E3D_REQUIRE(a_planes && w_planes && gamma && beta && out, "gemm_residual_layernorm (planes): null pointer");
+    E3D_REQUIRE(e3d_gemm_residual_layernorm_supported(M, N, K, K),
+                "gemm_residual_layernorm (planes): need M%%32==0, N==768, K%%32==0, K>=64 (M=%d N=%d K=%d)", M, N, K);
+    E3D_REQUIRE(((uintptr_t)a_planes % 16) == 0 && ((uintptr_t)w_planes % 16) == 0 && ldo >= N, "gemm_residual_layernorm (planes): alignment / ldo");
+    E3D_REQUIRE(!residual || (ldr >= N && ldr % 4 == 0 && ((uintptr_t)residual % 16) == 0 && 16 * ldr < (1ll << 31)),
+                "gemm_residual_layernorm (planes): residual needs ldr >= N, ldr%%4==0, 16-byte alignment");
+    E3D_REQUIRE(terms == 3 || terms == E3D_TERMS_F16X3, "gemm_residual_layernorm (planes): terms must be 3 or 19 (got %d)", terms);
+    hipStream_t s = (hipStream_t)stream;
+    const float* A = reinterpret_cast<const float*>(a_planes);
+    if (terms == 3) return launch_rowln<__bf16, true>(A, K, w_planes, bias, residual, ldr, gamma, beta, eps, out, ldo, M, K, out_scale, s);
+    return launch_rowln<_Float16, true>(A, K, w_planes, bias, residual, ldr, gamma, beta, eps, out, ldo, M, K, out_scale, s);
+}
diff --git a/e3-invaraint-diffusion-model_amd/csrc/gemm_split.hip b/e3-invaraint-diffusion-model_amd/csrc/gemm_split.hip
--- a/e3-invaraint-diffusion-model_amd/csrc/gemm_split.hip
+++ b/e3-invaraint-diffusion-model_amd/csrc/gemm_split.hip
@@ -741,7 +741,7 @@
 #define E3D_STORE_OUT(ptr, val) (*(ptr) = (val))
 #endif
 
-template <int ACT, typename E>
+template <int ACT, typename E, bool PLANES = false>
 __global__ __launch_bounds__(512, 2) void gemm_split256p_kernel(const float* __restrict__ A, int64_t lda,
                                                                  const float* __restrict__ W,
                                                                  const float* __restrict__ bias,
@@ -843,9 +843,15 @@
                     item_load(g);
 #pragma unroll
                     for (int n = 0; n < 2; ++n) {
-                        acc[m][n] = mma16(fa[0][m], fb[1][n], acc[m][n]);
-                        acc[m][n] = mma16(fa[1][m], fb[0][n], acc[m][n]);
-                        acc[m][n] = mma16(fa[0][m], fb[0][n], acc[m][n]);
+                        if constexpr (PLANES) {
+                            acc[m][n] = mma16(fb[1][n], fa[0][m], acc[m][n]);
+                            acc[m][n] = mma16(fb[0][n], fa[1][m], acc[m][n]);
+                            acc[m][n] = mma16(fb[0][n], fa[0][m], acc[m][n]);
+                        } else {
+                            acc[m][n] = mma16(fa[0][m], fb[1][n], acc[m][n]);
+                            acc[m][n] = mma16(fa[1][m], fb[0][n], acc[m][n]);
+                            acc[m][n] = mma16(fa[0][m], fb[0][n], acc[m][n]);
+                        }
                     }
                     __builtin_amdgcn_sched_barrier(0);
                 }
@@ -855,6 +861,57 @@
             cur ^= 1;
         }
 
+        if constexpr (PLANES) {
+            const int lid = xcd_remap(tile, total);
+            const int row0 = (lid / tiles_n) * BT, col0 = (lid % tiles_n) * BT;
+            unsigned char* const ob = reinterpret_cast<unsigned char*>(out) + lane * 16;
+            const int nks = N >> 4;
+#pragma unroll
+            for (int n = 0; n < 2; ++n) {
+                const int colb = __builtin_amdgcn_readfirstlane(col0 + wc * 64 + n * 32);
+                float bs[32];
+#pragma unroll
+                for (int c = 0; c < 32; ++c) bs[c] = 0.f;
+                if (bias) {
+#pragma unroll
+                    for (int c = 0; c < 32; ++c) bs[c] = bias[colb + c];
+                }
+                float bl[16];
+#pragma unroll
+                for (int r = 0; r < 16; ++r) {
+                    bl[r] = half ? bs[8 * (r >> 2) + 4 + (r & 3)] : bs[8 * (r >> 2) + (r & 3)];
+                    asm volatile("" : "+v"(bl[r]));
+                }
+#pragma unroll
+                for (int m = 0; m < 4; ++m) {
+                    unsigned char* o = ob + ((int64_t)((row0 + wr * 128 + m * 32) >> 5) * nks + (colb >> 4)) * 2048;
+#pragma unroll
+                    for (int kl = 0; kl < 2; ++kl) {
+                        f32x4 x0, x1;
+#pragma unroll
+                        for (int j = 0; j < 4; ++j) {
+                            float a = fmaf(acc[m][n][8 * kl + j], out_scale, bl[8 * kl + j]);
+                            float c = fmaf(acc[m][n][8 * kl + 4 + j], out_scale, bl[8 * kl + 4 + j]);
+                            if (ACT == E3D_ACT_GELU) { a = gelu_erf(a); c = gelu_erf(c); }
+                            if (ACT == E3D_ACT_SILU) { a = silu(a); c = silu(c); }
+                            if (ACT == E3D_ACT_NONE && absmax) { e3d_absmax_accum(amax, a); e3d_absmax_accum(amax, c); }
+                            asm volatile("" : "+v"(a));
+                            asm volatile("" : "+v"(c));
+                            const auto sw = __builtin_amdgcn_permlane32_swap(__float_as_uint(a), __float_as_uint(c), false, false);
+                            x0[j] = __uint_as_float(sw[0]);
+                            x1[j] = __uint_as_float(sw[1]);
+                        }
+                        typename Vec<E>::x4 p0[2], p1[2];
+                        split4<2, E>(x0, p0);
+                        split4<2, E>(x1, p1);
+                        typedef typename Vec<E>::x8 X8;
+                        *reinterpret_cast<X8*>(o + kl * 2048) = __builtin_shufflevector(p0[0], p1[0], 0, 1, 2, 3, 4, 5, 6, 7);
+                        *reinterpret_cast<X8*>(o + kl * 2048 + 1024) = __builtin_shufflevector(p0[1], p1[1], 0, 1, 2, 3, 4, 5, 6, 7);
+                    }
+                }
+            }
+            continue;
+        }
         const int lid = xcd_remap(tile, total);
         const int row0 = (lid / tiles_n) * BT, col0 = (lid % tiles_n) * BT;
 #pragma unroll
@@ -878,7 +935,7 @@
     if (ACT == E3D_ACT_NONE && absmax) e3d_absmax_commit(amax, absmax, lane);
 }
 
-template <int ACT, typename E>
+template <int ACT, typename E, bool PLANES = false>
 int launch256p(const float* A, int64_t lda, const float* W, const float* bias, float* out, int64_t ldc, int M, int N,
                int K, Epi epi, hipStream_t s) {
     const int tiles_m = M / BT, tiles_n = N / BT;
@@ -886,10 +943,10 @@
     static std::atomic<uint64_t> lds_ok{0};
     const int n_cu = e3d_cu_count();
     const int total = tiles_m * tiles_n;
-    e3d_allow_lds(lds_ok, gemm_split256p_kernel<ACT, E>, lds);
-    hipLaunchKernelGGL((gemm_split256p_kernel<ACT, E>), dim3(total < n_cu ? total : n_cu), dim3(512), lds, s, A, lda, W, bias, out,
+    e3d_allow_lds(lds_ok, gemm_split256p_kernel<ACT, E, PLANES>, lds);
+    hipLaunchKernelGGL((gemm_split256p_kernel<ACT, E, PLANES>), dim3(total < n_cu ? total : n_cu), dim3(512), lds, s, A, lda, W, bias, out,
                        ldc, N, K, tiles_m, tiles_n, epi.absmax, epi.scale, epi.run_if);
-    return e3d_launch_status("e3d_gemm_f32_split (persistent 256x256)");
+    return e3d_launch_status(PLANES ? "e3d_gemm_bias_act_planes_split (persistent 256x256)" : "e3d_gemm_f32_split (persistent 256x256)");
 }
 
 int g_general_form = -1;
@@ -921,6 +978,16 @@
     return v;
 }
 
+bool persistent_ok(int M, int Mp, int N, int K, int64_t lda, int64_t ldb, int k_min = 2 * BK) {
+    if (g_tile_pref < 0) {
+        const char* e = getenv("E3D_GEMM_TILE");
+        g_tile_pref = e ? atoi(e) : 4;
+    }
+    const int64_t n_tiles = (int64_t)(Mp / BT) * (N / BT);
+    return N % BT == 0 && M % BT == 0 && Mp % BT == 0 && ldb == K && g_tile_pref >= 4 && K >= k_min && lda < (1 << 22) &&
+           (g_tile_pref >= 5 || n_tiles >= p_min() || (n_tiles >= 96 && N >= 6 * BT && !getenv("E3D_GEMM_P_MIN")));
+}
+
 template <int NS, int ACT, bool A_KMAJ, bool B_KMAJ, typename E>
 int launch(const float* A, int64_t lda, const float* B, int64_t ldb, const float* bias, float* out, int64_t ldc,
            int M, int N, int K, Epi epi, hipStream_t s) {
@@ -931,9 +998,7 @@
     const int Mp = epi.plan_m > 0 ? epi.plan_m : M;
     if constexpr (!A_KMAJ && !B_KMAJ) {
         if constexpr (NS == 2) {
-            const int64_t n_tiles = (int64_t)(Mp / BT) * (N / BT);
-            if (N % BT == 0 && M % BT == 0 && Mp % BT == 0 && ldb == K && g_tile_pref >= 4 && K >= 2 * BK && lda < (1 << 22) &&
-                (g_tile_pref >= 5 || n_tiles >= p_min() || (n_tiles >= 96 && N >= 6 * BT && !getenv("E3D_GEMM_P_MIN"))))
+            if (persistent_ok(M, Mp, N, K, lda, ldb))
                 return launch256p<ACT, E>(A, lda, B, bias, out, ldc, M, N, K, epi, s);
             if (N % BT == 0 && ldb == K && g_tile_pref >= 3 && (int64_t)((Mp + BT - 1) / BT) * (N / BT) >= 256)
                 return launch256<NS, ACT, 2, 4, 2, true, E>(A, lda, B, bias, out, ldc, M, N, K, epi, s);
@@ -1223,3 +1288,28 @@
     return gemm_split_general(A, lda, 0, W, (int64_t)K, 0, bias, out, ldc, M, N, K, act, terms, out_absmax, out_scale, stream,
                               plan_m, run_if);
 }
+
+extern "C" int e3d_gemm_planes_supported(int M, int N, int K, int64_t lda, int act, int terms) {
+    return (terms == 3 || terms == E3D_TERMS_F16X3) && (act == E3D_ACT_NONE || act == E3D_ACT_GELU) && M > 0 && N > 0 && K > 0 &&
+           K % BK == 0 && lda >= K && lda % 4 == 0 && persistent_ok(M, M, N, K, lda, K, BK);
+}
+
+extern "C" int e3d_gemm_bias_act_planes_split(const float* A, int64_t lda, const float* W, const float* bias, void* out_planes,
+                                              int M, int N, int K, int act, int terms, float* out_absmax, float out_scale,
+                                              void* stream) {
+    E3D_REQUIRE(A && W && out_planes, "gemm_split (planes): null pointer");
+    E3D_REQUIRE(e3d_gemm_planes_supported(M, N, K, lda, act, terms),
+                "gemm_split (planes): this launch does not take the persistent kernel (M=%d N=%d K=%d act=%d terms=%d)", M, N, K, act, terms);
+    E3D_REQUIRE(((uintptr_t)A % 16) == 0 && ((uintptr_t)W % 16) == 0 && ((uintptr_t)bias % 16) == 0 && ((uintptr_t)out_planes % 16) == 0,
+                "gemm_split (planes): A, W, bias and the planes must be 16-byte aligned");
+    E3D_REQUIRE(!out_absmax || act == E3D_ACT_NONE, "gemm_split (planes): out_absmax exists for act = none");
+    const Epi epi{out_absmax, out_scale, 0, nullptr};
+    hipStream_t s = (hipStream_t)stream;
+    float* out = reinterpret_cast<float*>(out_planes);
+    if (terms == 3) {
+        if (act == E3D_ACT_GELU) return launch256p<E3D_ACT_GELU, __bf16, true>(A, lda, W, bias, out, N, M, N, K, epi, s);
+        return launch256p<E3D_ACT_NONE, __bf16, true>(A, lda, W, bias, out, N, M, N, K, epi, s);
+    }
+    if (act == E3D_ACT_GELU) return launch256p<E3D_ACT_GELU, _Float16, true>(A, lda, W, bias, out, N, M, N, K, epi, s);
+    return launch256p<E3D_ACT_NONE, _Float16, true>(A, lda, W, bias, out, N, M, N, K, epi, s);
+}
diff --git a/e3-invaraint-diffusion-model_amd/hip.py b/e3-invaraint-diffusion-model_amd/hip.py
--- a/e3-invaraint-diffusion-model_amd/hip.py
+++ b/e3-invaraint-diffusion-model_amd/hip.py
@@ -50,6 +50,16 @@
     "e3d_gemm_residual_layernorm_supported": (c_int, [c_int, c_int, c_int, c_int64]),
     "e3d_gemm_residual_layernorm_f32_split": (c_int, [_P, c_int64, _P, _P, _P, c_int64, _P, _P, c_float, _P, c_int64,
                                                       c_int, c_int, c_int, c_int, c_float, _P]),
+    "e3d_activation_planes_bytes": (c_int64, [c_int, c_int]),
+    "e3d_activation_planes_f32_split": (c_int, [_P, c_int64, c_int, c_int, c_int, _P, _P]),
+    "e3d_gemm_residual_layernorm_planes_split": (c_int, [_P, _P, _P, _P, c_int64, _P, _P, c_float, _P, c_int64,
+                                                         c_int, c_int, c_int, c_int, c_float, _P]),
+    "e3d_gemm_planes_supported": (c_int, [c_int, c_int, c_int, c_int64, c_int, c_int]),
+    "e3d_gemm_bias_act_planes_split": (c_int, [_P, c_int64, _P, _P, _P, c_int, c_int, c_int, c_int, c_int, _P, c_float, _P]),
+    "e3d_attn_planes_supported": (c_int, [c_int64, c_int64, c_int64, c_int, c_int, c_int, c_int]),
+    "e3d_relkey_attn_fwd_split_planes": (c_int, [_P, c_int64, c_int64, _P, c_int64, c_int64, _P, c_int64, c_int64,
+                                                 _P, c_int, _P, _P, c_int, c_int, c_int, c_int, c_int, _P, c_int,
+                                                 _P, _P, _P, _P]),
     "e3d_gemm_wgrad_ragged_f32_split": (c_int, [_P, _P, _P, _P, _P, _P, _P, _P, c_uint64, c_int, c_int, c_int, _P]),
     "e3d_relkey_attn_bwd_workspace_floats": (c_int64, [c_int, c_int, c_int, c_int, c_int]),
     "e3d_relkey_attn_bwd": (c_int, [_P, c_int64, c_int64, _P, c_int64, c_int64, _P, c_int64, c_int64, _P, c_int, _P,
diff --git a/e3-invaraint-diffusion-model_amd/ops.py b/e3-invaraint-diffusion-model_amd/ops.py
--- a/e3-invaraint-diffusion-model_amd/ops.py
+++ b/e3-invaraint-diffusion-model_amd/ops.py
@@ -210,16 +210,31 @@
     return terms != 0 and not (terms in (3, 19) and M <= min(SKINNY_MAX_M, SKINNY_GEMM_MAX_M))
 
 
-def gemm(a, weight, bias=None, act=ACT_NONE, out=None, mode=None, absmax=None, prescale=True, plan_m=None, run_if=None):
+def gemm(a, weight, bias=None, act=ACT_NONE, out=None, mode=None, absmax=None, prescale=True, plan_m=None, run_if=None,
+         planes_out=False):
     _chk(a, "gemm.a"); _chk(weight, "gemm.weight"); _chk(bias, "gemm.bias")
     assert a.dim() == 2 and a.stride(1) == 1 and weight.is_contiguous()
     M, K = a.shape
     N = weight.shape[0]
     assert weight.shape[1] == K, (a.shape, weight.shape)
+    terms = GEMM_MODES[GEMM_MODE if mode is None else mode]
+    if planes_out:
+        assert out is None and plan_m is None and run_if is None and prescale and terms in (3, 19)
+        if absmax is not None:
+            _chk(absmax, "gemm.absmax")
+            assert act == ACT_NONE and absmax.numel() == 1
+        scale = 1.0
+        if terms == 19:
+            weight, scale = f16_weight(weight)
+        out = torch.empty((M * N * 4,), device=a.device, dtype=torch.uint8)
+        with _timed("gemm", (M, N, K, act)):
+            hip.check(hip.lib().e3d_gemm_bias_act_planes_split(_p(a), a.stride(0), _p(weight), _p(bias), _p(out), M, N, K, act,
+                                                               terms, _p(absmax), scale, _stream()),
+                      "e3d_gemm_bias_act_planes_split")
+        return ActPlanes(out, M, N, terms)
     if out is None:
         out = torch.empty((M, N), device=a.device, dtype=torch.float32)
     assert out.dim() == 2 and out.stride(1) == 1 and out.shape == (M, N)
-    terms = GEMM_MODES[GEMM_MODE if mode is None else mode]
     if absmax is not None:
         _chk(absmax, "gemm.absmax")
         assert act == ACT_NONE and absmax.numel() == 1
@@ -411,7 +426,7 @@
 
 
 def attention(q, k, v, B, nh, Lq, Lk, key_mask=None, dist_emb=None, max_pos=0, want_lse=False, mode=None, drop=None,
-              bounds=None):
+              bounds=None, planes_out=False):
     for n, t in (("q", q), ("k", k), ("v", v), ("key_mask", key_mask), ("dist_emb", dist_emb)):
         _chk(t, "attention." + n)
     assert q.stride(1) == 1 and k.stride(1) == 1 and v.stride(1) == 1
@@ -420,9 +435,13 @@
         assert key_mask.is_contiguous() and key_mask.shape == (B, Lk)
     if dist_emb is not None:
         assert dist_emb.is_contiguous() and dist_emb.shape == (2 * max_pos - 1, 64), dist_emb.shape
-    out = torch.empty((B * Lq, nh * 64), device=q.device, dtype=torch.float32)
+    terms = GEMM_MODES[ATTN_MODE if mode is None else mode]
+    if planes_out:
+        assert not want_lse and (drop is None or drop[0] <= 0) and terms in (3, 19)
+        out = torch.empty((B * Lq * nh * 64 * 4,), device=q.device, dtype=torch.uint8)
+    else:
+        out = torch.empty((B * Lq, nh * 64), device=q.device, dtype=torch.float32)
     lse = torch.empty((B, nh, Lq), device=q.device, dtype=torch.float32) if want_lse else None
-    terms = GEMM_MODES[ATTN_MODE if mode is None else mode]
     with _timed("attn_relkey" if dist_emb is not None else "attn_cross", (B, nh, Lq, Lk)):
         args = (_p(q), Lq * q.stride(0), q.stride(0), _p(k), Lk * k.stride(0), k.stride(0),
                 _p(v), Lk * v.stride(0), v.stride(0), _p(dist_emb), max_pos, _p(key_mask), _p(out), _p(lse),
@@ -459,6 +478,11 @@
             p, seed = (float(drop[0]), int(drop[1])) if dropping else (0.0, 0)
             if q_abs is None or k_abs is None or (dist_emb is not None and e_abs is None):
                 q_abs = k_abs = e_abs = None
+            if planes_out:
+                hip.check(hip.lib().e3d_relkey_attn_fwd_split_planes(*args[:12], _p(out), B, nh, Lq, Lk, terms, _p(scratch), ready,
+                                                                     _p(q_abs), _p(k_abs), _p(e_abs), _stream()),
+                          "e3d_relkey_attn_fwd_split_planes")
+                return ActPlanes(out, B * Lq, nh * 64, terms)
             if dropping and len(drop) == 3:
                 p, site, keys = _keyed_drop(drop, B * Lq, "attention", nh)
                 hip.check(hip.lib().e3d_relkey_attn_fwd_split_ex_keyed(*args, terms or 6, p, site, keys, _p(scratch), ready,
@@ -547,15 +571,92 @@
 
 
 def rowln_ok(terms, M, H, K, a, residual=None):
-    return (terms in (3, 19) and M >= ROWLN_MIN_M and a.stride(1) == 1 and a.data_ptr() % 16 == 0
+    return (terms in (3, 19) and M >= ROWLN_MIN_M and (a is None or (a.stride(1) == 1 and a.data_ptr() % 16 == 0))
             and (residual is None or (residual.stride(1) == 1 and residual.stride(0) % 4 == 0 and residual.data_ptr() % 16 == 0))
-            and bool(hip.lib().e3d_gemm_residual_layernorm_supported(M, H, K, a.stride(0))))
+            and bool(hip.lib().e3d_gemm_residual_layernorm_supported(M, H, K, K if a is None else a.stride(0))))
+
+
+ACT_PLANES = {"1": True, "0": False, "gemm": "gemm", "attn": "attn"}.get(os.environ.get("E3D_ACT_PLANES", "1"))
+if ACT_PLANES is None:
+    raise ValueError(f"E3D_ACT_PLANES must be 1, 0, gemm or attn, got {os.environ['E3D_ACT_PLANES']!r}")
+ACT_PLANES_CALLS = 0
+
+
+class ActPlanes:
+    __slots__ = ("data", "shape", "terms")
+    requires_grad = False
+
+    def __init__(self, data, M, K, terms):
+        self.data, self.shape, self.terms = data, (M, K), terms
+
+    @property
+    def device(self):
+        return self.data.device
+
+    def decode(self):
+        M, K = self.shape
+        dt = torch.float16 if self.terms == 19 else torch.bfloat16
+        t = self.data.view(dt).view(M // 32, K // 16, 2, 2, 32, 8)
+        t = t.permute(2, 0, 4, 1, 3, 5).reshape(2, M, K)
+        return t[0], t[1]
+
+
+def activation_planes(x, mode=None):
+    _chk(x, "activation_planes.x")
+    M, K = x.shape
+    terms = GEMM_MODES[GEMM_MODE if mode is None else mode]
+    nbytes = hip.lib().e3d_activation_planes_bytes(M, K)
+    if nbytes < 0 or terms not in (3, 19) or x.stride(1) != 1:
+        raise ValueError(f"activation_planes: unsupported shape {tuple(x.shape)} / terms {terms}")
+    out = torch.empty((nbytes,), dtype=torch.uint8, device=x.device)
+    hip.check(hip.lib().e3d_activation_planes_f32_split(_p(x), x.stride(0), M, K, terms, _p(out), _stream()),
+              "e3d_activation_planes_f32_split")
+    return ActPlanes(out, M, K, terms)
+
+
+def gemm_planes_ok(a, weight, bias, act, out_features, residual=None, mode=None):
+    if ACT_PLANES not in (True, "gemm") or torch.is_grad_enabled():
+        return False
+    terms = GEMM_MODES[GEMM_MODE if mode is None else mode]
+    M, K = a.shape
+    N = weight.shape[0]
+    return (terms in (3, 19) and rowln_ok(terms, M, out_features, N, None, residual) and a.stride(1) == 1
+            and a.data_ptr() % 16 == 0 and (bias is None or bias.data_ptr() % 16 == 0)
+            and not (_skinny_ok(terms, M, N, K, a) and M <= min(SKINNY_MAX_M, SKINNY_GEMM_MAX_M))
+            and bool(hip.lib().e3d_gemm_planes_supported(M, N, K, a.stride(0), act, terms)))
+
+
+def attention_planes_ok(q, k, v, nh, Lq, Lk, out_features, residual=None, mode=None):
+    if ACT_PLANES not in (True, "attn") or torch.is_grad_enabled():
+        return False
+    terms = GEMM_MODES[ATTN_MODE if mode is None else mode]
+    if terms != GEMM_MODES[GEMM_MODE] or terms not in (3, 19):
+        return False
+    return (rowln_ok(terms, q.shape[0], out_features, nh * 64, None, residual) and v.stride(1) == 1 and k.stride(1) == 1
+            and bool(hip.lib().e3d_attn_planes_supported(k.stride(0), Lk * v.stride(0), v.stride(0), Lq, Lk, terms, 1)))
 
 
 def linear_residual_layernorm(a, weight, bias, residual, gamma, beta, eps, mode=None):
     M, K = a.shape
     H = weight.shape[0]
     terms = GEMM_MODES[GEMM_MODE if mode is None else mode]
+    if isinstance(a, ActPlanes):
+        global ACT_PLANES_CALLS
+        if a.terms != terms or not rowln_ok(terms, M, H, K, None, residual):
+            raise RuntimeError(f"linear_residual_layernorm: no kernel reads activation planes at M={M} H={H} K={K} terms={terms}")
+        _chk(a.data, "linear_residual_layernorm.a", torch.uint8)
+        for t, n in ((weight, "weight"), (bias, "bias"), (residual, "residual"), (gamma, "gamma"), (beta, "beta")):
+            _chk(t, "linear_residual_layernorm." + n)
+        assert weight.is_contiguous() and weight.shape[1] == K and (residual is None or residual.shape == (M, H))
+        planes, scale = weight_planes(weight, terms)
+        out = torch.empty((M, H), device=a.device, dtype=torch.float32)
+        with _timed("gemm_layernorm", (M, H, K)):
+            hip.check(hip.lib().e3d_gemm_residual_layernorm_planes_split(
+                _p(a.data), _p(planes), _p(bias), _p(residual), residual.stride(0) if residual is not None else 0,
+                _p(gamma), _p(beta), eps, _p(out), out.stride(0), M, H, K, terms, scale, _stream()),
+                "e3d_gemm_residual_layernorm_planes_split")
+        ACT_PLANES_CALLS += 1
+        return out
     if rowln_ok(terms, M, H, K, a, residual):
         for t, n in ((a, "a"), (weight, "weight"), (bias, "bias"), (residual, "residual"), (gamma, "gamma"), (beta, "beta")):
             _chk(t, "linear_residual_layernorm." + n)
diff --git a/include/e3d_hip.h b/include/e3d_hip.h
--- a/include/e3d_hip.h
+++ b/include/e3d_hip.h
@@ -247,6 +247,21 @@
 int e3d_gemm_residual_layernorm_f32_split(const float* A, int64_t lda, const void* w_planes, const float* bias,
                                           const float* residual, int64_t ldr, const float* gamma, const float* beta, float eps,
                                           float* out, int64_t ldo, int M, int N, int K, int terms, float out_scale, void* stream);
+
+int64_t e3d_activation_planes_bytes(int M, int K);
+int e3d_activation_planes_f32_split(const float* X, int64_t ldx, int M, int K, int terms, void* planes, void* stream);
+int e3d_gemm_residual_layernorm_planes_split(const void* a_planes, const void* w_planes, const float* bias,
+                                             const float* residual, int64_t ldr, const float* gamma, const float* beta, float eps,
+                                             float* out, int64_t ldo, int M, int N, int K, int terms, float out_scale, void* stream);
+int e3d_gemm_planes_supported(int M, int N, int K, int64_t lda, int act, int terms);
+int e3d_gemm_bias_act_planes_split(const float* A, int64_t lda, const float* W, const float* bias, void* out_planes,
+                                   int M, int N, int K, int act, int terms, float* out_absmax, float out_scale, void* stream);
+int e3d_attn_planes_supported(int64_t k_rs, int64_t v_bs, int64_t v_rs, int Lq, int Lk, int terms, int have_scratch);
+int e3d_relkey_attn_fwd_split_planes(const float* q, int64_t q_bs, int64_t q_rs, const float* k, int64_t k_bs,
+                                     int64_t k_rs, const float* v, int64_t v_bs, int64_t v_rs,
+                                     const float* dist_emb, int P, const float* key_mask, void* out_planes,
+                                     int B, int nh, int Lq, int Lk, int terms, void* e_scratch, int e_scratch_ready,
+                                     const float* q_absmax, const float* k_absmax, float* e_absmax, void* stream);
 
 int e3d_adamw_step_dyn(float* const* params, const float* const* grads, float* const* exp_avg, float* const* exp_avg_sq,
                        const int64_t* numel, const int* chunk_tensor, const int64_t* chunk_first, int n_chunks,
```

New measurement: 4050 pocket-steps/s, median of 6. 1.5% higher.
